# westlake-repl/Adapter4Rec

Hardware: AMD Instinct MI355X
Metric: user-sequences/sec, seq_len=23 BERT+SASRec+Adapter (higher is better)
Workload: dtype bf16

## Files before the change

adapter4rec_amd/_lib.py:

```python
import ctypes as C
import math
import os

import torch

_HERE = os.path.dirname(os.path.abspath(__file__))
LIB_PATH = os.environ.get('A4R_LIB_PATH') or os.path.join(_HERE, 'liba4r_hip.so')

ABI_VERSION = 411
BF16, F32, FP8 = 0, 1, 2
ACT_NONE, ACT_RELU, ACT_GELU, ACT_GELU_TANH, ACT_LEAKY = 0, 1, 2, 3, 4
DACT_MUL = 15
DACT_MUL_Q8 = 14
Q8_OFF, Q8_STEP = 0.1289, 0.0049326
EVAL_MAX_HISTORY = 264
ACT_BY_NAME = {'none': 0, 'relu': 1, 'RELU': 1, 'gelu': 2, 'GELU': 2, 'gelu_new': 3, 'leaky_relu': 4}

EXPORTS = [
    'a4r_version', 'a4r_gemm_nt', 'a4r_gemm_tn', 'a4r_gemm_tn_bias', 'a4r_gemm_tn_multi', 'a4r_gemm_tn2', 'a4r_colsum', 'a4r_attn_fwd', 'a4r_attn_bwd', 'a4r_embed_ln',
    'a4r_ln_fwd', 'a4r_ln_bwd', 'a4r_gather_rows', 'a4r_scatter_rows', 'a4r_rows_idx_copy', 'a4r_act_bwd_f32', 'a4r_score_bce_fwd',
    'a4r_score_bce_bwd', 'a4r_emb_grad_add_inputs', 'a4r_take_inputs', 'a4r_adam_step', 'a4r_pack_matrices',
    'a4r_eval_rank', 'a4r_dropout_apply', 'a4r_gemm_variant', 'a4r_gemm_tail_plan', 'a4r_gemm_tail_max', 'a4r_gemm_rows_256', 'a4r_adapter_ln_fwd', 'a4r_adapter_ln_bwd', 'a4r_ln_fwd_fp8', 'a4r_ln_fwd_sum', 'a4r_quant_rows_fp8', 'a4r_lora_merge', 'a4r_lora_merge_batch', 'a4r_lora_bwd_fused', 'a4r_lora_bwd_fused_ws_floats', 'a4r_phm_build', 'a4r_phm_bwd', 'a4r_unpack_add', 'a4r_memset_zero',
    'a4r_sasrec_block_fwd', 'a4r_sasrec_block_bwd', 'a4r_scatter_rows_fill', 'a4r_attn_long_fwd', 'a4r_attn_long_bwd', 'a4r_patchify', 'a4r_vit_assemble', 'a4r_resample_u8', 'a4r_embed_bwd', 'a4r_mae_keep_indices',
    'a4r_encoder_layer_fwd', 'a4r_encoder_layer_bwd', 'a4r_id_index', 'a4r_id_index_ws_ints', 'a4r_id_grad_sum',
    'a4r_topk_items', 'a4r_grad_sumsq', 'a4r_adamw_step',
]
ID_SUM_CHUNK = 16
TOPK_MAX_K = 256
TOPK_E = (64, 128, 256, 512)
GRAD_NORM_PARTS = 1024


class GemmArgs(C.Structure):
    _fields_ = [('A', C.c_void_p), ('B', C.c_void_p), ('C', C.c_void_p), ('bias', C.c_void_p), ('C2', C.c_void_p),
                ('R1', C.c_void_p), ('R2', C.c_void_p), ('Pre', C.c_void_p),
                ('M', C.c_int32), ('N', C.c_int32), ('K', C.c_int32),
                ('lda', C.c_int32), ('ldb', C.c_int32), ('ldc', C.c_int32), ('ldc2', C.c_int32),
                ('ldr1', C.c_int32), ('ldr2', C.c_int32), ('ldpre', C.c_int32),
                ('in_dtype', C.c_int32), ('out_dtype', C.c_int32), ('act', C.c_int32), ('dact', C.c_int32),
                ('drop_first', C.c_int32), ('c2_mode', C.c_int32), ('alpha', C.c_float), ('drop_p', C.c_float), ('drop_site', C.c_uint32), ('drop_seed', C.c_uint64),
                ('drop_row0', C.c_int64), ('scale_a', C.c_void_p), ('scale_b', C.c_void_p),
                ('c_fp8', C.c_int32), ('c_scale', C.c_float), ('c_scale_out', C.c_void_p), ('q8_tiled', C.c_int32)]


class AttnArgs(C.Structure):
    _fields_ = [('qkv', C.c_void_p), ('ld', C.c_int32), ('q_off', C.c_int32), ('k_off', C.c_int32), ('v_off', C.c_int32),
                ('out', C.c_void_p), ('ldo', C.c_int32), ('dout', C.c_void_p), ('dqkv', C.c_void_p), ('key_mask', C.c_void_p),
                ('n_items', C.c_int32), ('S', C.c_int32), ('n_heads', C.c_int32), ('dh', C.c_int32), ('causal', C.c_int32),
                ('dtype', C.c_int32), ('scale', C.c_float), ('mask_neg', C.c_float),
                ('drop_p', C.c_float), ('drop_site', C.c_uint32), ('drop_seed', C.c_uint64), ('offsets', C.c_void_p)]


class PackDesc(C.Structure):
    _fields_ = [('src_off', C.c_int64), ('dst', C.c_void_p), ('rows', C.c_int32), ('cols', C.c_int32),
                ('rows_pad', C.c_int32), ('cols_pad', C.c_int32), ('transpose', C.c_int32), ('dst_ld', C.c_int32)]


class PhmDesc(C.Structure):
    _fields_ = [('rule_off', C.c_int64), ('wl_off', C.c_int64), ('wr_off', C.c_int64), ('out_off', C.c_int64), ('G', C.c_void_p),
                ('ldg', C.c_int32), ('in_f', C.c_int32), ('out_f', C.c_int32), ('n', C.c_int32), ('pad_', C.c_int32)]


class LayerAdapter(C.Structure):
    _fields_ = [(n, C.c_void_p) for n in ('wd', 'wu', 'wdT', 'wuT', 'wd_f', 'wu_f', 'wdT_f', 'wuT_f', 'bd', 'bu', 'g_wu', 'g_wd', 'g_bu', 'g_bd')] + \
               [(n, C.c_int32) for n in ('ldg_wu', 'ldg_wd', 'act', 'pad_')]


class EncoderLayer(C.Structure):
    _fields_ = [(n, C.c_int32) for n in ('M', 'H', 'F', 'n_items', 'S', 'n_heads', 'dh', 'causal')] + \
               [(n, C.c_float) for n in ('scale', 'mask_neg', 'ln_eps', 'p_attn', 'p_hidden')] + [('drop_site', C.c_uint32), ('drop_seed', C.c_uint64)] + \
               [(n, C.c_void_p) for n in ('key_mask', 'offsets', 'wqkv', 'wqkvT', 'wo', 'woT', 'wi', 'wiT', 'wo2', 'wo2T',
                                          'bqkv', 'bo', 'bi', 'bo2', 'ln1_g', 'ln1_b', 'ln2_g', 'ln2_b')] + \
               [('ad', LayerAdapter * 2)] + \
               [(n, C.c_void_p) for n in ('qkv', 'ctx', 'h1', 'v1', 'zp1', 'z1', 'u', 'upre', 'h2', 'v2', 'zp2', 'z2', 'st1', 'st2')] + \
               [('upre_q8', C.c_int32), ('q8_tiled', C.c_int32)] + \
               [(n, C.c_void_p) for n in ('x_lo', 'x1_lo', 'xout_lo', 'dv1', 'dv2', 'dzp', 'd_h', 'du', 'dx1', 'dctx', 'dqkv')] + [('lo_nibble', C.c_int32)]


class SasrecBlock(C.Structure):
    _PTRS = ('wqkv', 'wfc', 'w1', 'b1', 'w2', 'b2', 'ln1_g', 'ln1_b', 'ln2_g', 'ln2_b', 'wd1', 'bd1', 'wu1', 'bu1', 'wd2', 'bd2', 'wu2', 'bu2',
             'g_wd1', 'g_bd1', 'g_wu1', 'g_bu1', 'g_wd2', 'g_bd2', 'g_wu2', 'g_bu2')
    _fields_ = [(n, C.c_void_p) for n in _PTRS] + \
               [(n, C.c_int32) for n in ('E', 'n_heads', 'F', 'd', 'ldwu', 'ldg_d', 'ldg_u', 'act', 'inner_res')] + \
               [(n, C.c_float) for n in ('eps', 'mask_neg', 'drop_attn', 'drop_hidden')] + [('drop_site', C.c_uint32), ('drop_seed', C.c_uint64)] + \
               [('mode', C.c_int32)] + [(n, C.c_void_p) for n in ('ln3_g', 'ln3_b', 'g_ln3_g', 'g_ln3_b')]


class AddDesc(C.Structure):
    _fields_ = [('src', C.c_void_p), ('dst_off', C.c_int64), ('rows', C.c_int32), ('cols', C.c_int32), ('ld', C.c_int32), ('alpha', C.c_float)]


_lib = None


def lib():
    global _lib
    if _lib is None:
        if not os.path.exists(LIB_PATH):
            raise RuntimeError(
                f'{LIB_PATH} not found: build it with `python -c "import __graft_entry__ as g; g.build()"` '
                '(hipcc --offload-arch=gfx950).  adapter4rec_amd has no CPU / PyTorch fallback.')
        _lib = C.CDLL(LIB_PATH)
        for name in EXPORTS:
            getattr(_lib, name).restype = C.c_int
        _lib.a4r_topk_ws_bytes.restype = C.c_size_t
        got = _lib.a4r_version()
        if got != ABI_VERSION:
            _lib = None
            raise RuntimeError(f'{LIB_PATH} has ABI version {got}, this binding is for {ABI_VERSION}: rebuild it (make -C adapter4rec_amd/csrc)')
    return _lib


def _check(rc, what):
    if rc != 0:
        raise RuntimeError(f'{what} failed with status {rc} ' + {-1: '(invalid argument)', -2: '(launch failure)'}.get(rc, ''))


_DEV_INDEX = None


def _stream():
    global _DEV_INDEX
    if _DEV_INDEX is None:
        _DEV_INDEX = torch.cuda.current_device()
    return C.c_void_p(torch._C._cuda_getCurrentRawStream(_DEV_INDEX))


def _p(t):
    return C.c_void_p(t.data_ptr()) if t is not None else C.c_void_p(0)


def _pi(t):
    return t.data_ptr() if t is not None else 0


def _dt(t):
    if t.dtype == torch.bfloat16:
        return BF16
    if t.dtype == torch.float32:
        return F32
    if t.dtype == torch.uint8:
        return FP8
    raise TypeError(f'unsupported dtype {t.dtype}')


def _ld(t):
    assert t.dim() == 2 and t.stride(1) == 1, 'row-major 2-D tensor expected'
    return t.stride(0)


def require_gpu(*tensors):
    for t in tensors:
        if t is not None and not t.is_cuda:
            raise RuntimeError('adapter4rec_amd kernels need device tensors (no CPU fallback)')


def gemm_nt(A, B, Cout, bias=None, C2=None, R1=None, R2=None, Pre=None, act=0, dact=0, alpha=1.0,
            drop_p=0.0, drop_site=0, drop_seed=0, M=None, drop_first=False, c2_deriv=False, scale_a=None, scale_b=None,
            c_fp8=0, c_scale=1.0, c_scale_out=None, q8_tiled=False):
    if not (A.is_cuda and B.is_cuda and Cout.is_cuda):
        require_gpu(A, B, Cout)
    N, K = B.shape
    din, dout = _dt(A), _dt(Cout)
    if c_fp8:
        assert din == FP8 and Cout.dtype == torch.uint8 and R1 is None and R2 is None and (c_fp8 == 1 or c_scale_out is not None)
        dout = BF16
    assert A.shape[1] == K and Cout.shape[1] == N and _dt(B) == din
    q8c, q8p = c2_deriv == 'q8', dact == DACT_MUL_Q8
    for t, q8 in ((C2, q8c), (R1, False), (R2, False), (Pre, q8p)):
        assert t is None or (t.dtype == torch.uint8 if q8 else _dt(t) == dout)
    assert bias is None or bias.dtype == torch.float32
    g = GemmArgs(A.data_ptr(), B.data_ptr(), Cout.data_ptr(), _pi(bias), _pi(C2), _pi(R1), _pi(R2), _pi(Pre),
                 A.shape[0] if M is None else M, N, K, _ld(A), _ld(B), _ld(Cout),
                 _ld(C2) if C2 is not None else 0, _ld(R1) if R1 is not None else 0, _ld(R2) if R2 is not None else 0,
                 _ld(Pre) if Pre is not None else 0, din, dout, act, dact, int(drop_first), 2 if q8c else int(bool(c2_deriv)), alpha, drop_p, drop_site,
                 drop_seed, 0, _pi(scale_a), _pi(scale_b), int(c_fp8), float(c_scale), _pi(c_scale_out), int(bool(q8_tiled)))
    _check(lib().a4r_gemm_nt(_stream(), C.byref(g)), 'a4r_gemm_nt')


def gemm_variant(v):
    return lib().a4r_gemm_variant(C.c_int(v))


def gemm_tail_max(k):
    return lib().a4r_gemm_tail_max(C.c_int(k))


def gemm_tail_plan(M, N):
    pf, kp = C.c_int(0), C.c_int(0)
    lib().a4r_gemm_tail_plan(C.c_int(M), C.c_int(N), C.byref(pf), C.byref(kp))
    return pf.value, kp.value


def gemm_rows_256(M, N):
    return lib().a4r_gemm_rows_256(C.c_int(M), C.c_int(N))


def adapter_ln_ok(A, d):
    return A.dtype == torch.bfloat16 and d == 64 and A.shape[1] in (128, 256, 512, 768, 1024)


def adapter_ln_fwd(A, R1, R2, Wd, bd, Wu, bu, gamma, beta, eps, act, zp, z, v, y, stats, M=None, y8=None, ys=None, res32=None, y32=None, frag=None):
    require_gpu(A, R1, R2, v, y, res32, y32)
    M = A.shape[0] if M is None else M
    assert y is not None or y8 is not None
    twins = [t for t in (res32, y32) if t is not None]
    lo8 = bool(twins) and twins[0].dtype == torch.int8
    assert all(t.dtype == (torch.int8 if lo8 else torch.float32) and t.shape[0] >= M for t in twins)
    lo4 = lo8 and twins[0].shape[1] == A.shape[1] // 2
    assert not lo8 or all(t.shape[1] == (A.shape[1] // 2 if lo4 else A.shape[1]) for t in twins)
    wd_, wu_ = (Wd, Wu) if frag is None else frag
    _check(lib().a4r_adapter_ln_fwd(_stream(), _p(A), C.c_int(_ld(A)), _p(R1), C.c_int(_ld(R1)), _p(R2), C.c_int(_ld(R2) if R2 is not None else 0),
                                    _p(wd_), _p(bd), _p(wu_), _p(bu), _p(gamma), _p(beta), C.c_float(eps), C.c_int(act),
                                    _p(zp), _p(z), _p(v), C.c_int(_ld(v) if v is not None else 0), _p(y), C.c_int(_ld(y) if y is not None else 0), _p(stats),
                                    C.c_int(M), C.c_int(A.shape[1]), C.c_int(Wd.shape[0]), C.c_int(_dt(A)),
                                    _p(y8), C.c_int(_ld(y8) if y8 is not None else 0), _p(ys),
                                    _p(res32), C.c_int(_ld(res32) if res32 is not None else 0), _p(y32), C.c_int(_ld(y32) if y32 is not None else 0),
                                    C.c_int((0 if frag is None else 1) | (2 if lo8 else 0) | (4 if lo4 else 0))),
           'a4r_adapter_ln_fwd')


def adapter_ln_bwd(dy, v, stats, gamma, dres, zp, act, WuT, WdT, inner_res, dv, dzp, dh, dgamma=None, dbeta=None, dbias=None, M=None,
                   drop_p=0.0, drop_site=0, drop_seed=0, dbd=None, bias_total=False, beta_y=None, frag=None):
    require_gpu(dy, v, dv, dh)
    M = dy.shape[0] if M is None else M
    wut_, wdt_ = (WuT, WdT) if frag is None else frag
    _check(lib().a4r_adapter_ln_bwd(_stream(), _p(dy), C.c_int(_ld(dy)), _p(v), C.c_int(_ld(v)), _p(stats), _p(gamma),
                                    _p(dres), C.c_int(_ld(dres) if dres is not None else 0), _p(zp), C.c_int(act), _p(wut_), _p(wdt_),
                                    C.c_int(int(inner_res)), _p(dv), C.c_int(_ld(dv)), _p(dzp), _p(dh), C.c_int(_ld(dh)),
                                    _p(dgamma), _p(dbeta), _p(dbias), C.c_int(M), C.c_int(dy.shape[1]), C.c_int(WuT.shape[0]), C.c_int(_dt(dy)),
                                    C.c_float(drop_p), C.c_uint32(drop_site), C.c_uint64(drop_seed), _p(dbd),
                                    C.c_int(int(bias_total) | (0 if frag is None else 2)), _p(beta_y)), 'a4r_adapter_ln_bwd')


def sasrec_block(desc, x, log_mask, out, n_users, T, train, dy=None):
    require_gpu(x, log_mask, out, dy)
    assert x.dtype == torch.float32 and out.dtype == torch.float32 and log_mask.dtype == torch.float32 and x.shape[1] == 64 and x.is_contiguous() and out.is_contiguous()
    b = SasrecBlock()
    for k, v in desc.items():
        setattr(b, k, (v.data_ptr() if v is not None else None) if (k in SasrecBlock._PTRS or k in ('ln3_g', 'ln3_b', 'g_ln3_g', 'g_ln3_b')) else v)
    if dy is None:
        _check(lib().a4r_sasrec_block_fwd(_stream(), C.byref(b), _p(x), _p(log_mask), _p(out), C.c_int(n_users), C.c_int(T), C.c_int(int(train))), 'a4r_sasrec_block_fwd')
    else:
        assert dy.dtype == torch.float32 and dy.is_contiguous()
        _check(lib().a4r_sasrec_block_bwd(_stream(), C.byref(b), _p(x), _p(log_mask), _p(dy), _p(out), C.c_int(n_users), C.c_int(T), C.c_int(int(train))),
               'a4r_sasrec_block_bwd')


def gemm_tn(X, Y, Cacc, M=None):
    require_gpu(X, Y, Cacc)
    assert Cacc.dtype == torch.float32 and _dt(X) == _dt(Y)
    M = X.shape[0] if M is None else M
    _check(lib().a4r_gemm_tn(_stream(), _p(X), C.c_int(_ld(X)), _p(Y), C.c_int(_ld(Y)), _p(Cacc), C.c_int(_ld(Cacc)),
                             C.c_int(M), C.c_int(X.shape[1]), C.c_int(Y.shape[1]), C.c_int(_dt(X))), 'a4r_gemm_tn')


def gemm_tn_bias(X, Y, Cacc, xsum, M=None):
    require_gpu(X, Y, Cacc, xsum)
    assert Cacc.dtype == torch.float32 and xsum.dtype == torch.float32 and xsum.numel() >= X.shape[1] and _dt(X) == _dt(Y)
    M = X.shape[0] if M is None else M
    _check(lib().a4r_gemm_tn_bias(_stream(), _p(X), C.c_int(_ld(X)), _p(Y), C.c_int(_ld(Y)), _p(Cacc), C.c_int(_ld(Cacc)),
                                  C.c_int(M), C.c_int(X.shape[1]), C.c_int(Y.shape[1]), C.c_int(_dt(X)), _p(xsum)), 'a4r_gemm_tn_bias')


class TnProb(C.Structure):
    _fields_ = [('X', C.c_void_p), ('Y', C.c_void_p), ('C', C.c_void_p), ('xsum', C.c_void_p),
                ('ldx', C.c_int32), ('ldy', C.c_int32), ('ldc', C.c_int32), ('P', C.c_int32), ('Q', C.c_int32), ('pad_', C.c_int32)]


def gemm_tn_multi(probs, M=None):
    assert 1 <= len(probs) <= 4
    arr = (TnProb * len(probs))()
    dt = _dt(probs[0][0])
    M = probs[0][0].shape[0] if M is None else M
    for a, (X, Y, Cacc, xsum) in zip(arr, probs):
        require_gpu(X, Y, Cacc, xsum)
        assert Cacc.dtype == torch.float32 and _dt(X) == dt and _dt(Y) == dt and (xsum is None or (xsum.dtype == torch.float32 and xsum.numel() >= X.shape[1]))
        a.X, a.Y, a.C, a.xsum = X.data_ptr(), Y.data_ptr(), Cacc.data_ptr(), (xsum.data_ptr() if xsum is not None else None)
        a.ldx, a.ldy, a.ldc, a.P, a.Q = _ld(X), _ld(Y), _ld(Cacc), X.shape[1], Y.shape[1]
    _check(lib().a4r_gemm_tn_multi(_stream(), arr, C.c_int(len(probs)), C.c_int(M), C.c_int(dt)), 'a4r_gemm_tn_multi')


def gemm_tn2(X1, Y1, C1, X2, Y2, C2, M=None, xsum1=None, xsum2=None):
    require_gpu(X1, Y1, C1, X2, Y2, C2, xsum1, xsum2)
    assert C1.dtype == torch.float32 and C2.dtype == torch.float32
    assert (xsum1 is None or (xsum1.dtype == torch.float32 and xsum1.numel() >= X1.shape[1])) and (xsum2 is None or (xsum2.dtype == torch.float32 and xsum2.numel() >= X2.shape[1]))
    M = X1.shape[0] if M is None else M
    _check(lib().a4r_gemm_tn2(_stream(), _p(X1), C.c_int(_ld(X1)), _p(Y1), C.c_int(_ld(Y1)), _p(C1), C.c_int(_ld(C1)), C.c_int(X1.shape[1]), C.c_int(Y1.shape[1]),
                              _p(X2), C.c_int(_ld(X2)), _p(Y2), C.c_int(_ld(Y2)), _p(C2), C.c_int(_ld(C2)), C.c_int(X2.shape[1]), C.c_int(Y2.shape[1]),
                              C.c_int(M), C.c_int(_dt(X1)), _p(xsum1), _p(xsum2)), 'a4r_gemm_tn2')


def colsum(X, out, M=None):
    require_gpu(X, out)
    M = X.shape[0] if M is None else M
    _check(lib().a4r_colsum(_stream(), _p(X), C.c_int(_ld(X)), _p(out), C.c_int(M), C.c_int(X.shape[1]), C.c_int(_dt(X))), 'a4r_colsum')


def _attn_args(qkv, q_off, k_off, v_off, key_mask, n_items, S, n_heads, dh, causal, scale, mask_neg, drop_p, drop_site, drop_seed, offsets=None):
    a = AttnArgs()
    if offsets is not None:
        require_gpu(offsets)
        assert offsets.dtype == torch.int32 and offsets.numel() >= n_items + 1
    a.offsets = _p(offsets)
    a.qkv, a.ld, a.q_off, a.k_off, a.v_off = _p(qkv), _ld(qkv), q_off, k_off, v_off
    a.key_mask = _p(key_mask)
    a.n_items, a.S, a.n_heads, a.dh, a.causal, a.dtype = n_items, S, n_heads, dh, int(causal), _dt(qkv)
    a.scale, a.mask_neg = scale, mask_neg
    a.drop_p, a.drop_site, a.drop_seed = drop_p, drop_site, drop_seed
    return a


def attn_fwd(qkv, out, key_mask, n_items, S, n_heads, dh, q_off, k_off, v_off, causal, scale, mask_neg,
             drop_p=0.0, drop_site=0, drop_seed=0, offsets=None):
    require_gpu(qkv, out)
    a = _attn_args(qkv, q_off, k_off, v_off, key_mask, n_items, S, n_heads, dh, causal, scale, mask_neg, drop_p, drop_site, drop_seed, offsets)
    a.out, a.ldo = _p(out), _ld(out)
    _check(lib().a4r_attn_fwd(_stream(), C.byref(a)), 'a4r_attn_fwd')


def attn_bwd(qkv, dout, dqkv, key_mask, n_items, S, n_heads, dh, q_off, k_off, v_off, causal, scale, mask_neg,
             drop_p=0.0, drop_site=0, drop_seed=0, offsets=None):
    require_gpu(qkv, dout, dqkv)
    assert _ld(dqkv) == _ld(qkv)
    a = _attn_args(qkv, q_off, k_off, v_off, key_mask, n_items, S, n_heads, dh, causal, scale, mask_neg, drop_p, drop_site, drop_seed, offsets)
    a.dout, a.ldo, a.dqkv = _p(dout), _ld(dout), _p(dqkv)
    _check(lib().a4r_attn_bwd(_stream(), C.byref(a)), 'a4r_attn_bwd')


def attn_long_fwd(qkv, out, lse, n_items, S, n_heads, dh, q_off, k_off, v_off, scale, drop_p=0.0, drop_site=0, drop_seed=0, key_mask=None, causal=False):
    require_gpu(qkv, out, lse, key_mask)
    assert lse.dtype == torch.float32 and lse.numel() >= n_items * n_heads * S
    a = _attn_args(qkv, q_off, k_off, v_off, key_mask, n_items, S, n_heads, dh, causal, scale, 0.0, drop_p, drop_site, drop_seed)
    a.out, a.ldo = _p(out), _ld(out)
    _check(lib().a4r_attn_long_fwd(_stream(), C.byref(a), _p(lse)), 'a4r_attn_long_fwd')


def attn_long_bwd(qkv, out, dout, dqkv, lse, delta_ws, n_items, S, n_heads, dh, q_off, k_off, v_off, scale,
                  drop_p=0.0, drop_site=0, drop_seed=0, key_mask=None, causal=False):
    require_gpu(qkv, out, dout, dqkv, lse, delta_ws, key_mask)
    assert _ld(dqkv) == _ld(qkv) and delta_ws.dtype == torch.float32 and delta_ws.numel() >= n_items * n_heads * S
    a = _attn_args(qkv, q_off, k_off, v_off, key_mask, n_items, S, n_heads, dh, causal, scale, 0.0, drop_p, drop_site, drop_seed)
    assert _ld(out) == _ld(dout)
    a.out, a.dout, a.ldo, a.dqkv = _p(out), _p(dout), _ld(dout), _p(dqkv)
    _check(lib().a4r_attn_long_bwd(_stream(), C.byref(a), _p(lse), _p(delta_ws)), 'a4r_attn_long_bwd')


def encoder_layer_fwd(desc, x, x1, x_out):
    require_gpu(x, x1, x_out)
    _check(lib().a4r_encoder_layer_fwd(_stream(), C.byref(desc), _p(x), _p(x1), _p(x_out)), 'a4r_encoder_layer_fwd')


def encoder_layer_bwd(desc, x1, x_out, dx_out, dx_in):
    require_gpu(x1, x_out, dx_out, dx_in)
    _check(lib().a4r_encoder_layer_bwd(_stream(), C.byref(desc), _p(x1), _p(x_out), _p(dx_out), _p(dx_in)), 'a4r_encoder_layer_bwd')


def patchify(img, out, patch, keep_idx=None):
    require_gpu(img, out)
    assert img.is_contiguous()
    if img.dtype == torch.uint8:
        kind, (n, Hi, Wi, Cc) = 1, img.shape
    else:
        assert img.dtype == torch.float32
        kind, (n, Cc, Hi, Wi) = 0, img.shape
    n_keep = keep_idx.shape[1] if keep_idx is not None else (Hi // patch) * (Wi // patch)
    assert keep_idx is None or (keep_idx.dtype == torch.int32 and keep_idx.is_contiguous() and keep_idx.shape[0] == n)
    _check(lib().a4r_patchify(_stream(), _p(img), C.c_int(kind), _p(out), C.c_int(_ld(out)), _p(keep_idx), C.c_int(n_keep),
                              C.c_int(n), C.c_int(Cc), C.c_int(Hi), C.c_int(Wi), C.c_int(patch), C.c_int(_dt(out))), 'a4r_patchify')


def mae_keep_indices(keep, n_patches, noise=None, seed=0, site=0):
    require_gpu(keep, noise)
    assert keep.dtype == torch.int32 and keep.is_contiguous()
    assert noise is None or (noise.dtype == torch.float32 and noise.is_contiguous() and tuple(noise.shape) == (keep.shape[0], n_patches))
    _check(lib().a4r_mae_keep_indices(_stream(), _p(noise), _p(keep), C.c_int(keep.shape[0]), C.c_int(n_patches), C.c_int(keep.shape[1]),
                                      C.c_uint64(int(seed) & (2 ** 64 - 1)), C.c_uint32(site)), 'a4r_mae_keep_indices')


def resample_u8(src, dst, bounds, kk, n_outer, in_len, out_len, inner):
    require_gpu(src, dst, bounds, kk)
    assert src.dtype == torch.uint8 and dst.dtype == torch.uint8 and bounds.dtype == torch.int32 and kk.dtype == torch.int32
    assert src.is_contiguous() and dst.is_contiguous() and src.numel() == n_outer * in_len * inner and dst.numel() == n_outer * out_len * inner
    _check(lib().a4r_resample_u8(_stream(), _p(src), _p(dst), _p(bounds), _p(kk), C.c_int(kk.shape[1]), C.c_long(n_outer),
                                 C.c_int(in_len), C.c_int(out_len), C.c_long(inner)), 'a4r_resample_u8')


def vit_assemble(patches, cls, pos, out, n_items, n_keep, keep_idx=None, tokens_out=0):
    require_gpu(patches, out)
    _check(lib().a4r_vit_assemble(_stream(), _p(patches), C.c_int(_ld(patches)), _p(cls), _p(pos), _p(keep_idx), _p(out),
                                  C.c_int(_ld(out)), C.c_int(n_items), C.c_int(n_keep), C.c_int(cls.numel()), C.c_int(_dt(out)),
                                  C.c_int(tokens_out)), 'a4r_vit_assemble')


def embed_bwd(ids, dpre, dword, dpos, n_items, S, roberta=False, pad_id=0):
    H = dpre.shape[1]
    assert ids.dtype == torch.int64 and ids.dim() == 2 and ids.stride(1) == 1, 'ids: int64 [n_items, >= S] with unit column stride'
    assert ids.shape[0] >= n_items and ids.shape[1] >= S, f'ids {tuple(ids.shape)} smaller than [{n_items}, {S}]'
    assert dpre.dim() == 2 and dpre.shape[0] >= n_items * S, f'dpre {tuple(dpre.shape)}: fewer than {n_items * S} rows'
    for name, t in (('dword', dword), ('dpos', dpos)):
        assert t is None or (t.dtype == torch.float32 and t.dim() == 2 and t.is_contiguous() and t.shape[1] == H), \
            f'{name}: contiguous fp32 [rows, {H}] expected, got {None if t is None else (t.dtype, tuple(t.shape), t.stride())}'
    n_pos = S + pad_id + 1 if roberta else S
    assert dpos is None or dpos.shape[0] >= n_pos, f'dpos has {dpos.shape[0]} rows, position ids reach {n_pos - 1}'
    require_gpu(ids, dpre, dword, dpos)
    _check(lib().a4r_embed_bwd(_stream(), _p(ids), C.c_int(ids.stride(0)), _p(dpre), C.c_int(_ld(dpre)), _p(dword), _p(dpos),
                               C.c_int(n_items), C.c_int(S), C.c_int(dpre.shape[1]), C.c_int(int(roberta)), C.c_int(pad_id),
                               C.c_int(_dt(dpre))), 'a4r_embed_bwd')


def embed_ln(ids, word, pos, type0, gamma, beta, eps, out, n_items, S, roberta=False, pad_id=0,
             drop_p=0.0, drop_site=0, drop_seed=0, pre_out=None, stats_out=None, key_mask_out=None):
    require_gpu(ids, word, out)
    assert ids.dtype == torch.int64 and ids.stride(1) == 1
    _check(lib().a4r_embed_ln(_stream(), _p(ids), C.c_int(ids.stride(0)), _p(word), _p(pos), _p(type0), _p(gamma), _p(beta),
                              C.c_float(eps), _p(out), C.c_int(_ld(out)), C.c_int(n_items), C.c_int(S), C.c_int(word.shape[1]),
                              C.c_int(int(roberta)), C.c_int(pad_id), C.c_int(_dt(out)),
                              C.c_float(drop_p), C.c_uint32(drop_site), C.c_uint64(drop_seed), _p(pre_out), _p(stats_out), _p(key_mask_out)), 'a4r_embed_ln')


def quantize_weight_fp8(w):
    wf = w.detach().float()
    amax = wf.abs().amax(1).clamp_min(1e-30)
    q = (wf * (448.0 / amax)[:, None]).to(torch.float8_e4m3fn).view(torch.uint8).contiguous()
    return q, (amax / 448.0).contiguous()


def quant_rows_fp8(x, q, scale, M=None):
    require_gpu(x, q, scale)
    M = x.shape[0] if M is None else M
    assert q.dtype == torch.uint8 and scale.dtype == torch.float32
    _check(lib().a4r_quant_rows_fp8(_stream(), _p(x), C.c_int(_ld(x)), _p(q), C.c_int(_ld(q)), _p(scale), C.c_int(M), C.c_int(x.shape[1]),
                                    C.c_int(_dt(x))), 'a4r_quant_rows_fp8')


def ln_fwd_sum(h, res, gamma, beta, eps, y, stats, M=None, res32=None, sum_out=None, sum32=None, y32=None):
    require_gpu(h, res, res32, y, sum_out, sum32, y32)
    M = h.shape[0] if M is None else M
    assert res32 is not None or res is not None
    _check(lib().a4r_ln_fwd_sum(_stream(), _p(h), C.c_int(_ld(h)), _p(res32), C.c_int(_ld(res32) if res32 is not None else 0), _p(res),
                                C.c_int(_ld(res) if res is not None else 0), _p(gamma), _p(beta), C.c_float(eps), _p(y), C.c_int(_ld(y)),
                                _p(sum_out), C.c_int(_ld(sum_out) if sum_out is not None else 0), _p(sum32), C.c_int(_ld(sum32) if sum32 is not None else 0),
                                _p(y32), C.c_int(_ld(y32) if y32 is not None else 0), _p(stats), C.c_int(M), C.c_int(h.shape[1]), C.c_int(_dt(h))),
           'a4r_ln_fwd_sum')


def ln_fwd(v, gamma, beta, eps, y, stats, M=None, add=None, drop_p=0.0, drop_site=0, drop_seed=0, y8=None, ys=None):
    require_gpu(v, y, y8)
    M = v.shape[0] if M is None else M
    if y8 is not None:
        assert drop_p == 0.0 and y8.dtype == torch.uint8 and ys.dtype == torch.float32
        _check(lib().a4r_ln_fwd_fp8(_stream(), _p(v), C.c_int(_ld(v)), _p(add), C.c_int(add.shape[0] if add is not None else 0),
                                    _p(gamma), _p(beta), C.c_float(eps), _p(y), C.c_int(_ld(y) if y is not None else 0), _p(y8), C.c_int(_ld(y8)),
                                    _p(ys), _p(stats), C.c_int(M), C.c_int(v.shape[1]), C.c_int(_dt(v))), 'a4r_ln_fwd_fp8')
        return
    _check(lib().a4r_ln_fwd(_stream(), _p(v), C.c_int(_ld(v)), _p(add), C.c_int(add.shape[0] if add is not None else 0),
                            _p(gamma), _p(beta), C.c_float(eps), _p(y), C.c_int(_ld(y)), _p(stats), C.c_int(M),
                            C.c_int(v.shape[1]), C.c_int(_dt(v)), C.c_float(drop_p), C.c_uint32(drop_site), C.c_uint64(drop_seed)),
           'a4r_ln_fwd')


def ln_bwd(dy, v, stats, gamma, dv, M=None, add=None, dgamma=None, dbeta=None, dbias=None, dres=None,
           drop_p=0.0, drop_site=0, drop_seed=0, dv2=None, drop2_p=0.0, drop2_site=0, drop2_seed=0):
    require_gpu(dy, v, dv)
    M = v.shape[0] if M is None else M
    _check(lib().a4r_ln_bwd(_stream(), _p(dy), C.c_int(_ld(dy)), _p(v), C.c_int(_ld(v)), _p(add),
                            C.c_int(add.shape[0] if add is not None else 0), _p(stats), _p(gamma), _p(dres), C.c_int(_ld(dres) if dres is not None else 0), _p(dv), C.c_int(_ld(dv)),
                            _p(dgamma), _p(dbeta), _p(dbias), C.c_int(M), C.c_int(v.shape[1]), C.c_int(_dt(v)),
                            C.c_float(drop_p), C.c_uint32(drop_site), C.c_uint64(drop_seed),
                            _p(dv2), C.c_int(_ld(dv2) if dv2 is not None else 0), C.c_float(drop2_p), C.c_uint32(drop2_site), C.c_uint64(drop2_seed)), 'a4r_ln_bwd')


def gather_rows(src, dst, n, row_step):
    require_gpu(src, dst)
    _check(lib().a4r_gather_rows(_stream(), _p(src), C.c_int(_ld(src)), _p(dst), C.c_int(_ld(dst)), C.c_int(n), C.c_int(row_step),
                                 C.c_int(src.shape[1]), C.c_int(_dt(src))), 'a4r_gather_rows')


def rows_idx_copy(src, dst, idx, n, scatter=False):
    require_gpu(src, dst, idx)
    assert src.dim() == 2 and dst.dim() == 2 and src.dtype == dst.dtype and src.shape[1] == dst.shape[1] and idx.dtype == torch.int32 and idx.numel() >= n
    es = src.element_size()
    _check(lib().a4r_rows_idx_copy(_stream(), _p(src), C.c_int64(src.stride(0) * es), _p(dst), C.c_int64(dst.stride(0) * es), _p(idx), C.c_int(n),
                                   C.c_int64(src.shape[1] * es), C.c_int(int(scatter))), 'a4r_rows_idx_copy')


def id_index_ws_ints(n, item_num):
    k = int(lib().a4r_id_index_ws_ints(C.c_int(n), C.c_int(item_num)))
    if k < 0:
        raise RuntimeError(f'a4r_id_index: n = {n}, item_num = {item_num} outside the supported range (include/a4r.h)')
    return k


def id_index(ids, item_num, rows, slots, ptr, uniq, n_uniq, err, ws):
    require_gpu(ids, rows, slots, ptr, uniq, n_uniq, err, ws)
    n = ids.numel()
    assert ids.dtype == torch.int64 and ids.is_contiguous() and ws.dtype == torch.int32
    assert all(t.dtype == torch.int32 for t in (rows, slots, ptr, uniq, n_uniq, err))
    assert rows.numel() >= n and slots.numel() >= n and ptr.numel() >= n + 1 and uniq.numel() >= n
    _check(lib().a4r_id_index(_stream(), _p(ids), C.c_int(n), C.c_int(item_num), _p(rows), _p(slots), _p(ptr), _p(uniq), _p(n_uniq), _p(err),
                              _p(ws), C.c_int64(ws.numel())), 'a4r_id_index')


def id_grad_sum(src, slots, ptr, uniq, n_uniq, n, grad):
    require_gpu(src, slots, ptr, uniq, n_uniq, grad)
    assert src.dtype == torch.float32 and grad.dtype == torch.float32 and src.shape[1] == grad.shape[1] and src.shape[0] >= n
    _check(lib().a4r_id_grad_sum(_stream(), _p(src), C.c_int(_ld(src)), _p(slots), _p(ptr), _p(uniq), _p(n_uniq), C.c_int(n), _p(grad),
                                 C.c_int(_ld(grad)), C.c_int(grad.shape[1])), 'a4r_id_grad_sum')


def scatter_rows(src, dst, n, row_step):
    require_gpu(src, dst)
    _check(lib().a4r_scatter_rows(_stream(), _p(src), C.c_int(_ld(src)), _p(dst), C.c_int(_ld(dst)), C.c_int(n), C.c_int(row_step),
                                  C.c_int(src.shape[1]), C.c_int(_dt(src))), 'a4r_scatter_rows')


def scatter_rows_fill(src, dst, n, row_step, fill_rows):
    require_gpu(src, dst)
    _check(lib().a4r_scatter_rows_fill(_stream(), _p(src), C.c_int(_ld(src)), _p(dst), C.c_int(_ld(dst)), C.c_int(n), C.c_int(row_step),
                                       C.c_int(src.shape[1]), C.c_int(_dt(src)), C.c_int(fill_rows)), 'a4r_scatter_rows_fill')


def zero(t):
    require_gpu(t)
    assert t.is_contiguous()
    _check(lib().a4r_memset_zero(_stream(), _p(t), C.c_int64(t.numel() * t.element_size())), 'a4r_memset_zero')


def lora_merge(W, A, B, scaling, dst, dstT, r):
    require_gpu(W, dst, dstT)
    out_f, in_f = W.shape
    assert W.dtype == torch.float32 and W.is_contiguous() and (r == 0 or (A.is_contiguous() and B.is_contiguous()))
    _check(lib().a4r_lora_merge(_stream(), _p(W), _p(A) if r else C.c_void_p(0), _p(B) if r else C.c_void_p(0), C.c_float(scaling),
                                _p(dst), C.c_int(_ld(dst)), _p(dstT), C.c_int(_ld(dstT)), C.c_int(out_f), C.c_int(in_f), C.c_int(r),
                                C.c_int(_dt(dst))), 'a4r_lora_merge')


class LoraDesc(C.Structure):
    _fields_ = [('W', C.c_void_p), ('A', C.c_void_p), ('B', C.c_void_p), ('dst', C.c_void_p), ('dstT', C.c_void_p),
                ('scaling', C.c_float), ('ld', C.c_int32), ('ldT', C.c_int32), ('out_f', C.c_int32), ('in_f', C.c_int32), ('r', C.c_int32)]


def lora_table(entries, device):
    descs = []
    for W, A, B, s, dst, dstT, r in entries:
        assert W.dtype == torch.float32 and W.is_contiguous() and (r == 0 or (A.is_contiguous() and B.is_contiguous())) and _dt(dst) == _dt(entries[0][4])
        descs.append(LoraDesc(W.data_ptr(), A.data_ptr() if r else 0, B.data_ptr() if r else 0, dst.data_ptr(), dstT.data_ptr(), float(s),
                              _ld(dst), _ld(dstT), W.shape[0], W.shape[1], int(r)))
    return desc_table(descs, device), len(descs), max(W.numel() for W, *_ in entries), _dt(entries[0][4])


def lora_merge_batch(tab):
    t, n, mx, code = tab
    _check(lib().a4r_lora_merge_batch(_stream(), _p(t), C.c_int(n), C.c_int(mx), C.c_int(code)), 'a4r_lora_merge_batch')


def lora_bwd_fused_ok(x, M, H):
    return x.dtype == torch.bfloat16 and H == 768 and M % 16 == 0


_lora_ws = {}


def lora_bwd_fused(x, dqa, dqb, Aa, Ab, BTa, BTb, scale_a, scale_b, dAa, dAb, dBa, dBb, dbias_a, dbias_b, M, rank_rows=8):
    require_gpu(x, dqa, dqb, dAa, dBa)
    H = x.shape[1]
    assert _ld(dqa) == _ld(dqb) and _ld(Aa) == _ld(Ab) == _ld(BTa) == _ld(BTb) and _ld(dAa) == _ld(dAb) and _ld(dBa) == _ld(dBb)
    ldbias = 0
    for bvec in (dbias_a, dbias_b):
        if bvec is not None:
            assert bvec.dtype == torch.float32 and bvec.dim() == 1
            ldbias = bvec.stride(0)
    ws = _lora_ws.get(x.device)
    if ws is None:
        ws = _lora_ws[x.device] = torch.empty(int(lib().a4r_lora_bwd_fused_ws_floats(C.c_int(H))), dtype=torch.float32, device=x.device)
    _check(lib().a4r_lora_bwd_fused(_stream(), _p(x), C.c_int(_ld(x)), _p(dqa), _p(dqb), C.c_int(_ld(dqa)), _p(Aa), _p(Ab), _p(BTa), _p(BTb),
                                    C.c_int(_ld(Aa)), C.c_float(scale_a), C.c_float(scale_b), _p(dAa), _p(dAb), C.c_int(_ld(dAa)), _p(dBa), _p(dBb),
                                    C.c_int(_ld(dBa)), _p(dbias_a), _p(dbias_b), C.c_int(ldbias), C.c_int(M), C.c_int(H), C.c_int(_dt(x)),
                                    C.c_int(rank_rows), _p(ws), C.c_int64(ws.numel())), 'a4r_lora_bwd_fused')


def desc_table(entries, device):
    arr = (type(entries[0]) * len(entries))(*entries)
    return torch.frombuffer(bytearray(bytes(arr)), dtype=torch.uint8).to(device)


def phm_build(params, desc_dev, n_desc, eff):
    _check(lib().a4r_phm_build(_stream(), _p(params), _p(desc_dev), C.c_int(n_desc), _p(eff)), 'a4r_phm_build')


def phm_bwd(params, desc_dev, n_desc, grads):
    _check(lib().a4r_phm_bwd(_stream(), _p(params), _p(desc_dev), C.c_int(n_desc), _p(grads)), 'a4r_phm_bwd')


def unpack_add(target, desc_dev, n_desc, max_elems):
    _check(lib().a4r_unpack_add(_stream(), _p(target), _p(desc_dev), C.c_int(n_desc), C.c_int(max_elems)), 'a4r_unpack_add')


def dropout_apply(x, y, drop_p, drop_site, drop_seed, M=None):
    require_gpu(x, y)
    M = x.shape[0] if M is None else M
    _check(lib().a4r_dropout_apply(_stream(), _p(x), C.c_int(_ld(x)), _p(y), C.c_int(_ld(y)), C.c_int(M), C.c_int(x.shape[1]),
                                   C.c_int(_dt(x)), C.c_float(drop_p), C.c_uint32(drop_site), C.c_uint64(drop_seed)), 'a4r_dropout_apply')


def act_bwd_f32(dy, pre, dx, act):
    require_gpu(dy, pre, dx)
    _check(lib().a4r_act_bwd_f32(_stream(), _p(dy), _p(pre), _p(dx), C.c_int64(dy.numel()), C.c_int(act)), 'a4r_act_bwd_f32')


def score_bce_fwd(emb, prec, log_mask, pos, neg, loss_ws, B, L, E, cpc):
    require_gpu(emb, prec)
    _check(lib().a4r_score_bce_fwd(_stream(), _p(emb), _p(prec), _p(log_mask), _p(pos), _p(neg), _p(loss_ws),
                                   C.c_int(B), C.c_int(L), C.c_int(E), C.c_int(int(cpc))), 'a4r_score_bce_fwd')


def score_bce_bwd(emb, prec, log_mask, pos, neg, loss_ws, loss_scale, d_prec, d_emb, B, L, E, cpc, scale_dev=None):
    require_gpu(emb, prec, scale_dev)
    assert scale_dev is None or (scale_dev.dtype == torch.float32 and scale_dev.numel() == 1)
    _check(lib().a4r_score_bce_bwd(_stream(), _p(emb), _p(prec), _p(log_mask), _p(pos), _p(neg), _p(loss_ws), C.c_float(loss_scale), _p(scale_dev),
                                   _p(d_prec), _p(d_emb), C.c_int(B), C.c_int(L), C.c_int(E), C.c_int(int(cpc))), 'a4r_score_bce_bwd')


def emb_grad_add_inputs(d_in, d_emb, B, L, E):
    _check(lib().a4r_emb_grad_add_inputs(_stream(), _p(d_in), C.c_int(_ld(d_in)), _p(d_emb), C.c_int(B), C.c_int(L), C.c_int(E)),
           'a4r_emb_grad_add_inputs')


def take_inputs(emb, out, B, L, E):
    _check(lib().a4r_take_inputs(_stream(), _p(emb), _p(out), C.c_int(_ld(out)), C.c_int(B), C.c_int(L), C.c_int(E)), 'a4r_take_inputs')
# ... 98 lines not shown
```

adapter4rec_amd/csrc/a4r_attn.hip:

```cpp
#include <cstdlib>
#include "a4r_common.h"
#include "../../include/a4r.h"

namespace {

template <typename T> A4R_DEV uint4 ldg16(const T* p) { return *reinterpret_cast<const uint4*>(p); }

A4R_DEV void wave_lds_fence() {
    asm volatile("s_waitcnt lgkmcnt(0)" ::: "memory");
    __builtin_amdgcn_wave_barrier();
}

template <typename T, int STRIDE> A4R_DEV void lds_put16(char* tile, int row, int ch, const uint4& v) {
    char* d = tile + row * STRIDE + ch * 16;
    if constexpr (STRIDE % 16 == 0) {
        *reinterpret_cast<uint4*>(d) = v;
    } else {
        reinterpret_cast<uint2*>(d)[0] = make_uint2(v.x, v.y);
        reinterpret_cast<uint2*>(d)[1] = make_uint2(v.z, v.w);
    }
}

template <typename T, int DH> struct AttnCfg {
    static constexpr int PER = Elem<T>::PER16;
    static constexpr int KSTEP = Mma<T>::KSTEP;
    static constexpr int KSD = DH / KSTEP;
    static constexpr int KSP = 32 / KSTEP;
    static constexpr int DT = DH / 16;
    static constexpr int CPR = DH / PER;
    static constexpr int NLD = 32 * CPR / 64;
    static constexpr int PSTRIDE = 32 * (int)sizeof(T);
    static constexpr int GSTRIDE = DH * (int)sizeof(T) + (sizeof(T) == 2 ? 8 : 16);
    static constexpr int OSTRIDE = DH * (int)sizeof(T);
};

template <typename T, int DH>
A4R_DEV void qk_scores(const T* base, int ld, int q_off, int k_off, int S, int lane, f32x4_t (&sc)[2][2]) {
    using C = AttnCfg<T, DH>;
    const int r16 = lane & 15, kg = lane >> 4;
#pragma unroll
    for (int mt = 0; mt < 2; ++mt)
#pragma unroll
        for (int nt = 0; nt < 2; ++nt) sc[mt][nt] = f32x4_t{0.f, 0.f, 0.f, 0.f};
#pragma unroll
    for (int ks = 0; ks < C::KSD; ++ks) {
        uint4 qa[2], kb[2];
#pragma unroll
        for (int t = 0; t < 2; ++t) {
            const int row = min(t * 16 + r16, S - 1);
            qa[t] = ldg16(base + (size_t)row * ld + q_off + (ks * 4 + kg) * C::PER);
            kb[t] = ldg16(base + (size_t)row * ld + k_off + (ks * 4 + kg) * C::PER);
        }
#pragma unroll
        for (int mt = 0; mt < 2; ++mt)
#pragma unroll
            for (int nt = 0; nt < 2; ++nt) Mma<T>::mma(qa[mt], kb[nt], sc[mt][nt]);
    }
}

A4R_DEV void softmax_row(const float (&s)[2], int q, int r16, int S, const float (&km)[2], int causal, float scale, float mask_neg,
                         float (&p)[2]) {
    float x[2];
#pragma unroll
    for (int nt = 0; nt < 2; ++nt) {
        const int key = nt * 16 + r16;
        const float v = s[nt] * scale;
        const bool allowed = (km[nt] != 0.f) && (!causal || key <= q);
        x[nt] = key < S ? (allowed ? v : v + mask_neg) : -INFINITY;
    }
    const float m = group16_max(fmaxf(x[0], x[1]));
    const float e0 = expf(x[0] - m), e1 = expf(x[1] - m);
    const float inv = 1.f / group16_sum(e0 + e1);
    p[0] = e0 * inv;
    p[1] = e1 * inv;
}

template <typename T, int DH, int WAVES>
__global__ void __launch_bounds__(WAVES * 64) attn_fwd_kernel(const T* __restrict__ qkv, int ld, int q_off, int k_off, int v_off,
                                                              T* __restrict__ out, int ldo, const float* __restrict__ key_mask,
                                                              int n_items, int S_in, int n_heads, int causal, float scale, float mask_neg,
                                                              uint64_t seed, uint32_t site, uint32_t thr16, float keep_scale,
                                                              const int* __restrict__ offsets) {
    using C = AttnCfg<T, DH>;
    constexpr int WAVE_LDS = 32 * C::PSTRIDE + 32 * C::GSTRIDE;
    extern __shared__ __attribute__((aligned(16))) char smem[];
    const int lane = threadIdx.x & 63, wave = threadIdx.x >> 6;
    const int r16 = lane & 15, kg = lane >> 4;
    char* Ps = smem + wave * WAVE_LDS;
    char* Vs = Ps + 32 * C::PSTRIDE;
    const int total = n_items * n_heads;
    int gw = blockIdx.x * WAVES + wave;
    const bool active = gw < total;
    if (!active) gw = total - 1;
    const int item = gw / n_heads, head = gw % n_heads;
    const int row0 = offsets ? __builtin_amdgcn_readfirstlane(offsets[item]) : item * S_in;
    const int S = offsets ? __builtin_amdgcn_readfirstlane(offsets[item + 1]) - row0 : S_in;
    const T* base = qkv + (size_t)row0 * ld + head * DH;

    float km[2];
#pragma unroll
    for (int nt = 0; nt < 2; ++nt) {
        const int key = nt * 16 + r16;
        km[nt] = key_mask ? key_mask[(size_t)row0 + min(key, S - 1)] : 1.f;
    }
    uint4 sv[C::NLD];
#pragma unroll
    for (int i = 0; i < C::NLD; ++i) {
        const int id = lane + 64 * i, row = id / C::CPR, ch = id % C::CPR;
        sv[i] = ldg16(base + (size_t)min(row, S - 1) * ld + v_off + ch * C::PER);
    }
    f32x4_t sc[2][2];
    qk_scores<T, DH>(base, ld, q_off, k_off, S, lane, sc);
#pragma unroll
    for (int nt = 0; nt < 2; ++nt)
        if (nt * 16 + r16 >= S) km[nt] = 0.f;

#pragma unroll
    for (int i = 0; i < C::NLD; ++i) {
        const int id = lane + 64 * i, row = id / C::CPR, ch = id % C::CPR;
        lds_put16<T, C::GSTRIDE>(Vs, row, ch, row < S ? sv[i] : make_uint4(0u, 0u, 0u, 0u));
    }

#pragma unroll
    for (int mt = 0; mt < 2; ++mt)
#pragma unroll
        for (int rr = 0; rr < 4; ++rr) {
            const int q = mt * 16 + kg * 4 + rr;
            const float s2[2] = {sc[mt][0][rr], sc[mt][1][rr]};
            float p[2];
            softmax_row(s2, q, r16, S, km, causal, scale, mask_neg, p);
#pragma unroll
            for (int nt = 0; nt < 2; ++nt) {
                const int key = nt * 16 + r16;
                float pv = p[nt];
                if (thr16) pv = dropout_keep(seed, site, ((uint64_t)gw * 32 + q) * 32 + key, thr16) ? pv * keep_scale : 0.f;
                Elem<T>::st(reinterpret_cast<T*>(Ps + q * C::PSTRIDE) + key, pv);
            }
        }
    wave_lds_fence();

    f32x4_t o[2][C::DT];
#pragma unroll
    for (int mt = 0; mt < 2; ++mt)
#pragma unroll
        for (int dt = 0; dt < C::DT; ++dt) o[mt][dt] = f32x4_t{0.f, 0.f, 0.f, 0.f};
#pragma unroll
    for (int ks = 0; ks < C::KSP; ++ks) {
        uint4 pa[2];
#pragma unroll
        for (int mt = 0; mt < 2; ++mt)
            pa[mt] = *reinterpret_cast<const uint4*>(Ps + (mt * 16 + r16) * C::PSTRIDE + (ks * 4 + kg) * 16);
#pragma unroll
        for (int dt = 0; dt < C::DT; ++dt) {
            const uint4 vb = gather_chunk<T>(Vs, C::GSTRIDE, ks * C::KSTEP, dt * 16, lane);
#pragma unroll
            for (int mt = 0; mt < 2; ++mt) Mma<T>::mma(pa[mt], vb, o[mt][dt]);
        }
    }
    wave_lds_fence();
#pragma unroll
    for (int mt = 0; mt < 2; ++mt)
#pragma unroll
        for (int dt = 0; dt < C::DT; ++dt)
#pragma unroll
            for (int rr = 0; rr < 4; ++rr)
                Elem<T>::st(reinterpret_cast<T*>(Vs + (mt * 16 + kg * 4 + rr) * C::OSTRIDE) + dt * 16 + r16, o[mt][dt][rr]);
    wave_lds_fence();
    if (active) {
#pragma unroll
        for (int i = 0; i < C::NLD; ++i) {
            const int id = lane + 64 * i, row = id / C::CPR, ch = id % C::CPR;
            if (row < S)
                *reinterpret_cast<uint4*>(out + ((size_t)row0 + row) * ldo + head * DH + ch * C::PER) =
                    *reinterpret_cast<const uint4*>(Vs + row * C::OSTRIDE + ch * 16);
        }
    }
}

template <typename T, int DH>
A4R_DEV void img_times_tile(const char* Aimg, const char* Gtile, int lane, f32x4_t (&acc)[2][AttnCfg<T, DH>::DT]) {
    using C = AttnCfg<T, DH>;
    const int r16 = lane & 15, kg = lane >> 4;
#pragma unroll
    for (int t = 0; t < 2; ++t)
#pragma unroll
        for (int dt = 0; dt < C::DT; ++dt) acc[t][dt] = f32x4_t{0.f, 0.f, 0.f, 0.f};
#pragma unroll
    for (int ks = 0; ks < C::KSP; ++ks) {
        uint4 a[2];
#pragma unroll
        for (int t = 0; t < 2; ++t) a[t] = *reinterpret_cast<const uint4*>(Aimg + (t * 16 + r16) * C::PSTRIDE + (ks * 4 + kg) * 16);
#pragma unroll
        for (int dt = 0; dt < C::DT; ++dt) {
            const uint4 b = gather_chunk<T>(Gtile, C::GSTRIDE, ks * C::KSTEP, dt * 16, lane);
#pragma unroll
            for (int t = 0; t < 2; ++t) Mma<T>::mma(a[t], b, acc[t][dt]);
        }
    }
}

template <typename T, int DH>
A4R_DEV void store_block(char* stage, const f32x4_t (&acc)[2][AttnCfg<T, DH>::DT], T* gdst, int ldg, int S, int lane, bool active) {
    using C = AttnCfg<T, DH>;
    const int r16 = lane & 15, kg = lane >> 4;
#pragma unroll
    for (int t = 0; t < 2; ++t)
#pragma unroll
        for (int dt = 0; dt < C::DT; ++dt)
#pragma unroll
            for (int rr = 0; rr < 4; ++rr)
                Elem<T>::st(reinterpret_cast<T*>(stage + (t * 16 + kg * 4 + rr) * C::OSTRIDE) + dt * 16 + r16, acc[t][dt][rr]);
    wave_lds_fence();
    if (active) {
#pragma unroll
        for (int i = 0; i < C::NLD; ++i) {
            const int id = lane + 64 * i, row = id / C::CPR, ch = id % C::CPR;
            if (row < S)
                *reinterpret_cast<uint4*>(gdst + (size_t)row * ldg + ch * C::PER) =
                    *reinterpret_cast<const uint4*>(stage + row * C::OSTRIDE + ch * 16);
        }
    }
}

template <typename T, int DH, int WAVES>
__global__ void __launch_bounds__(WAVES * 64) attn_bwd_kernel(const T* __restrict__ qkv, int ld, int q_off, int k_off, int v_off,
                                                              const T* __restrict__ dout, int ldo, T* __restrict__ dqkv,
                                                              const float* __restrict__ key_mask, int n_items, int S_in, int n_heads,
                                                              int causal, float scale, float mask_neg,
                                                              uint64_t seed, uint32_t site, uint32_t thr16, float keep_scale,
                                                              const int* __restrict__ offsets) {
    using C = AttnCfg<T, DH>;
    constexpr int TILE = 32 * C::GSTRIDE, IMG = 32 * C::PSTRIDE;
    constexpr int WAVE_LDS = 3 * TILE + 3 * IMG;
    extern __shared__ __attribute__((aligned(16))) char smem[];
    const int lane = threadIdx.x & 63, wave = threadIdx.x >> 6;
    const int r16 = lane & 15, kg = lane >> 4;
    char* Qs = smem + wave * WAVE_LDS;
    char* Ks = Qs + TILE;
    char* dOs = Ks + TILE;
    char* PT = dOs + TILE;
    char* dS = PT + IMG;
    char* dST = dS + IMG;
    const int total = n_items * n_heads;
    int gw = blockIdx.x * WAVES + wave;
    const bool active = gw < total;
    if (!active) gw = total - 1;
    const int item = gw / n_heads, head = gw % n_heads;
    const int row0 = offsets ? __builtin_amdgcn_readfirstlane(offsets[item]) : item * S_in;
    const int S = offsets ? __builtin_amdgcn_readfirstlane(offsets[item + 1]) - row0 : S_in;
    const T* base = qkv + (size_t)row0 * ld + head * DH;
    const T* dbase = dout + (size_t)row0 * ldo + head * DH;
    T* gbase = dqkv + (size_t)row0 * ld + head * DH;

    float km[2];
#pragma unroll
    for (int nt = 0; nt < 2; ++nt) {
        const int key = nt * 16 + r16;
        km[nt] = key_mask ? key_mask[(size_t)row0 + min(key, S - 1)] : 1.f;
    }
    uint4 fq[C::KSD][2], fk[C::KSD][2], fd[C::KSD][2], fv[C::KSD][2];
#pragma unroll
    for (int ks = 0; ks < C::KSD; ++ks)
#pragma unroll
        for (int t = 0; t < 2; ++t) {
            const int row = t * 16 + r16, rc = min(row, S - 1);
            fq[ks][t] = ldg16(base + (size_t)rc * ld + q_off + (ks * 4 + kg) * C::PER);
            fk[ks][t] = ldg16(base + (size_t)rc * ld + k_off + (ks * 4 + kg) * C::PER);
            fv[ks][t] = ldg16(base + (size_t)rc * ld + v_off + (ks * 4 + kg) * C::PER);
            fd[ks][t] = ldg16(dbase + (size_t)rc * ldo + (ks * 4 + kg) * C::PER);
        }
#pragma unroll
    for (int nt = 0; nt < 2; ++nt)
        if (nt * 16 + r16 >= S) km[nt] = 0.f;
#pragma unroll
    for (int ks = 0; ks < C::KSD; ++ks)
#pragma unroll
        for (int t = 0; t < 2; ++t) {
            const int row = t * 16 + r16, ch = ks * 4 + kg;
            const bool in = row < S;
            const uint4 z = make_uint4(0u, 0u, 0u, 0u);
            lds_put16<T, C::GSTRIDE>(Qs, row, ch, in ? fq[ks][t] : z);
            lds_put16<T, C::GSTRIDE>(Ks, row, ch, in ? fk[ks][t] : z);
            if (!in) fd[ks][t] = z;
            lds_put16<T, C::GSTRIDE>(dOs, row, ch, fd[ks][t]);
        }

    f32x4_t sc[2][2], dp[2][2];
#pragma unroll
    for (int mt = 0; mt < 2; ++mt)
#pragma unroll
        for (int nt = 0; nt < 2; ++nt) { sc[mt][nt] = f32x4_t{0.f, 0.f, 0.f, 0.f}; dp[mt][nt] = sc[mt][nt]; }
#pragma unroll
    for (int ks = 0; ks < C::KSD; ++ks)
#pragma unroll
        for (int mt = 0; mt < 2; ++mt)
#pragma unroll
            for (int nt = 0; nt < 2; ++nt) {
                Mma<T>::mma(fq[ks][mt], fk[ks][nt], sc[mt][nt]);
                Mma<T>::mma(fd[ks][mt], fv[ks][nt], dp[mt][nt]);
            }

#pragma unroll
    for (int mt = 0; mt < 2; ++mt)
#pragma unroll
        for (int rr = 0; rr < 4; ++rr) {
            const int q = mt * 16 + kg * 4 + rr;
            const float s2[2] = {sc[mt][0][rr], sc[mt][1][rr]};
            float p[2], g[2], pd[2];
            softmax_row(s2, q, r16, S, km, causal, scale, mask_neg, p);
#pragma unroll
            for (int nt = 0; nt < 2; ++nt) {
                const int key = nt * 16 + r16;
                float keepf = 1.f;
                if (thr16) keepf = dropout_keep(seed, site, ((uint64_t)gw * 32 + q) * 32 + key, thr16) ? keep_scale : 0.f;
                pd[nt] = p[nt] * keepf;
                g[nt] = dp[mt][nt][rr] * keepf;
            }
            const float delta = group16_sum(g[0] * p[0] + g[1] * p[1]);
#pragma unroll
            for (int nt = 0; nt < 2; ++nt) {
                const int key = nt * 16 + r16;
                const float ds = p[nt] * (g[nt] - delta) * scale;
                Elem<T>::st(reinterpret_cast<T*>(PT + key * C::PSTRIDE) + q, pd[nt]);
                Elem<T>::st(reinterpret_cast<T*>(dS + q * C::PSTRIDE) + key, ds);
                Elem<T>::st(reinterpret_cast<T*>(dST + key * C::PSTRIDE) + q, ds);
            }
        }
    wave_lds_fence();

    f32x4_t acc[2][C::DT];
    img_times_tile<T, DH>(PT, dOs, lane, acc);
    wave_lds_fence();
    store_block<T, DH>(dOs, acc, gbase + v_off, ld, S, lane, active);
    img_times_tile<T, DH>(dST, Qs, lane, acc);
    wave_lds_fence();
    store_block<T, DH>(Qs, acc, gbase + k_off, ld, S, lane, active);
    img_times_tile<T, DH>(dS, Ks, lane, acc);
    wave_lds_fence();
    store_block<T, DH>(Ks, acc, gbase + q_off, ld, S, lane, active);
}

#ifndef A4R_ATTN_BWD_ABL_CT
#define A4R_ATTN_BWD_ABL_CT 0
#endif
typedef short bt_v4s_t __attribute__((ext_vector_type(4)));
template <int DH> struct BtGeo {
    static constexpr int ROWB = DH * 2, CPR = DH / 8, KSD = DH / 32, ND = DH / 16, IMG = 32 * ROWB;
    static constexpr int WAVE_LDS = 2 * IMG + (IMG > 4096 ? IMG : 4096);
    static A4R_DEV int swz(int row) { return CPR == 8 ? ((row >> 1) & 7) : ((row >> 2) & 3); }
};
template <int DH> A4R_DEV uint4 bt_frag_tr(const char* img, int d0, int lane) {
    using G = BtGeo<DH>;
    const int kg = lane >> 4, q = (lane >> 2) & 3, pp = lane & 3;
    const int chunk = (d0 >> 3) + (pp >> 1);
    const int r0 = 4 * kg + q, r1 = r0 + 16;
    const char* a0 = img + r0 * G::ROWB + ((chunk ^ G::swz(r0)) << 4) + 8 * (pp & 1);
    const char* a1 = img + r1 * G::ROWB + ((chunk ^ G::swz(r1)) << 4) + 8 * (pp & 1);
    const bt_v4s_t lo = __builtin_amdgcn_ds_read_tr16_b64_v4i16((__attribute__((address_space(3))) bt_v4s_t*)(a0));
    const bt_v4s_t hi = __builtin_amdgcn_ds_read_tr16_b64_v4i16((__attribute__((address_space(3))) bt_v4s_t*)(a1));
    const uint2 l2 = __builtin_bit_cast(uint2, lo), h2 = __builtin_bit_cast(uint2, hi);
    return make_uint4(l2.x, l2.y, h2.x, h2.y);
}
A4R_DEV uint4 bt_pack(const f32x4_t& a, const f32x4_t& b) {
    return make_uint4(pack2_bf16(a[0], a[1]), pack2_bf16(a[2], a[3]),
                      pack2_bf16(b[0], b[1]), pack2_bf16(b[2], b[3]));
}
A4R_DEV void bt_store4(bf16_t* p, const f32x4_t& v) {
    *reinterpret_cast<uint2*>(p) = make_uint2(pack2_bf16(v[0], v[1]),
                                              pack2_bf16(v[2], v[3]));
}
A4R_DEV float bt_red4(float v, bool mx) {
    const float a = __shfl_xor(v, 16, 64);
    v = mx ? fmaxf(v, a) : v + a;
    const float b = __shfl_xor(v, 32, 64);
    return mx ? fmaxf(v, b) : v + b;
}

template <int DH, int WAVES>
__global__ void __launch_bounds__(WAVES * 64, 3) attn_bwd_tr_kernel(const bf16_t* __restrict__ qkv, int ld, int q_off, int k_off, int v_off,
                                                                 const bf16_t* __restrict__ dout, int ldo, bf16_t* __restrict__ dqkv,
                                                                 const float* __restrict__ key_mask, int n_items, int S_in, int n_heads,
                                                                 int causal, float scale, float mask_neg,
                                                                 uint64_t seed, uint32_t site, uint32_t thr16, float keep_scale,
                                                                 const int* __restrict__ offsets) {
    using T = bf16_t;
    using G = BtGeo<DH>;
    extern __shared__ __attribute__((aligned(16))) char smem[];
    const int lane = threadIdx.x & 63, wave = threadIdx.x >> 6;
    const int r16 = lane & 15, kg = lane >> 4;
    char* Qi = smem + wave * G::WAVE_LDS;
    char* Oi = Qi + G::IMG;
    char* Ki = Oi + G::IMG;
    const int total = n_items * n_heads;
    const int gw = blockIdx.x * WAVES + wave;
    if (gw >= total) return;
    const int item = gw / n_heads, head = gw % n_heads;
    const int row0 = offsets ? __builtin_amdgcn_readfirstlane(offsets[item]) : item * S_in;
    const int S = offsets ? __builtin_amdgcn_readfirstlane(offsets[item + 1]) - row0 : S_in;
    const T* base = qkv + (size_t)row0 * ld + head * DH;
    const T* dbase = dout + (size_t)row0 * ldo + head * DH;
    T* gbase = dqkv + (size_t)row0 * ld + head * DH;

    float kmT[2][4];
#pragma unroll
    for (int nt = 0; nt < 2; ++nt)
#pragma unroll
        for (int r = 0; r < 4; ++r) {
            const int kt = nt * 16 + kg * 4 + r;
            kmT[nt][r] = (kt < S) ? (key_mask ? key_mask[(size_t)row0 + kt] : 1.f) : 0.f;
        }
    uint4 fq[G::KSD][2], fk[G::KSD][2], fd[G::KSD][2], fv[G::KSD][2];
#pragma unroll
    for (int ks = 0; ks < G::KSD; ++ks)
#pragma unroll
        for (int t = 0; t < 2; ++t) {
            const int row = t * 16 + r16, rc = min(row, S - 1);
            if (A4R_ATTN_BWD_ABL_CT & 2) { fq[ks][t] = make_uint4(lane, ks, t, 1); fk[ks][t] = fq[ks][t]; fv[ks][t] = fq[ks][t]; fd[ks][t] = fq[ks][t]; continue; }
            fq[ks][t] = ldg16(base + (size_t)rc * ld + q_off + (ks * 4 + kg) * 8);
            fk[ks][t] = ldg16(base + (size_t)rc * ld + k_off + (ks * 4 + kg) * 8);
            fv[ks][t] = ldg16(base + (size_t)rc * ld + v_off + (ks * 4 + kg) * 8);
            fd[ks][t] = ldg16(dbase + (size_t)rc * ldo + (ks * 4 + kg) * 8);
        }
#pragma unroll
    for (int ks = 0; ks < G::KSD; ++ks)
#pragma unroll
        for (int t = 0; t < 2; ++t) {
            const int row = t * 16 + r16, off = row * G::ROWB + (((ks * 4 + kg) ^ G::swz(row)) << 4);
            if (row >= S) fd[ks][t] = make_uint4(0u, 0u, 0u, 0u);
            *reinterpret_cast<uint4*>(Qi + off) = fq[ks][t];
            *reinterpret_cast<uint4*>(Ki + off) = fk[ks][t];
            *reinterpret_cast<uint4*>(Oi + off) = fd[ks][t];
        }
    f32x4_t scT[2][2], dpT[2][2];
#pragma unroll
    for (int a = 0; a < 2; ++a)
#pragma unroll
        for (int b = 0; b < 2; ++b) { scT[a][b] = f32x4_t{0.f, 0.f, 0.f, 0.f}; dpT[a][b] = scT[a][b]; }
#pragma unroll
    for (int ks = 0; ks < G::KSD; ++ks)
#pragma unroll
        for (int mt = 0; mt < 2; ++mt)
#pragma unroll
            for (int nt = 0; nt < 2; ++nt) {
                Mma<T>::mma(fk[ks][nt], fq[ks][mt], scT[nt][mt]);
                Mma<T>::mma(fv[ks][nt], fd[ks][mt], dpT[nt][mt]);
            }
    wave_lds_fence();
    uint2 pw[2][2], dw[2][2];
    f32x4_t aq[2][G::ND], av[2][G::ND], ak[2][G::ND];
#pragma unroll
    for (int mt = 0; mt < 2; ++mt) {
        const int q = mt * 16 + r16;
        float x[2][4];
        float m = -INFINITY;
#pragma unroll
        for (int nt = 0; nt < 2; ++nt)
#pragma unroll
            for (int r = 0; r < 4; ++r) {
                const int key = nt * 16 + kg * 4 + r;
                const float v = scT[nt][mt][r] * scale;
                const bool allowed = (kmT[nt][r] != 0.f) && (!causal || key <= q);
                x[nt][r] = key < S ? (allowed ? v : v + mask_neg) : -INFINITY;
                m = fmaxf(m, x[nt][r]);
            }
        m = bt_red4(m, true);
        float l = 0.f;
#pragma unroll
        for (int nt = 0; nt < 2; ++nt)
#pragma unroll
            for (int r = 0; r < 4; ++r) { x[nt][r] = __expf(x[nt][r] - m); l += x[nt][r]; }
        const float inv = 1.f / bt_red4(l, false);
        float dsum = 0.f;
        f32x4_t pk[2];
#pragma unroll
        for (int nt = 0; nt < 2; ++nt) {
            uint64_t hsh = 0;
            if (thr16) hsh = a4r_hash64(seed, site, (((uint64_t)gw * 32 + q) * 32 + nt * 16 + kg * 4) >> 2);
#pragma unroll
            for (int r = 0; r < 4; ++r) {
                x[nt][r] *= inv;
                float keepf = 1.f;
                if (thr16) keepf = (((uint32_t)(hsh >> (16 * r)) & 0xffffu) >= thr16) ? keep_scale : 0.f;
                dpT[nt][mt][r] *= keepf;
                pk[nt][r] = x[nt][r] * keepf;
                dsum += dpT[nt][mt][r] * x[nt][r];
            }
        }
        dsum = bt_red4(dsum, false);
#pragma unroll
        for (int nt = 0; nt < 2; ++nt) {
#pragma unroll
            for (int r = 0; r < 4; ++r) dpT[nt][mt][r] = x[nt][r] * (dpT[nt][mt][r] - dsum) * scale;
            pw[nt][mt] = make_uint2(pack2_bf16(pk[nt][0], pk[nt][1]),
                                    pack2_bf16(pk[nt][2], pk[nt][3]));
            dw[nt][mt] = make_uint2(pack2_bf16(dpT[nt][mt][0], dpT[nt][mt][1]),
                                    pack2_bf16(dpT[nt][mt][2], dpT[nt][mt][3]));
        }
        const uint4 dsB = make_uint4(dw[0][mt].x, dw[0][mt].y, dw[1][mt].x, dw[1][mt].y);
#pragma unroll
        for (int dt = 0; dt < G::ND; ++dt) {
            aq[mt][dt] = f32x4_t{0.f, 0.f, 0.f, 0.f};
            Mma<T>::mma(bt_frag_tr<DH>(Ki, dt * 16, lane), dsB, aq[mt][dt]);
        }
    }
    wave_lds_fence();
    unsigned short* Pt = reinterpret_cast<unsigned short*>(Ki);
    unsigned short* Dt = Pt + 32 * 32;
#pragma unroll
    for (int nt = 0; nt < 2; ++nt)
#pragma unroll
        for (int mt = 0; mt < 2; ++mt) {
            const int q = mt * 16 + r16, k0 = nt * 16 + kg * 4;
            Pt[(k0 + 0) * 32 + q] = (unsigned short)(pw[nt][mt].x & 0xffffu);
            Pt[(k0 + 1) * 32 + q] = (unsigned short)(pw[nt][mt].x >> 16);
            Pt[(k0 + 2) * 32 + q] = (unsigned short)(pw[nt][mt].y & 0xffffu);
            Pt[(k0 + 3) * 32 + q] = (unsigned short)(pw[nt][mt].y >> 16);
            Dt[(k0 + 0) * 32 + q] = (unsigned short)(dw[nt][mt].x & 0xffffu);
            Dt[(k0 + 1) * 32 + q] = (unsigned short)(dw[nt][mt].x >> 16);
            Dt[(k0 + 2) * 32 + q] = (unsigned short)(dw[nt][mt].y & 0xffffu);
            Dt[(k0 + 3) * 32 + q] = (unsigned short)(dw[nt][mt].y >> 16);
        }
    wave_lds_fence();
#pragma unroll
    for (int nt = 0; nt < 2; ++nt) {
        const int key = nt * 16 + r16;
        const uint2 p0 = *reinterpret_cast<const uint2*>(Pt + key * 32 + kg * 4), p1 = *reinterpret_cast<const uint2*>(Pt + key * 32 + 16 + kg * 4);
        const uint2 d0 = *reinterpret_cast<const uint2*>(Dt + key * 32 + kg * 4), d1 = *reinterpret_cast<const uint2*>(Dt + key * 32 + 16 + kg * 4);
        const uint4 pB = make_uint4(p0.x, p0.y, p1.x, p1.y), dsB = make_uint4(d0.x, d0.y, d1.x, d1.y);
#pragma unroll
        for (int dt = 0; dt < G::ND; ++dt) {
            av[nt][dt] = f32x4_t{0.f, 0.f, 0.f, 0.f};
            ak[nt][dt] = f32x4_t{0.f, 0.f, 0.f, 0.f};
            Mma<T>::mma(bt_frag_tr<DH>(Oi, dt * 16, lane), pB, av[nt][dt]);
            Mma<T>::mma(bt_frag_tr<DH>(Qi, dt * 16, lane), dsB, ak[nt][dt]);
        }
    }
    wave_lds_fence();
#pragma unroll
    for (int t = 0; t < 2; ++t) {
        const int tok = t * 16 + r16;
#pragma unroll
        for (int dt = 0; dt < G::ND; ++dt) {
            const int off = tok * G::ROWB + (((dt * 2 + (kg >> 1)) ^ G::swz(tok)) << 4) + 8 * (kg & 1);
            bt_store4(reinterpret_cast<T*>(Qi + off), aq[t][dt]);
            bt_store4(reinterpret_cast<T*>(Oi + off), av[t][dt]);
            bt_store4(reinterpret_cast<T*>(Ki + off), ak[t][dt]);
        }
    }
    wave_lds_fence();
    if (!(A4R_ATTN_BWD_ABL_CT & 1)) {
#pragma unroll
        for (int i = 0; i < 32 * G::CPR / 64; ++i) {
            const int id = lane + 64 * i, row = id / G::CPR, ch = id % G::CPR;
            if (row < S) {
                const int off = row * G::ROWB + ((ch ^ G::swz(row)) << 4);
                *reinterpret_cast<uint4*>(gbase + (size_t)row * ld + q_off + ch * 8) = *reinterpret_cast<const uint4*>(Qi + off);
                *reinterpret_cast<uint4*>(gbase + (size_t)row * ld + v_off + ch * 8) = *reinterpret_cast<const uint4*>(Oi + off);
                *reinterpret_cast<uint4*>(gbase + (size_t)row * ld + k_off + ch * 8) = *reinterpret_cast<const uint4*>(Ki + off);
            }
        }
    }
}

struct Launch {
    hipStream_t s; const a4r_attn_t* a; uint32_t thr; float ks;
};

template <typename T, int DH, int WAVES>
int launch_fwd(const Launch& L) {
    using C = AttnCfg<T, DH>;
    const a4r_attn_t& a = *L.a;
    constexpr int LDS = WAVES * (32 * C::PSTRIDE + 32 * C::GSTRIDE);
    const int total = a.n_items * a.n_heads;
    hipLaunchKernelGGL((attn_fwd_kernel<T, DH, WAVES>), dim3((total + WAVES - 1) / WAVES), dim3(WAVES * 64), LDS, L.s,
                       (const T*)a.qkv, a.ld, a.q_off, a.k_off, a.v_off, (T*)a.out, a.ldo, a.offsets ? nullptr : a.key_mask, a.n_items, a.S, a.n_heads,
                       a.causal, a.scale, a.mask_neg, a.drop_seed, a.drop_site, L.thr, L.ks, a.offsets);
    return a4r_launch_status();
}
template <typename T, int DH, int WAVES>
int launch_bwd(const Launch& L) {
    using C = AttnCfg<T, DH>;
    const a4r_attn_t& a = *L.a;
    constexpr int LDS = WAVES * (3 * 32 * C::GSTRIDE + 3 * 32 * C::PSTRIDE);
    static bool lds_ok = false;
    if (!lds_ok) {
        if (int rc = a4r_set_lds(attn_bwd_kernel<T, DH, WAVES>, LDS)) return rc;
        lds_ok = true;
    }
    const int total = a.n_items * a.n_heads;
    hipLaunchKernelGGL((attn_bwd_kernel<T, DH, WAVES>), dim3((total + WAVES - 1) / WAVES), dim3(WAVES * 64), LDS, L.s,
                       (const T*)a.qkv, a.ld, a.q_off, a.k_off, a.v_off, (const T*)a.dout, a.ldo, (T*)a.dqkv, a.offsets ? nullptr : a.key_mask,
                       a.n_items, a.S, a.n_heads, a.causal, a.scale, a.mask_neg, a.drop_seed, a.drop_site, L.thr, L.ks, a.offsets);
    return a4r_launch_status();
}

template <int DH, int WAVES>
int launch_bwd_tr(const Launch& L) {
    const a4r_attn_t& a = *L.a;
    constexpr int LDS = WAVES * BtGeo<DH>::WAVE_LDS;
    static bool lds_ok = false;
    if (!lds_ok) {
        if (int rc = a4r_set_lds(attn_bwd_tr_kernel<DH, WAVES>, LDS)) return rc;
        lds_ok = true;
    }
    const int total = a.n_items * a.n_heads;
    hipLaunchKernelGGL((attn_bwd_tr_kernel<DH, WAVES>), dim3((total + WAVES - 1) / WAVES), dim3(WAVES * 64), LDS, L.s,
                       (const bf16_t*)a.qkv, a.ld, a.q_off, a.k_off, a.v_off, (const bf16_t*)a.dout, a.ldo, (bf16_t*)a.dqkv, a.offsets ? nullptr : a.key_mask,
                       a.n_items, a.S, a.n_heads, a.causal, a.scale, a.mask_neg, a.drop_seed, a.drop_site, L.thr, L.ks, a.offsets);
    return a4r_launch_status();
}

int check(const a4r_attn_t* a, bool bwd) {
    if (!a || !a->qkv) return A4R_EINVAL;
    if (bwd ? (!a->dout || !a->dqkv) : !a->out) return A4R_EINVAL;
    if (a->dtype != A4R_BF16 && a->dtype != A4R_F32) return A4R_EINVAL;
    const bool narrow = a->dh > 0 && a->dh <= 16;
    const bool wide = (a->dh == 128 || a->dh == 256) && a->dtype == A4R_F32 && !a->offsets;
    if (a->n_items <= 0 || a->n_heads <= 0 || a->S <= 0 || a->S > 32 || (a->dh != 32 && a->dh != 64 && !narrow && !wide)) return A4R_EINVAL;
    const int esz = a->dtype == A4R_F32 ? 4 : 2, per = narrow ? 1 : 16 / esz;
    if ((a->ld * esz) % 16 || (a->ldo * esz) % 16 || a->q_off % per || a->k_off % per || a->v_off % per) return A4R_EINVAL;
    if (a->ldo < a->n_heads * a->dh) return A4R_EINVAL;
    if (a->drop_p < 0.f || a->drop_p >= 1.f) return A4R_EINVAL;
    if (a->offsets && narrow) return A4R_EINVAL;
    uintptr_t m = reinterpret_cast<uintptr_t>(a->qkv) | reinterpret_cast<uintptr_t>(a->out) | reinterpret_cast<uintptr_t>(a->dout) |
                  reinterpret_cast<uintptr_t>(a->dqkv);
    if (m & 15u) return A4R_EINVAL;
    return A4R_OK;
}

}

int a4r_attn_small(hipStream_t s, const a4r_attn_t* t, bool bwd);

extern "C" int a4r_attn_fwd(void* stream, const a4r_attn_t* a) {
    if (int e = check(a, false)) return e;
    if (a->dh <= 16) return a4r_attn_small(reinterpret_cast<hipStream_t>(stream), a, false);
    Launch L{reinterpret_cast<hipStream_t>(stream), a, a4r_thr16(a->drop_p), a4r_keep_scale(a->drop_p)};
    if (a->dtype == A4R_BF16) return a->dh == 64 ? launch_fwd<bf16_t, 64, 4>(L) : launch_fwd<bf16_t, 32, 4>(L);
    if (a->dh == 128) return launch_fwd<float, 128, 2>(L);
    if (a->dh == 256) return launch_fwd<float, 256, 1>(L);
    return a->dh == 64 ? launch_fwd<float, 64, 4>(L) : launch_fwd<float, 32, 4>(L);
}

extern "C" int a4r_attn_bwd(void* stream, const a4r_attn_t* a) {
    if (int e = check(a, true)) return e;
    if (a->dh <= 16) return a4r_attn_small(reinterpret_cast<hipStream_t>(stream), a, true);
    Launch L{reinterpret_cast<hipStream_t>(stream), a, a4r_thr16(a->drop_p), a4r_keep_scale(a->drop_p)};
    if (a->dtype == A4R_BF16) {
        return a->dh == 64 ? launch_bwd_tr<64, 4>(L) : launch_bwd_tr<32, 4>(L);
    }
    if (a->dh == 128) return launch_bwd<float, 128, 1>(L);
    if (a->dh == 256) return launch_bwd<float, 256, 1>(L);
    return a->dh == 64 ? launch_bwd<float, 64, 2>(L) : launch_bwd<float, 32, 4>(L);
}
```

adapter4rec_amd/engine.py:

```python
import math
import os as _os

import torch

from . import _lib as L
from .model.bert import backbone_geometry
from .model.modules import AdapterBlock, AdapterPfeifferBlock, HyperComplexAdapterBlock, PHMLinear

FMIN = float(torch.finfo(torch.float32).min)


def pad_to(n, m):
    return (n + m - 1) // m * m


def _skip_unused_items():
    return _os.environ.get('A4R_SKIP_UNUSED_ITEMS', '1')


WGRAD_STREAM = bool(int(_os.environ.get('A4R_WGRAD_STREAM', '0')))

class _LN:

    def __init__(self, mod, eng):
# ... 509 lines not shown
            self.cls_only = False

    def _build_bert(self, bert):
        g = self.geo
        H, nh = g['hidden_size'], g['num_attention_heads']
        self.H, self.F = H, g['intermediate_size']
        if H % 64 or self.F % 64 or (H // nh) not in (32, 64) or self.S > 256 or (self.S > 32 and H // nh != 64):
            raise NotImplementedError(f'encoder geometry H={H} F={self.F} heads={nh} S={self.S}')
        emb = bert.embeddings
        tab = lambda p: p.data if p.requires_grad else self._f32(p)
        wemb = emb.word_embeddings
        self.prompt_n, self.g_prompt = 0, None
        if type(wemb).__name__ == 'SoftEmbedding':
            self.prompt_n = int(wemb.n_tokens)
            if self.prompt_n > self.S:
                raise ValueError(f'--n_tokens {self.prompt_n} exceeds the title length {self.S}')
            self.prompt_param = wemb.learned_embedding
            self.g_prompt = self.grad_view(wemb.learned_embedding)
            wemb = wemb.wte
            if wemb.weight.requires_grad:
                raise NotImplementedError('soft prompt together with a trainable vocabulary table')
            V = wemb.weight.shape[0]
            self.prompt_V = V
            self.emb_word_ext = torch.cat([self._f32(wemb.weight), torch.zeros(self.prompt_n, H, device=self.dev)], 0)
        self.emb_word, self.emb_pos = tab(wemb.weight), tab(emb.position_embeddings.weight)
        self.emb_type = tab(emb.token_type_embeddings.weight)
        self.emb_type0 = self.emb_type[0]
        self.emb_ln = _LN(emb.LayerNorm, self)
        self.g_word, self.g_pos = self.grad_view(wemb.weight), self.grad_view(emb.position_embeddings.weight)
        self.g_type = self.grad_view(emb.token_type_embeddings.weight)
        self.train_emb = any(f is not None for f in (self.g_word, self.g_pos, self.g_type, self.emb_ln.g_gamma, self.emb_ln.g_beta, self.g_prompt))
        if getattr(bert, 'pooler', None) is not None:
            for p in bert.pooler.parameters():
                self.grad_view(p)
        self.cls_only = bool(getattr(self.args, 'cls_only_last', True))
        self.roberta = g['model_type'] == 'roberta'
        self.pad_id = int(g['pad_token_id'])
        self.p_hidden = float(g['hidden_dropout_prob'])
        self.p_attn = float(g['attention_probs_dropout_prob'])
        self.bert_blocks = []
        for i, layer in enumerate(bert.encoder.layer):
            b = _Block()
            att = layer.attention.self
            for lin in (att.query, att.key, att.value):
                if type(lin).__name__ not in ('LoRALinear', 'Linear'):
                    raise NotImplementedError(f'projection module {type(lin).__name__}')
            b.lora = _Lora.for_block((att.query, att.key, att.value), H, self, self.T)
            b.H, b.F, b.nh, b.dh, b.S = H, self.F, nh, H // nh, self.S
            b.is_item = True
            b.long = self.S > 32
            b.causal, b.mask_neg, b.scale = False, FMIN, 1.0 / math.sqrt(H // nh)
            b.ffn_act = L.ACT_GELU
            b.p_hidden, b.p_attn, b.site = self.p_hidden, self.p_attn, 16 * i
            b.wqkv = torch.zeros(3 * H, H, dtype=self.T, device=self.dev)
            b.wqkvT = torch.zeros(H, 3 * H, dtype=self.T, device=self.dev)
            b.bqkv = torch.zeros(3 * H, dtype=torch.float32, device=self.dev)
            self._pack_lora_bias(b, H)
            b.qkv = tuple(None if type(lin).__name__ == 'LoRALinear' else
                          _Dense(self, lin.weight, lin.bias, self.T, b.wqkv[sl * H:(sl + 1) * H], b.wqkvT[:, sl * H:(sl + 1) * H],
                                 b.bqkv[sl * H:(sl + 1) * H])
                          for sl, lin in enumerate((att.query, att.key, att.value)))
            d1, ln1, ad1, pl1, lnn1 = self._so(layer.attention.output, H, self.T)
            d2, ln2, ad2, pl2, lnn2 = self._so(layer.output, H, self.T)
            b.d_o = _Dense(self, d1.weight, d1.bias, self.T)
            b.d_i = _Dense(self, layer.intermediate.dense.weight, layer.intermediate.dense.bias, self.T)
            b.d_o2 = _Dense(self, d2.weight, d2.bias, self.T)
            b.wo, b.woT, b.bo = b.d_o.w, b.d_o.wT, b.d_o.b
            b.wi, b.wiT, b.bi = b.d_i.w, b.d_i.wT, b.d_i.b
            b.wo2, b.wo2T, b.bo2 = b.d_o2.w, b.d_o2.wT, b.d_o2.b
            b.train_dense = any(d is not None and d.trainable for d in b.qkv + (b.d_o, b.d_i, b.d_o2))
            b.ln1, b.ln2 = _LN(ln1, self), _LN(ln2, self)
            b.ad1, b.ad2, b.pl1, b.pl2, b.lnn1, b.lnn2 = ad1, ad2, pl1, pl2, lnn1, lnn2
            b.need_dx = i > 0 or self.train_emb
            b.T = self.T
            self.bert_blocks.append(b)
        lastb = self.bert_blocks[-1]
        if lastb.pl1 == 'parallel' or lastb.pl2 == 'parallel':
            self.cls_only = False

    def _build_head(self):
        fc = self.model.bert_encoder.text_encoders['title'].fc
        self.d_fc = _Dense(self, fc.weight, fc.bias, self.T)
        self.fc_w, self.fc_b = self.d_fc.w, self.d_fc.b
        self.fc_wT32 = torch.zeros(fc.in_features, fc.out_features, dtype=torch.float32, device=self.dev)
        if fc.weight.requires_grad:
            self.add_pack(fc.weight, self.fc_wT32, True)
        else:
            self.fc_wT32.copy_(fc.weight.detach().t().float())
        if self.E % 64:
            raise NotImplementedError('item head: embedding_dim % 64 == 0')

    def _build_sasrec(self):
        te = self.model.user_encoder.transformer_encoder
        E, nh = self.E, self.args.num_attention_heads
        if (E // nh) not in (32, 64, 128, 256) or E % nh or self.Lseq - 1 > 256 or (self.Lseq - 1 > 32 and (E // nh) not in (32, 64)
                                                                                   and not (E // nh == 128 and self.Lseq - 1 <= 128)):
            raise NotImplementedError(f'SASRec geometry E={E} heads={nh} T={self.Lseq - 1}')
        pe = te.position_embedding.weight
        self.pos_emb = pe.data if pe.requires_grad else self._f32(pe)
        self.g_pos_emb = self.grad_view(pe)
        self.sas_ln0 = _LN(te.layer_norm, self)
        self.p_sas = float(self.args.drop_rate)
        f32 = torch.float32
        self.sas_blocks = []
        kad = type(te.transformer_blocks).__name__ == 'SASRecKAdaptedTransformerBlocks'
        block_list = te.transformer_blocks.transformer_blocks if kad else te.transformer_blocks
        for j, blk in enumerate(block_list):
            tb = blk.transformer_block if hasattr(blk, 'transformer_block') else blk
            b = self._make_block(tb, E, nh, self.Lseq - 1, f32, True, -1e9, self.p_sas, 4096 + 16 * j)
            placement = getattr(blk, 'placement', None) if blk is not tb else None
            if blk is not tb:
                if placement == 'pfeiffer':
                    b.ad2, b.pl2, b.lnn2 = self._adapter_of(blk, 'adapter', E, f32), 'pfeiffer', _LN(blk.LN, self)
                else:
                    b.ad1 = self._adapter_of(blk, 'adapter1', E, f32)
                    b.ad2 = self._adapter_of(blk, 'adapter2', E, f32)
                    b.pl1 = (placement or 'serial') if b.ad1 else None
                    b.pl2 = (placement or 'serial') if b.ad2 else None
            self.sas_blocks.append(b)
        self.sas_kads, self.d_com2 = [], None
        if kad:
            tbs = te.transformer_blocks
            self.sas_kads = [self._make_kadapter(m, E, self.Lseq - 1, f32, 5000 + 64 * j) for j, m in enumerate(tbs.adapter_list)]
            self.d_com2 = _Dense(self, tbs.com_dense2.weight, tbs.com_dense2.bias, f32)

    def _sas_fused_ok(self):
        if self.sas_kads or not self.sas_blocks or self.Lseq - 1 > 32:
            return False
        for b in self.sas_blocks:
            if (b.H, getattr(b, 'Hv', b.H), b.nh, b.F, b.T) != (64, 64, 2, 256, torch.float32) or not b.causal or b.lora or b.train_dense:
                return False
            pfe = b.ad1 is None and b.ad2 is not None and b.pl2 == 'pfeiffer' and b.lnn2 is not None
            ser = b.ad1 is not None and b.ad2 is not None and b.pl1 == 'serial' and b.pl2 == 'serial' and b.lnn1 is None and b.lnn2 is None
            if not (pfe or ser):
                return False
            ads = (b.ad2,) if pfe else (b.ad1, b.ad2)
            if any(a.d > 32 or a.dp != 64 or a.act != b.ad2.act or a.kind != b.ad2.kind or a.d != b.ad2.d or a.virtual is not None and pfe for a in ads):
                return False
            if any(f is not None for ln in (b.ln1, b.ln2) for f in (ln.g_gamma, ln.g_beta)):
                return False
        return True

    def _sas_desc(self, b, seed, with_grads):
        gg = lambda f: f() if f is not None else None
        a0 = b.ad1 if b.ad1 is not None else b.ad2
        d = dict(wqkv=b.wqkv, wfc=b.wo, w1=b.wi, b1=b.bi, w2=b.wo2, b2=b.bo2, ln1_g=b.ln1.gamma, ln1_b=b.ln1.beta, ln2_g=b.ln2.gamma, ln2_b=b.ln2.beta,
                 E=64, n_heads=2, F=256, d=a0.d, ldwu=a0.dp, ldg_d=64, ldg_u=64, act=a0.act, inner_res=int(a0.kind == 'houlsby'), mode=0,
                 eps=float(b.ln1.eps), mask_neg=float(b.mask_neg), drop_attn=float(b.p_attn), drop_hidden=float(b.p_hidden),
                 drop_site=int(b.site), drop_seed=int(seed))
        pfe = b.ad1 is None
        if pfe:
            d.update(mode=1, ln3_g=b.lnn2.gamma, ln3_b=b.lnn2.beta, g_ln3_g=gg(b.lnn2.g_gamma) if with_grads else None,
                     g_ln3_b=gg(b.lnn2.g_beta) if with_grads else None, inner_res=0, d=b.ad2.d, ldwu=b.ad2.dp, act=b.ad2.act)
        for k, ad in (('1', b.ad2 if pfe else b.ad1), ('2', b.ad2)):
            d.update({'wd' + k: ad.wd, 'bd' + k: ad.bd, 'wu' + k: ad.wu, 'bu' + k: ad.bu})
            trains = with_grads and (ad.virtual is not None or ad.g_wu is not None) and not (pfe and k == '1')
            wg = with_grads and not (pfe and k == '1')
            d.update({'g_wd' + k: ad.s_wd if trains else None, 'g_wu' + k: ad.s_wu if trains else None,
                      'g_bd' + k: (ad.s_bd if ad.s_bd is not None else gg(ad.g_bd)) if (wg and ad.g_bd is not None) else None,
                      'g_bu' + k: gg(ad.g_bu) if wg else None})
        return d

    def _make_block(self, tb, Hv, nh, S, dt, causal, mask_neg, p_drop, site):
        mha, ff = tb.multi_head_attention, tb.feed_forward
        H = pad_to(Hv, 64)
        Fv = ff.w_1.out_features
        F = pad_to(Fv, 64)
        dh = Hv // nh
        long = S > 32
        wide = dh in (128, 256) and dt == torch.float32 and not long
        wide_long = long and dh == 128 and dt == torch.float32 and S <= 128
        if dh not in (32, 64) and not wide and not wide_long and not (0 < dh <= 16 and not long) or S > 256 or (long and H != Hv):
            raise NotImplementedError(f'transformer block geometry width={Hv} heads={nh} S={S}')
        b = _Block()
        b.long = long
        for lin in (mha.w_Q, mha.w_K, mha.w_V):
            if type(lin).__name__ not in ('LoRALinear', 'Linear'):
                raise NotImplementedError(f'projection module {type(lin).__name__}')
        b.lora = _Lora.for_block((mha.w_Q, mha.w_K, mha.w_V), Hv, self, dt)
        if b.lora and H != Hv:
            raise NotImplementedError('LoRA on a zero-padded block')
        b.H, b.Hv, b.F, b.nh, b.dh, b.S = H, Hv, F, nh, dh, S
        b.causal, b.mask_neg, b.scale = causal, mask_neg, 1.0 / math.sqrt(dh)
        b.ffn_act = L.ACT_RELU
        b.p_hidden, b.p_attn, b.site = p_drop, p_drop, site
        b.wqkv = torch.zeros(3 * H, H, dtype=dt, device=self.dev)
        b.wqkvT = torch.zeros(H, 3 * H, dtype=dt, device=self.dev)
        b.bqkv = torch.zeros(3 * H, dtype=torch.float32, device=self.dev) if b.lora else None
        self._pack_lora_bias(b, H)
        b.qkv = tuple(None if type(lin).__name__ == 'LoRALinear' else
                      _Dense(self, lin.weight, None, dt, b.wqkv[sl * H:(sl + 1) * H], b.wqkvT[:, sl * H:(sl + 1) * H])
                      for sl, lin in enumerate((mha.w_Q, mha.w_K, mha.w_V)))
        b.d_o = _Dense(self, mha.fc.weight, None, dt, pad=(H, H))
        b.d_i = _Dense(self, ff.w_1.weight, ff.w_1.bias, dt, pad=(F, H))
        b.d_o2 = _Dense(self, ff.w_2.weight, ff.w_2.bias, dt, pad=(H, F))
        b.wo, b.woT, b.bo = b.d_o.w, b.d_o.wT, None
        b.wi, b.wiT, b.bi = b.d_i.w, b.d_i.wT, b.d_i.b
        b.wo2, b.wo2T, b.bo2 = b.d_o2.w, b.d_o2.wT, b.d_o2.b
        b.train_dense = any(d is not None and d.trainable for d in b.qkv + (b.d_o, b.d_i, b.d_o2))
        b.ln1, b.ln2 = _LN(mha.layer_norm, self), _LN(ff.layer_norm, self)
        b.ad1 = b.ad2 = b.lnn1 = b.lnn2 = None
        b.pl1 = b.pl2 = None
        b.need_dx = True
        b.T = dt
        return b

    def _pack_lora_bias(self, b, H):
        for lo in b.lora:
            if lo.mod.bias is not None:
                self.add_pack_bias(lo.mod.bias, b.bqkv[lo.slot * H:(lo.slot + 1) * H])

    def _make_kadapter(self, mod, width, S, dt, site):
        k = _KAdapter()
        d = mod.down_project.out_features
        dp = pad_to(d, 64)
        k.width, k.d, k.dp, k.T = width, d, dp, dt
        k.down = _Dense(self, mod.down_project.weight, mod.down_project.bias, dt, pad=(dp, width))
        k.up = _Dense(self, mod.up_project.weight, mod.up_project.bias, dt, pad=(width, dp))
        p_drop = float(mod.transformer_blocks[0].multi_head_attention.dropout.p)
        k.blocks = [self._make_block(tb, d, mod.num_head, S, dt, False, 0.0, p_drop, site + 16 * j)
                    for j, tb in enumerate(mod.transformer_blocks)]
        k.tag = f'kad{site}'
        return k

    def _kad_forward(self, k, fus, n_seq, M, train, seed, out, saved):
        T, dp = k.T, k.dp
        dn = self._buf(k.tag + '.dn', M, dp, T)
        L.gemm_nt(fus, k.down.w, dn, bias=k.down.b, M=M)
        x = dn
        for j, blk in enumerate(k.blocks):
            bufs = saved['blk'][j] if saved is not None else self._block_bufs(k.tag + f'.b{j}.shared', blk, M, True)
            nxt = (saved['bo'] if (saved is not None and j == len(k.blocks) - 1) else self._buf(k.tag + f'.o{j}', M, dp, T))
            self._block_forward(blk, x, None, n_seq, M, bufs, train, seed, nxt)
            x = nxt
        L.gemm_nt(x, k.up.w, out, bias=k.up.b, R1=fus, M=M)

    def _kad_bufs(self, k, M):
        return dict(blk=[self._block_bufs(k.tag + f'.b{j}', blk, M, False) for j, blk in enumerate(k.blocks)],
                    bo=self._buf(k.tag + '.bo', M, k.dp, k.T), fus=self._buf(k.tag + '.fus', M, k.width, k.T))

    def _kad_backward(self, k, d_out, n_seq, M, train, seed, d_fus, saved):
        T, dp = k.T, k.dp
        self._dense_wgrad(k.up, d_out, saved['bo'], M)
        dx = self._buf(k.tag + '.dbo', M, dp, T)
        L.gemm_nt(d_out, k.up.wT, dx, M=M)
        for j in range(len(k.blocks) - 1, -1, -1):
            dprev = self._buf(k.tag + f'.dx{j}', M, dp, T)
            self._block_backward(k.blocks[j], dx, None, n_seq, M, saved['blk'][j], train, seed, dprev)
            dx = dprev
        self._dense_wgrad(k.down, dx, saved['fus'], M)
        L.gemm_nt(dx, k.down.wT, d_fus, R1=d_out, M=M)

    def _buf(self, name, rows, cols, dt):
        key = (name, cols, dt)
        t = self._bufs.get(key)
        if t is None or t.shape[0] < rows:
            t = torch.zeros(rows, cols, dtype=dt, device=self.dev)
            self._bufs[key] = t
        return t[:rows]

    def _buf_tail0(self, name, rows, cols, dt, real):
        t = self._buf(name, rows, cols, dt)
        key = (name, cols, dt)
        hw = self._dirty.get(key, 0)
        if hw > real:
            full = self._bufs[key]
            full[real:min(hw, full.shape[0])].zero_()
        self._dirty[key] = real
        return t

    def _q8(self, blk):
        if blk.d_i is not None and (blk.d_i.trainable or blk.d_o2.trainable):
            return False
        return self.q8_deriv and blk.T == torch.bfloat16 and getattr(blk, 'ffn_act', L.ACT_GELU) == L.ACT_GELU and blk.F % 16 == 0

    def _vskip(self, blk, which):
        ad, pl, ln = (blk.ad1, blk.pl1, blk.ln1) if which == '1' else (blk.ad2, blk.pl2, blk.ln2)
        if ad is None or pl != 'serial' or hasattr(blk, 'lnA') or blk.T != torch.bfloat16:
            return False
        if not (getattr(blk, 'Hv', blk.H) == blk.H and blk.H in (128, 256, 512, 768) and ad.dp == 64):
            return False
        if ln.g_gamma is not None or ln.g_beta is not None:
            return False
        key = '_vskip_ok' + which
        if not hasattr(blk, key):
            g, b = ln.gamma.detach().float(), ln.beta.detach().float()
            setattr(blk, key, bool(float(g.abs().min()) > 1e-3 and float((b / g).abs().max()) < 8.0))
        return getattr(blk, key)

    def _q8t(self, blk, M):
        return self._q8(blk) and M % 256 == 0 and blk.F % 256 == 0

    def _block_bufs(self, tag, blk, M, shared, Mc=None):
        pre = tag if not shared else tag.split('.')[0] + '.shared'
        T, H, F = blk.T, blk.H, blk.F
        d = {}
        d['qkv'] = self._buf(pre + '.qkv', M, 3 * H, T)
        if getattr(blk, 'long', False):
            d['lse'] = self._buf(pre + '.lse', (M // blk.S + 1) * blk.nh * blk.S, 1, torch.float32)
            if not shared:
                d['ctx_o'] = self._buf(pre + '.ctx_o', M, H, T)
        if Mc is not None:
            pre, M = pre + '.cls', Mc
        if (blk.lora or blk.pl1 == 'parallel' or blk.train_dense) and not shared:
            d['xin'] = self._buf(pre + '.xin', d['qkv'].shape[0], H, T)
        if (blk.pl2 == 'parallel' or blk.train_dense) and not shared:
            d['x1s'] = self._buf(pre + '.x1s', M, H, T)
        if blk.train_dense and not shared:
            d['ctx_s'] = self._buf(pre + '.ctx_s', M, H, T)
            d['u_s'] = self._buf(pre + '.u_s', M, F, T)
        keep_y = not shared and Mc is None
        d['h1'] = self._buf(pre + '.h1', M, H, T)
        d['y1' if keep_y and self._vskip(blk, '1') else 'v1'] = self._buf(pre + '.v1', M, H, T)
        d['st1'] = self._buf(pre + '.st1', M, 2, torch.float32)
        d['upre'] = self._buf(pre + '.upre', M, F, torch.uint8 if self._q8(blk) else T)
        d['h2'] = self._buf(pre + '.h2', M, H, T)
        d['y2' if keep_y and self._vskip(blk, '2') else 'v2'] = self._buf(pre + '.v2', M, H, T)
        d['st2'] = self._buf(pre + '.st2', M, 2, torch.float32)
        for k, ad, pl in (('1', blk.ad1, blk.pl1), ('2', blk.ad2, blk.pl2)):
            if ad is not None:
                d['zp' + k] = self._buf(pre + '.zp' + k, M, ad.dp, T)
                d['z' + k] = self._buf(pre + '.z' + k, M, ad.dp, T)
                if pl == 'pfeiffer':
                    d['t' + k] = self._buf(pre + '.t' + k, M, H, T)
                    d['va' + k] = self._buf(pre + '.va' + k, M, H, T)
                    d['sta' + k] = self._buf(pre + '.sta' + k, M, 2, torch.float32)
        return d

    @staticmethod
    def _vc(blk, t):
        hv = getattr(blk, 'Hv', blk.H)
        return t if hv == t.shape[1] else t[:, :hv]

    def _sub_forward(self, blk, which, dense_in, w, bias, resid, ln, ad, pl, lnn, bufs, M, p_drop, site, seed, out, scales=None, out8=None):
        h, v, st = bufs['h' + which], bufs.get('v' + which), bufs['st' + which]
        self._twin.pop(out.data_ptr(), None)
        assert v is not None or out.data_ptr() == bufs['y' + which].data_ptr()
        sk = dict(scale_a=scales[0], scale_b=scales[1]) if scales is not None else {}
        y8, ys = out8 if out8 is not None else (None, None)
        if not (ad is not None and pl not in ('pfeiffer', 'parallel') and self._fuse(blk, ad, h)):
            if out8 is not None:
                self._sub_forward(blk, which, dense_in, w, bias, resid, ln, ad, pl, lnn, bufs, M, p_drop, site, seed, out, scales=scales)
                L.quant_rows_fp8(out, y8, ys, M=M)
                return
        r32mode = self.res32 and blk.T == torch.bfloat16 and getattr(blk, 'Hv', blk.H) == blk.H and v is not None and v.shape[1] == blk.H
        if ad is None:
            if r32mode:
                hd = self._buf('res32.h', M, blk.H, blk.T)
                L.gemm_nt(dense_in, w, hd, bias=bias, drop_p=p_drop, drop_site=site, drop_seed=seed, M=M, **sk)
                y32 = self._buf('res32.' + which, M, blk.H, torch.float32)
                L.ln_fwd_sum(hd, resid, ln.gamma, ln.beta, ln.eps, out, st, M=M, res32=self._twin_of(resid, M), sum_out=v, y32=y32)
                self._twin[out.data_ptr()] = y32
                return
            L.gemm_nt(dense_in, w, v, bias=bias, R1=resid, drop_p=p_drop, drop_site=site, drop_seed=seed, drop_first=True, M=M, **sk)
            L.ln_fwd(self._vc(blk, v), ln.gamma, ln.beta, ln.eps, self._vc(blk, out), st, M=M)
            return
        zp, z = bufs['zp' + which], bufs['z' + which]
        if pl == 'pfeiffer':
            va, t, sta = bufs['va' + which], bufs['t' + which], bufs['sta' + which]
            if r32mode and self._fuse(blk, ad, t):
                hd = self._buf('res32.h', M, blk.H, blk.T)
                va32 = self._buf('res32.va', M, blk.H, torch.float32)
                L.gemm_nt(dense_in, w, hd, bias=bias, drop_p=p_drop, drop_site=site, drop_seed=seed, M=M, **sk)
                L.ln_fwd_sum(hd, resid, ln.gamma, ln.beta, ln.eps, t, sta, M=M, res32=self._twin_of(resid, M), sum_out=va, sum32=va32)
                y32 = self._buf('res32.' + which, M, blk.H, torch.float32)
                L.adapter_ln_fwd(t, va, None, ad.wd, ad.bd, ad.wu, ad.bu, lnn.gamma, lnn.beta, lnn.eps, ad.act, zp, z, v, out, st, M=M, res32=va32, y32=y32, frag=ad.frag_f)
                self._twin[out.data_ptr()] = y32
                return
            L.gemm_nt(dense_in, w, va, bias=bias, R1=resid, drop_p=p_drop, drop_site=site, drop_seed=seed, drop_first=True, M=M, **sk)
            L.ln_fwd(va, ln.gamma, ln.beta, ln.eps, t, sta, M=M)
            if self._fuse(blk, ad, t):
                L.adapter_ln_fwd(t, va, None, ad.wd, ad.bd, ad.wu, ad.bu, lnn.gamma, lnn.beta, lnn.eps, ad.act, zp, z, v, out, st, M=M, frag=ad.frag_f)
                return
            L.gemm_nt(t, ad.wd, z, bias=ad.bd, C2=zp, act=ad.act, M=M)
            L.gemm_nt(z, ad.wu, v, bias=ad.bu, R1=va, M=M)
            L.ln_fwd(v, lnn.gamma, lnn.beta, lnn.eps, out, st, M=M)
            return
        if pl == 'parallel':
            L.gemm_nt(dense_in, w, h, bias=bias, R1=resid, drop_p=p_drop, drop_site=site, drop_seed=seed, drop_first=True, M=M, **sk)
            L.gemm_nt(resid, ad.wd, z, bias=ad.bd, C2=zp, act=ad.act, M=M)
            L.gemm_nt(z, ad.wu, v, bias=ad.bu, R1=h, R2=resid, M=M)
            L.ln_fwd(v, ln.gamma, ln.beta, ln.eps, out, st, M=M)
            return
        L.gemm_nt(dense_in, w, h, bias=bias, drop_p=p_drop, drop_site=site, drop_seed=seed, M=M, **sk)
        comp = ad.kind == 'compacter'
        if self._fuse(blk, ad, h):
            r32 = y32 = None
            if (self.res32 or self.res24) and blk.T == torch.bfloat16:
                r32 = self._twin_of(resid, M)
                y32 = self._buf(('res8.' if self.res24 else 'res32.') + which, M, blk.H // self.lo_div if self.res24 else blk.H, torch.int8 if self.res24 else torch.float32)
            L.adapter_ln_fwd(h, resid if comp else h, None if comp else resid, ad.wd, ad.bd, ad.wu, ad.bu, ln.gamma, ln.beta, ln.eps, ad.act,
                             zp, z, v, out, st, M=M, y8=y8, ys=ys, **(dict(res32=r32, y32=y32) if y32 is not None else {}), frag=ad.frag_f)
            if y32 is not None:
                self._twin[out.data_ptr()] = y32
            return
        L.gemm_nt(h, ad.wd, z, bias=ad.bd, C2=zp, act=ad.act, M=M)
        if comp:
            L.gemm_nt(z, ad.wu, v, bias=ad.bu, R1=resid, M=M)
        else:
            L.gemm_nt(z, ad.wu, v, bias=ad.bu, R1=h, R2=resid, M=M)
        L.ln_fwd(v, ln.gamma, ln.beta, ln.eps, out, st, M=M)

    _pk = None

    def _off(self, blk):
        return self._pk['off'] if (self._pk is not None and getattr(blk, 'is_item', False)) else None

    def _cls_gather(self, src, dst, n_items, S, blk=None):
        if self._pk is not None and (blk is None or getattr(blk, 'is_item', False)):
            L.rows_idx_copy(src, dst, self._pk['off'], n_items)
        else:
            L.gather_rows(src, dst, n_items, S)

    def _cls_scatter_fill(self, src, dst, n_items, S, M, blk=None):
        if self._pk is not None and (blk is None or getattr(blk, 'is_item', False)):
            L.zero(dst[:M])
            L.rows_idx_copy(src, dst, self._pk['off'], n_items, scatter=True)
        else:
            L.scatter_rows_fill(src, dst, n_items, S, M)

    def _twin_of(self, t, M):
        w = self._twin.get(t.data_ptr())
        return w if (w is not None and w.shape[0] >= M and w.shape[1] == (t.shape[1] // self.lo_div if w.dtype == torch.int8 else t.shape[1])) else None

    def _fuse_bwd(self, blk, ad, t):
        return self._fuse(blk, ad, t) and blk.H != 1024

    def _fuse(self, blk, ad, t):
        return getattr(blk, 'Hv', blk.H) == blk.H and L.adapter_ln_ok(t, ad.dp)

    LAYER_CALL = _os.environ.get('A4R_LAYER_CALL', '1') != '0'
    _LAYER_DBG = _os.environ.get('A4R_LAYER_CALL', '1')

    def _layer_ok(self, blk, bufs, cls_rows, backward):
        if not (self.LAYER_CALL and hasattr(L, 'encoder_layer_fwd') and blk.T == torch.bfloat16 and not self.fp8 and not self.res32):
            return False
        if (self._LAYER_DBG == '2' and backward) or (self._LAYER_DBG == '3' and not backward):
            return False
        if cls_rows is not None or getattr(blk, 'long', False) or blk.lora or blk.train_dense or hasattr(blk, 'lnA') or getattr(blk, 'Hv', blk.H) != blk.H:
            return False
        if any(k in bufs for k in ('xin', 'x1s', 'ctx_s', 'u_s')) or blk.ffn_act != L.ACT_GELU or blk.S > 32 or blk.H not in (128, 256, 512, 768):
            return False
        if any(d is not None and d.trainable for d in blk.qkv):
            return False
        for ad, pl, ln in ((blk.ad1, blk.pl1, blk.ln1), (blk.ad2, blk.pl2, blk.ln2)):
            if ad is None or pl != 'serial' or ad.kind == 'compacter' or ad.virtual is not None or ad.dp != 64:
                return False
            if ln.g_gamma is not None or ln.g_beta is not None:
                return False
            if backward and ad.g_wu is not None and (WGRAD_STREAM or ad.s_wu is not None or ad.s_bd is not None or ad.g_bu is None or ad.g_bd is None):
                return False
        return True

    def _layer_desc(self, blk, bufs, M):
        key = (id(blk), id(bufs), M)
        cache = self.__dict__.setdefault('_layer_descs', {})
        hit = cache.get(key)
        if hit is not None and hit['bufs'] is bufs:
            return hit
        if len(cache) >= 256:
            cache.clear()
        T, H, F = blk.T, blk.H, blk.F
        d = L.EncoderLayer()
        d.M, d.H, d.F, d.S, d.n_heads, d.dh, d.causal = M, H, F, blk.S, blk.nh, blk.dh, int(blk.causal)
        d.scale, d.mask_neg, d.ln_eps = blk.scale, blk.mask_neg, blk.ln1.eps
        p = lambda t: None if t is None else t.data_ptr()
        d.wqkv, d.wqkvT, d.wo, d.woT, d.wi, d.wiT, d.wo2, d.wo2T = (p(t) for t in (blk.wqkv, blk.wqkvT, blk.wo, blk.woT, blk.wi, blk.wiT, blk.wo2, blk.wo2T))
        d.bqkv, d.bo, d.bi, d.bo2 = p(blk.bqkv), p(blk.bo), p(blk.bi), p(blk.bo2)
        d.ln1_g, d.ln1_b, d.ln2_g, d.ln2_b = p(blk.ln1.gamma), p(blk.ln1.beta), p(blk.ln2.gamma), p(blk.ln2.beta)
        keep = []
        for i, ad in enumerate((blk.ad1, blk.ad2)):
            a = d.ad[i]
            a.wd, a.wu, a.wdT, a.wuT, a.bd, a.bu, a.act = p(ad.wd), p(ad.wu), p(ad.wdT), p(ad.wuT), p(ad.bd), p(ad.bu), ad.act
            if ad.frag_f is not None:
                a.wd_f, a.wu_f, a.wuT_f, a.wdT_f = p(ad.frag_f[0]), p(ad.frag_f[1]), p(ad.frag_b[0]), p(ad.frag_b[1])
        x1 = bufs['y1'] if 'y1' in bufs else self._buf('x1', M, H, T)
        ws = dict(ctx=self._buf('ctx', M, H, T), u=self._buf('u', M, F, T), x1=x1)
        d.qkv, d.ctx, d.h1, d.v1, d.zp1, d.z1 = p(bufs['qkv']), p(ws['ctx']), p(bufs['h1']), p(bufs.get('v1')), p(bufs['zp1']), p(bufs['z1'])
        d.u, d.upre, d.h2, d.v2, d.zp2, d.z2 = p(ws['u']), p(bufs['upre']), p(bufs['h2']), p(bufs.get('v2')), p(bufs['zp2']), p(bufs['z2'])
        d.st1, d.st2 = p(bufs['st1']), p(bufs['st2'])
        d.upre_q8, d.q8_tiled = int(self._q8(blk)), int(self._q8t(blk, M))
        hit = dict(d=d, x1=x1, keep=keep, ws=ws, bufs=bufs)
        cache[key] = hit
        return hit

    def _layer_forward(self, blk, x, key_mask, n_items, M, bufs, train, seed, x_out):
        e = self._layer_desc(blk, bufs, M)
        d, x1 = e['d'], e['x1']
        d.n_items, d.p_attn, d.p_hidden = n_items, (blk.p_attn if train else 0.0), (blk.p_hidden if train else 0.0)
        d.drop_site, d.drop_seed = blk.site, seed
        d.key_mask = None if key_mask is None else key_mask.data_ptr()
        off = self._off(blk)
        d.offsets = None if off is None else off.data_ptr()
        x_lo = self._twin_of(x, M) if self.res24 else None
        x1_lo = self._buf('res8.1', M, blk.H // self.lo_div, torch.int8) if self.res24 else None
        xo_lo = self._buf('res8.2', M, blk.H // self.lo_div, torch.int8) if self.res24 else None
        d.x_lo, d.x1_lo, d.xout_lo = (None if t is None else t.data_ptr() for t in (x_lo, x1_lo, xo_lo))
        d.lo_nibble = 1 if (self.res24 and self.lo_div == 2) else 0
        self._twin.pop(x1.data_ptr(), None)
        self._twin.pop(x_out.data_ptr(), None)
        if 'y2' in bufs:
            assert x_out.data_ptr() == bufs['y2'].data_ptr()
        L.encoder_layer_fwd(d, x, x1, x_out)
        if self.res24:
            self._twin[x1.data_ptr()], self._twin[x_out.data_ptr()] = x1_lo, xo_lo

    def _layer_backward(self, blk, dx_out, key_mask, n_items, M, bufs, train, seed, dx_in):
        e = self._layer_desc(blk, bufs, M)
        d, T, H, F = e['d'], blk.T, blk.H, blk.F
        d.n_items, d.p_attn, d.p_hidden = n_items, (blk.p_attn if train else 0.0), (blk.p_hidden if train else 0.0)
        d.drop_site, d.drop_seed = blk.site, seed
        d.key_mask = None if key_mask is None else key_mask.data_ptr()
        off = self._off(blk)
        d.offsets = None if off is None else off.data_ptr()
        self._wgrad_join()
        for i, ad in enumerate((blk.ad1, blk.ad2)):
            a = d.ad[i]
            if ad.g_wu is not None:
                gw, gd, gbu, gbd = ad.g_wu(), ad.g_wd(), ad.g_bu(), ad.g_bd()
                a.g_wu, a.g_wd, a.g_bu, a.g_bd, a.ldg_wu, a.ldg_wd = gw.data_ptr(), gd.data_ptr(), gbu.data_ptr(), gbd.data_ptr(), gw.stride(0), gd.stride(0)
            else:
                a.g_wu = a.g_wd = a.g_bu = a.g_bd = None
        n_tok = self._pk['Mtok'] if off is not None else n_items * blk.S
        sc = dict(dv1=self._buf('dv1', M, H, T), dv2=self._buf('dv2', M, H, T), dzp=self._buf('dzp', M, 64, T), d_h=self._buf('dh2', M, H, T),
                  du=self._buf('du', M, F, T), dx1=self._buf('dx1', M, H, T), dctx=self._buf('dctx', M, H, T))
        for k, t in sc.items():
            setattr(d, k, t.data_ptr())
        d.dqkv = self._buf_tail0('dqkv', M, 3 * H, T, n_tok).data_ptr() if dx_in is not None else self._buf('dqkv', M, 3 * H, T).data_ptr()
        x_out = bufs['y2'] if 'y2' in bufs else bufs['v2']
        L.encoder_layer_bwd(d, e['x1'], x_out, dx_out, dx_in)

    def _block_forward(self, blk, x, key_mask, n_items, M, bufs, train, seed, x_out, cls_rows=None, x8=None, want8=False):
        T, H = blk.T, blk.H
        if x8 is None and not want8 and self._layer_ok(blk, bufs, cls_rows, False):
            self._layer_forward(blk, x, key_mask, n_items, M, bufs, train, seed, x_out)
            return None
        pa = blk.p_attn if train else 0.0
        ph = blk.p_hidden if train else 0.0
        f8 = self.fp8 and T == torch.bfloat16 and M % 256 == 0 and getattr(blk, 'wqkv8', None) is not None
        if f8:
            if x8 is None:
                x8 = (self._buf('x8', M, H, torch.uint8), self._buf('x8s', M, 1, torch.float32))
                L.quant_rows_fp8(x, x8[0], x8[1], M=M)
            L.gemm_nt(x8[0], blk.wqkv8, bufs['qkv'], bias=blk.bqkv, M=M, scale_a=x8[1], scale_b=blk.wqkv8s)
        else:
            L.gemm_nt(x, blk.wqkv, bufs['qkv'], bias=blk.bqkv, M=M)
        if 'xin' in bufs and x.data_ptr() != bufs['xin'].data_ptr():
            L.gather_rows(x, bufs['xin'], M, 1)
        if getattr(blk, 'long', False):
            ctx = bufs['ctx_o'] if 'ctx_o' in bufs else self._buf('ctx', M, H, T)
            L.attn_long_fwd(bufs['qkv'], ctx, bufs['lse'], n_items, blk.S, blk.nh, blk.dh, 0, H, 2 * H, blk.scale,
                            drop_p=pa, drop_site=blk.site, drop_seed=seed, key_mask=key_mask, causal=blk.causal)
        else:
            ctx = bufs['ctx_s'] if ('ctx_s' in bufs and cls_rows is None) else self._buf('ctx', M, H, T)
            L.attn_fwd(bufs['qkv'], ctx, key_mask, n_items, blk.S, blk.nh, blk.dh, 0, H, 2 * H, blk.causal, blk.scale, blk.mask_neg,
                       drop_p=pa, drop_site=blk.site, drop_seed=seed, offsets=self._off(blk))
        if cls_rows is not None:
            ctx_c, x_c = self._buf('ctx_c', cls_rows, H, T), self._buf('x_c', cls_rows, H, T)
            self._cls_gather(ctx, ctx_c, n_items, blk.S, blk)
            self._cls_gather(x, x_c, n_items, blk.S, blk)
            x32 = self._twin_of(x, M) if (self.res32 or self.res24) else None
            if x32 is not None:
                if x32.dtype == torch.int8:
                    x_c32 = self._buf('x_c8', cls_rows, x32.shape[1], torch.int8)
                    self._cls_gather(x32.view(torch.bfloat16), x_c32.view(torch.bfloat16), n_items, blk.S, blk)
                else:
                    x_c32 = self._buf('x_c32', cls_rows, H, torch.float32)
                    self._cls_gather(x32, x_c32, n_items, blk.S, blk)
                self._twin[x_c.data_ptr()] = x_c32
            ctx, x, M = ctx_c, x_c, cls_rows
        if 'ctx_s' in bufs and ctx is not bufs['ctx_s']:
            L.gather_rows(ctx, bufs['ctx_s'], M, 1)
        x1 = self._buf('x1', M, H, T)
        x1 = bufs['x1s'] if 'x1s' in bufs else x1
        if 'y1' in bufs:
            if 'x1s' in bufs:
                raise RuntimeError('y1 and x1s are the same tensor: one of them should not have been allocated')
            x1 = bufs['y1']
        f8 = self.fp8 and T == torch.bfloat16 and M % 256 == 0
        f8_o = f8 and getattr(blk, 'wo8', None) is not None and 'ctx_s' not in bufs
        f8_up = f8 and getattr(blk, 'wi8', None) is not None and blk.ffn_act == L.ACT_GELU
        f8_ffn = f8_up and getattr(blk, 'wo28', None) is not None and 'u_s' not in bufs and self._q8(blk)
        x1_8 = (self._buf('x1_8', M, H, torch.uint8), self._buf('x1_8s', M, 1, torch.float32)) if f8_up else None
        if f8_o:
            c8, cs = self._buf('ctx8', M, H, torch.uint8), self._buf('ctx8s', M, 1, torch.float32)
            L.quant_rows_fp8(ctx, c8, cs, M=M)
            self._sub_forward(blk, '1', c8, blk.wo8, blk.bo, x, blk.ln1, blk.ad1, blk.pl1, blk.lnn1, bufs, M, ph, blk.site + 1, seed, x1,
                              scales=(cs, blk.wo8s), out8=x1_8)
        else:
            self._sub_forward(blk, '1', ctx, blk.wo, blk.bo, x, blk.ln1, blk.ad1, blk.pl1, blk.lnn1, bufs, M, ph, blk.site + 1, seed, x1, out8=x1_8)
        out8 = (self._buf('x8', M, H, torch.uint8), self._buf('x8s', M, 1, torch.float32)) if (want8 and f8) else None
        if f8_ffn:
            u = self._buf('u8', M, blk.F, torch.uint8)
            L.gemm_nt(x1_8[0], blk.wi8, u, bias=blk.bi, C2=bufs['upre'], act=L.ACT_GELU, c2_deriv='q8', M=M, scale_a=x1_8[1], scale_b=blk.wi8s,
                      c_fp8=1, c_scale=self.FP8_U_SCALE, q8_tiled=self._q8t(blk, M))
            self._sub_forward(blk, '2', u, blk.wo28, blk.bo2, x1, blk.ln2, blk.ad2, blk.pl2, blk.lnn2, bufs, M, ph, blk.site + 2, seed, x_out,
                              scales=(self._const_rows('su', M, self.FP8_U_SCALE), blk.wo28s), out8=out8)
            return out8
        u = bufs['u_s'] if 'u_s' in bufs else self._buf('u', M, blk.F, T)
        if f8_up:
            L.gemm_nt(x1_8[0], blk.wi8, u, bias=blk.bi, C2=bufs['upre'], act=L.ACT_GELU, c2_deriv='q8' if self._q8(blk) else True, M=M,
                      scale_a=x1_8[1], scale_b=blk.wi8s, q8_tiled=self._q8t(blk, M))
        else:
            L.gemm_nt(x1, blk.wi, u, bias=blk.bi, C2=bufs['upre'], act=blk.ffn_act, c2_deriv='q8' if self._q8(blk) else True, M=M,
                      q8_tiled=self._q8t(blk, M))
        self._sub_forward(blk, '2', u, blk.wo2, blk.bo2, x1, blk.ln2, blk.ad2, blk.pl2, blk.lnn2, bufs, M, ph, blk.site + 2, seed, x_out, out8=out8)
        return out8

    def _sub_backward(self, blk, which, dy, ln, ad, pl, lnn, bufs, M, p_drop, site, seed):
        T, H = blk.T, blk.H
        v, st = bufs.get('v' + which), bufs['st' + which]
        beta_y = None
        if v is None:
            v, beta_y = bufs['y' + which], ln.beta
        gg = lambda f: f() if f is not None else None
        self._wgrad_join()
        if ad is None:
            dv = self._buf('dv' + which, M, H, T)
            if p_drop > 0 and getattr(blk, 'Hv', H) == H:
                dh = self._buf('dh' + which, M, H, T)
                L.ln_bwd(dy, v, st, ln.gamma, dv, M=M, dgamma=gg(ln.g_gamma), dbeta=gg(ln.g_beta),
                         dv2=dh, drop2_p=p_drop, drop2_site=site, drop2_seed=seed)
                return dh, dv
            L.ln_bwd(self._vc(blk, dy), self._vc(blk, v), st, ln.gamma, self._vc(blk, dv), M=M, dgamma=gg(ln.g_gamma), dbeta=gg(ln.g_beta))
            if p_drop > 0:
                dh = self._buf('dh' + which, M, H, T)
                L.dropout_apply(dv, dh, p_drop, site, seed, M=M)
                return dh, dv
            return dv, dv
        zp, z = bufs['zp' + which], bufs['z' + which]
        dzp = self._buf('dzp', M, ad.dp, T)
        dv = self._buf('dv' + which, M, H, T)
        dh = self._buf('dh' + which, M, H, T)
        if pl == 'pfeiffer':
            va, t, sta = bufs['va' + which], bufs['t' + which], bufs['sta' + which]
            dt = self._buf('dt', M, H, T)
            fused_bd = False
            b2 = False
            if self._fuse_bwd(blk, ad, dy):
                b2 = self._tn2_bias_ok(ad, dv, M)
                L.adapter_ln_bwd(dy, v, st, lnn.gamma, None, zp, ad.act, ad.wuT, ad.wdT, False, dv, dzp, dt,
                                 dgamma=gg(lnn.g_gamma), dbeta=gg(lnn.g_beta), dbias=None if b2 else gg(ad.g_bu), M=M, dbd=None if b2 else self._bd_target(ad), frag=ad.frag_b)
                fused_bd = self._bd_target(ad) is not None
            else:
                L.ln_bwd(dy, v, st, lnn.gamma, dv, M=M, dgamma=gg(lnn.g_gamma), dbeta=gg(lnn.g_beta), dbias=gg(ad.g_bu))
                L.gemm_nt(dv, ad.wuT, dzp, Pre=zp, dact=ad.act, M=M)
                L.gemm_nt(dzp, ad.wdT, dt, M=M)
            self._adapter_wgrads(ad, dv, z, dzp, t, M, bd_done=fused_bd, bias_in_tn2=b2)
            dva = self._buf('dva', M, H, T)
            if p_drop > 0:
                L.ln_bwd(dt, va, sta, ln.gamma, dva, M=M, dgamma=gg(ln.g_gamma), dbeta=gg(ln.g_beta), dres=dv,
                         dv2=dh, drop2_p=p_drop, drop2_site=site, drop2_seed=seed)
                return dh, dva
            L.ln_bwd(dt, va, sta, ln.gamma, dva, M=M, dgamma=gg(ln.g_gamma), dbeta=gg(ln.g_beta), dres=dv)
            return dva, dva
        h = bufs['h' + which]
        if pl != 'parallel' and self._fuse_bwd(blk, ad, dy):
            b2 = self._tn2_bias_ok(ad, dv, M)
            L.adapter_ln_bwd(dy, v, st, ln.gamma, None, zp, ad.act, ad.wuT, ad.wdT, ad.kind != 'compacter', dv, dzp, dh,
                             dgamma=gg(ln.g_gamma), dbeta=gg(ln.g_beta), dbias=None if b2 else gg(ad.g_bu), M=M,
                             drop_p=p_drop, drop_site=site, drop_seed=seed, dbd=None if b2 else self._bd_target(ad), beta_y=beta_y, frag=ad.frag_b)
            self._adapter_wgrads(ad, dv, z, dzp, h, M, bd_done=self._bd_target(ad) is not None, bias_in_tn2=b2)
            return dh, dv
        assert beta_y is None, 'a sub-layer that keeps y instead of v runs the fused backward only'
        L.ln_bwd(dy, v, st, ln.gamma, dv, M=M, dgamma=gg(ln.g_gamma), dbeta=gg(ln.g_beta), dbias=gg(ad.g_bu))
        L.gemm_nt(dv, ad.wuT, dzp, Pre=zp, dact=ad.act, M=M)
        if pl == 'parallel':
            sub_in = bufs['xin'] if which == '1' else bufs['x1s']
            dres = self._buf('dres' + which, M, H, T)
            L.gemm_nt(dzp, ad.wdT, dres, R1=dv, R2=dv, M=M)
            self._adapter_wgrads(ad, dv, z, dzp, sub_in, M)
            if p_drop > 0:
                L.dropout_apply(dv, dh, p_drop, site, seed, M=M)
                return dh, dres
            return dv, dres
        if ad.kind == 'compacter':
            L.gemm_nt(dzp, ad.wdT, dh, drop_p=p_drop, drop_site=site, drop_seed=seed, M=M)
        else:
            L.gemm_nt(dzp, ad.wdT, dh, R1=dv, drop_p=p_drop, drop_site=site, drop_seed=seed, M=M)
        self._adapter_wgrads(ad, dv, z, dzp, h, M)
        return dh, dv

    LORA_FUSED = _os.environ.get('A4R_LORA_FUSED', '1') != '0'

    def _lora_backward_all(self, blk, dqkv, x, M):
        sh = blk.lora[0].share if blk.lora else None
        if sh is None or any(lo.share is not sh for lo in blk.lora):
            for lo in blk.lora:
                self._lora_backward(blk, lo, dqkv, x, M)
            return
        H, T = blk.H, blk.T
        a, b = blk.lora
        dqa, dqb = dqkv[:, a.slot * H:(a.slot + 1) * H], dqkv[:, b.slot * H:(b.slot + 1) * H]
        if self.LORA_FUSED and a.r <= 15 and b.r <= 15 and L.lora_bwd_fused_ok(x, M, H):
            oc, R = _Lora.ONES_COL, (8 if a.r <= 8 and b.r <= 8 else 16)
            L.lora_bwd_fused(x, dqa, dqb, sh['A'][a.off:a.off + R], sh['A'][b.off:b.off + R], a.BT[a.off:a.off + R], b.BT[b.off:b.off + R],
                             a.scaling, b.scaling, sh['s_A'][a.off:a.off + R], sh['s_A'][b.off:b.off + R],
                             a.s_B[:, a.off:a.off + R], b.s_B[:, b.off:b.off + R],
                             a.s_B[:, oc] if a.g_bias is not None else None, b.s_B[:, oc] if b.g_bias is not None else None, M, rank_rows=R)
            return
        t = self._buf('lora_t', M, 64, T)
        dt = self._buf('lora_dt', M, 64, T)
        L.gemm_nt(x, sh['A'], t, bias=sh['ones'], M=M)
        L.gemm_nt(dqa, a.BT, dt, alpha=a.scaling, M=M)
        L.gemm_nt(dqb, b.BT, dt, alpha=b.scaling, R1=dt, M=M)
        if T == torch.bfloat16 and M % 64 == 0:
            L.gemm_tn2(dqa, t, a.s_B, dqb, t, b.s_B, M=M)
        else:
            L.gemm_tn(dqa, t, a.s_B, M=M)
            L.gemm_tn(dqb, t, b.s_B, M=M)
        L.gemm_tn(dt, x, sh['s_A'], M=M)

    def _lora_backward(self, blk, lo, dqkv, x, M):
        H, T = blk.H, blk.T
        dq = dqkv[:, lo.slot * H:(lo.slot + 1) * H]
        if lo.g_bias is not None:
            L.colsum(dq, lo.g_bias(), M=M)
        if lo.r == 0:
            if lo.g_W is not None:
                L.gemm_tn(dq, x, lo.g_W(), M=M)
            return
        t = self._buf('lora_t', M, lo.rp, T)
        dt = self._buf('lora_dt', M, lo.rp, T)
        L.gemm_nt(x, lo.A, t, M=M)
        L.gemm_nt(dq, lo.BT, dt, alpha=lo.scaling, M=M)
        L.gemm_tn(dq, t, lo.s_B, M=M)
        L.gemm_tn(dt, x, lo.s_A, M=M)

    WGRAD_SIDE_OK = True

    def _wgrad_join(self):
        if self._wdone is not None:
            torch.cuda.current_stream().wait_event(self._wdone)
            self._wdone = None

    def _bd_target(self, ad):
        if ad.g_bd is None:
            return None
        return ad.s_bd if ad.s_bd is not None else ad.g_bd()

    def _tn2_bias_ok(self, ad, dv, M):
        return (not (WGRAD_STREAM and self.WGRAD_SIDE_OK) and dv.dtype == torch.bfloat16 and M % 64 == 0
                and (ad.virtual is not None or ad.g_wu is not None) and ad.s_bd is None and ad.g_bu is not None and ad.g_bd is not None
                and ad.dp == 64 and dv.shape[1] % 64 == 0)

    def _adapter_wgrads(self, ad, dv, z, dzp, down_in, M, bd_done=False, bias_in_tn2=False):
        if ad.virtual is None and ad.g_wu is None:
            return
        if WGRAD_STREAM and self.WGRAD_SIDE_OK and ad.s_wu is None and ad.virtual is None and torch.device(self.dev).type == 'cuda':
            if self._wstream is None:
                self._wstream = torch.cuda.Stream(device=self.dev)
                self._wev = [torch.cuda.Event(), torch.cuda.Event()]
            ev = self._wev[0]
            ev.record()
            with torch.cuda.stream(self._wstream):
                self._wstream.wait_event(ev)
                if dv.dtype == torch.bfloat16:
                    L.gemm_tn2(dv, z, ad.g_wu(), dzp, down_in, ad.g_wd(), M=M)
                else:
                    L.gemm_tn(dv, z, ad.g_wu(), M=M)
                    L.gemm_tn(dzp, down_in, ad.g_wd(), M=M)
                if ad.g_bd is not None and ad.s_bd is None and not bd_done:
                    L.colsum(dzp, ad.g_bd(), M=M)
                self._wev[1].record()
            self._wdone = self._wev[1]
            self._wev.reverse()
            if ad.g_bd is not None and ad.s_bd is not None and not bd_done:
                L.colsum(dzp, ad.s_bd, M=M)
            return
        t_wu, t_wd = (ad.s_wu if ad.s_wu is not None else ad.g_wu()), (ad.s_wd if ad.s_wd is not None else ad.g_wd())
        if bias_in_tn2:
            assert dv.shape[1] * z.shape[1] == dzp.shape[1] * down_in.shape[1]
            L.gemm_tn2(dv, z, t_wu, dzp, down_in, t_wd, M=M, xsum1=ad.g_bu(), xsum2=ad.g_bd())
            return
        if dv.dtype == torch.bfloat16 and dv.shape[1] * z.shape[1] == dzp.shape[1] * down_in.shape[1] and M % 64 == 0:
            L.gemm_tn2(dv, z, t_wu, dzp, down_in, t_wd, M=M)
        else:
            L.gemm_tn(dv, z, t_wu, M=M)
            L.gemm_tn(dzp, down_in, t_wd, M=M)
        if ad.g_bd is not None and not bd_done:
            L.colsum(dzp, ad.s_bd if ad.s_bd is not None else ad.g_bd(), M=M)

    def _block_backward(self, blk, dx_out, key_mask, n_items, M, bufs, train, seed, dx_in, cls_rows=None):
        T, H, F = blk.T, blk.H, blk.F
        if self._layer_ok(blk, bufs, cls_rows, True):
            self._layer_backward(blk, dx_out, key_mask, n_items, M, bufs, train, seed, dx_in)
            return
        pa = blk.p_attn if train else 0.0
        ph = blk.p_hidden if train else 0.0
        M_full = M
        if cls_rows is not None:
            M = cls_rows
        dh2, dres2 = self._sub_backward(blk, '2', dx_out, blk.ln2, blk.ad2, blk.pl2, blk.lnn2, bufs, M, ph, blk.site + 2, seed)
        self._dense_wgrad(blk.d_o2, dh2, bufs.get('u_s'), M)
        dx1 = self._buf('dx1', M, H, T)
        if (self.fp8 and getattr(blk, 'wo2T8', None) is not None and T == torch.bfloat16 and M % 256 == 0 and bufs['upre'].dtype == torch.uint8
                and 'u_s' not in bufs):
            do8, dos = self._buf('do8', M, H, torch.uint8), self._buf('do8s', M, 1, torch.float32)
            L.quant_rows_fp8(dh2, do8, dos, M=M)
            du8, dus = self._buf('du8', M, F, torch.uint8), self._buf('du8s', M, 1, torch.float32)
            L.gemm_nt(do8, blk.wo2T8, du8, Pre=bufs['upre'], dact=L.DACT_MUL_Q8, M=M, scale_a=dos, scale_b=blk.wo2T8s,
                      c_fp8=2, c_scale=blk.c_du, c_scale_out=dus, q8_tiled=self._q8t(blk, M))
            L.gemm_nt(du8, blk.wiT8, dx1, R1=dres2, M=M, scale_a=dus, scale_b=blk.wiT8s)
        else:
            du = self._buf('du', M, F, T)
            L.gemm_nt(dh2, blk.wo2T, du, Pre=bufs['upre'], dact=L.DACT_MUL_Q8 if self._q8(blk) else L.DACT_MUL, M=M, q8_tiled=self._q8t(blk, M))
            self._dense_wgrad(blk.d_i, du, bufs.get('x1s'), M)
            L.gemm_nt(du, blk.wiT, dx1, R1=dres2, M=M)
        dh1, dres1 = self._sub_backward(blk, '1', dx1, blk.ln1, blk.ad1, blk.pl1, blk.lnn1, bufs, M, ph, blk.site + 1, seed)
        qkv_train = any(d is not None and d.trainable for d in blk.qkv)
        pend = []
        if qkv_train and cls_rows is None:
            pend = [(blk.d_o, dh1, bufs.get('ctx_s'))]
        else:
            self._dense_wgrad(blk.d_o, dh1, bufs.get('ctx_s'), M)
        if dx_in is None and not blk.lora and not qkv_train:
            return
        dctx = self._buf('dctx_c' if cls_rows is not None else 'dctx', M, H, T)
        L.gemm_nt(dh1, blk.woT, dctx, M=M)
        if cls_rows is not None:
            M = M_full
            full = self._buf('dctx', M, H, T)
            self._cls_scatter_fill(dctx, full, n_items, blk.S, M, blk)
            dctx = full
            rfull = self._buf('dres_full', M, H, T)
            self._cls_scatter_fill(dres1, rfull, n_items, blk.S, M, blk)
            dres1 = rfull
        n_tok = self._pk['Mtok'] if self._off(blk) is not None else n_items * blk.S
        dqkv = self._buf_tail0('dqkv', M, 3 * H, T, n_tok)
        if getattr(blk, 'long', False):
            ws = self._buf('attn_ws', bufs['lse'].shape[0], 1, torch.float32)
            L.attn_long_bwd(bufs['qkv'], bufs['ctx_o'], dctx, dqkv, bufs['lse'], ws, n_items, blk.S, blk.nh, blk.dh, 0, H, 2 * H, blk.scale,
                            drop_p=pa, drop_site=blk.site, drop_seed=seed, key_mask=key_mask, causal=blk.causal)
        else:
            L.attn_bwd(bufs['qkv'], dctx, dqkv, key_mask, n_items, blk.S, blk.nh, blk.dh, 0, H, 2 * H, blk.causal, blk.scale, blk.mask_neg,
                       drop_p=pa, drop_site=blk.site, drop_seed=seed, offsets=self._off(blk))
        if blk.lora:
            self._lora_backward_all(blk, dqkv, bufs['xin'], M)
        self._dense_wgrads([(d, dqkv[:, sl * H:(sl + 1) * H], bufs.get('xin')) for sl, d in enumerate(blk.qkv)] + pend, M)
        if dx_in is not None:
            L.gemm_nt(dqkv, blk.wqkvT, dx_in, R1=dres1, M=M)

    def _dense_wgrads(self, items, M):
        live = [(d, dy, x) for d, dy, x in items if d is not None and d.trainable]
        if len(live) < 2 or len(live) > 4 or any(d.g_w is None for d, _, _ in live):
            for d, dy, x in live:
                self._dense_wgrad(d, dy, x, M)
            return
        L.gemm_tn_multi([(dy, x, d.s_w if d.s_w is not None else d.g_w().view(d.out_f, d.in_f),
                          None if d.g_b is None else (d.s_b if d.s_b is not None else d.g_b())) for d, dy, x in live], M=M)

    def _dense_wgrad(self, d, dy, x, M):
        if d is None or not d.trainable:
            return
        if d.g_w is not None and d.g_b is not None:
            L.gemm_tn_bias(dy, x, d.s_w if d.s_w is not None else d.g_w().view(d.out_f, d.in_f),
                           d.s_b if d.s_b is not None else d.g_b(), M=M)
            return
        if d.g_w is not None:
            L.gemm_tn(dy, x, d.s_w if d.s_w is not None else d.g_w().view(d.out_f, d.in_f), M=M)
        if d.g_b is not None:
            L.colsum(dy, d.s_b if d.s_b is not None else d.g_b(), M=M)

    def _kad_chain_forward(self, x_last, n_items, M, Ip, train, seed, cls, keep):
        H, T, nb = self.H, self.T, len(self.bert_blocks)
        if keep and (getattr(self, '_kad_saved_b', None) is None or self._kad_saved_M != M):
            self._kad_saved_b = [self._kad_bufs(k, M) for k in self.bert_kads]
            self._kad_saved_M = M
        last = None
        for j, (kk, kad) in enumerate(zip(self.bert_klist, self.bert_kads)):
            sv = self._kad_saved_b[j] if keep else None
            fus = sv['fus'] if sv is not None else self._buf(kad.tag + '.fus', M, H, T)
            fus.copy_(x_last if kk == nb else self._buf(f'khs{kk}', M, H, T))
            if last is not None:
                fus.add_(last)
            out = self._buf(kad.tag + '.out', M, H, T)
            self._kad_forward(kad, fus, n_items, M, train, seed, out, sv)
            last = out
        cat = self._buf('kcat', Ip, 2 * H, T)
        L.gather_rows(x_last, cat[:, :H], n_items, self.S)
        L.gather_rows(last, cat[:, H:], n_items, self.S)
        L.gemm_nt(cat, self.d_com.w, cls, bias=self.d_com.b, M=Ip)

    def _kad_chain_backward(self, dcls, n_items, M, Ip, train, seed, dxb):
        H, T, S = self.H, self.T, self.S
        self._dense_wgrad(self.d_com, dcls, self._buf('kcat', Ip, 2 * H, T), Ip)
        dcat = self._buf('dkcat', Ip, 2 * H, T)
        L.gemm_nt(dcls, self.d_com.wT, dcat, M=Ip)
        dxb.zero_()
        L.scatter_rows(dcat[:, :H], dxb, n_items, S)
        dlast = self._buf('kd_last', M, H, T)
        dlast.zero_()
        L.scatter_rows(dcat[:, H:], dlast, n_items, S)
        d_hs = {}
        for j in range(len(self.bert_kads) - 1, -1, -1):
            kad, kk = self.bert_kads[j], self.bert_klist[j]
            d_fus = self._buf(kad.tag + '.dfus', M, H, T)
            self._kad_backward(kad, dlast, n_items, M, train, seed, d_fus, self._kad_saved_b[j])
            d_hs[kk] = d_fus if kk not in d_hs else d_hs[kk].add_(d_fus)
            dlast = d_fus
        return d_hs

    def _encode(self, news, n_items, train, seed, saved):
        S, H = self.S, self.H
        pk = self._pk
        M = pad_to(pk['Mtok'], 256) if pk is not None else pad_to(n_items * S, 256)
        self._twin.clear()
        key_mask = self._buf('kmask', n_items, S, torch.float32)
        x = self._buf('xa', M, H, self.T)
        direct_xin = lambda j: (saved is not None and j < len(self.bert_blocks) and 'xin' in saved[j] and 'y2' not in saved[j]
                                and tuple(saved[j]['xin'].shape) == (M, H))
        if direct_xin(0):
            x = saved[0]['xin']
        keep = self.train_emb and saved is not None
        word = self.emb_word
        if self.prompt_n:
            n, V = self.prompt_n, self.prompt_V
            word = self.emb_word_ext
            word[V:V + n].copy_(self.prompt_param.detach())
            news = news.clone()
            red = torch.arange(V, V + n, device=news.device).expand(news.shape[0], n)
            if self.roberta:
                red = torch.where(news[:, :n] == self.pad_id, -red - 1, red)
            news[:, :n] = red
        x_emb = self._buf('x_unpacked', pad_to(n_items * S, 256), H, self.T) if pk is not None else x
        L.embed_ln(news, word, self.emb_pos, self.emb_type0, self.emb_ln.gamma, self.emb_ln.beta, self.emb_ln.eps,
                   x_emb, n_items, S, roberta=self.roberta, pad_id=self.pad_id,
                   drop_p=self.p_hidden if train else 0.0, drop_site=999, drop_seed=seed,
                   pre_out=self._buf('emb_pre', M, H, self.T) if keep else None,
                   stats_out=self._buf('emb_st', M, 2, torch.float32) if keep else None, key_mask_out=key_mask)
        if pk is not None:
            L.rows_idx_copy(x_emb, x, pk['map'], pk['Mtok'])
            if M > pk['Mtok']:
                L.zero(x[pk['Mtok']:M])
            key_mask = None
        self._news = news
        other = self._buf('xb', M, H, self.T)
        xa_buf = self._buf('xa', M, H, self.T)
        Ip = pad_to(n_items, 128)
        cls = self._buf('cls', Ip, H, self.T)
        last = len(self.bert_blocks) - 1
        x8 = None
        for i, blk in enumerate(self.bert_blocks):
            cmode = self.cls_only and i == last
            bufs = saved[i] if saved is not None else self._block_bufs('bert.shared', blk, M, True, Mc=Ip if cmode else None)
            w8 = self.fp8 and i != last
            if cmode:
                self._block_forward(blk, x, key_mask, n_items, M, bufs, train, seed, cls, cls_rows=Ip, x8=x8)
            elif 'y2' in bufs:
                x8 = self._block_forward(blk, x, key_mask, n_items, M, bufs, train, seed, bufs['y2'], x8=x8, want8=w8)
                x = bufs['y2']
            else:
                out = other if x.data_ptr() != other.data_ptr() else xa_buf
                if direct_xin(i + 1) and not (self.fp8 and i != last):
                    out = saved[i + 1]['xin']
                x8 = self._block_forward(blk, x, key_mask, n_items, M, bufs, train, seed, out, x8=x8, want8=w8)
                x = out
            if not cmode:
                if (i + 1) in self.bert_klist and i != last:
                    self._buf(f'khs{i + 1}', M, H, self.T).copy_(x)
        if self.bert_kads:
            self._kad_chain_forward(x, n_items, M, Ip, train, seed, cls, saved is not None)
        elif not self.cls_only:
            self._cls_gather(x, cls, n_items, S)
        emb = self._buf('emb', Ip, self.E, torch.float32)
        pre = self._buf('embpre', Ip, self.E, torch.float32)
        L.gemm_nt(cls, self.fc_w, emb, bias=self.fc_b, C2=pre, act=L.ACT_GELU, M=Ip)
        return emb, pre, key_mask, M

    def _user_forward(self, xin, log_mask, B, train, seed, saved):
        E, Tn = self.E, self.Lseq - 1
        Mu = pad_to(B * Tn, 128)
        x = self._buf('sx_a', Mu, E, torch.float32)
        st0 = self._buf('sst0', Mu, 2, torch.float32)
        L.ln_fwd(xin, self.sas_ln0.gamma, self.sas_ln0.beta, self.sas_ln0.eps, x, st0, M=Mu, add=self.pos_emb[:Tn],
                 drop_p=self.p_sas if train else 0.0, drop_site=4000, drop_seed=seed)
        if self._sas_fused_ok():
            xs = [x] + [self._buf(f'sas.fused{j}', Mu, E, torch.float32) for j in range(len(self.sas_blocks))]
            for j, blk in enumerate(self.sas_blocks):
                L.sasrec_block(self._sas_desc(blk, seed, False), xs[j], log_mask, xs[j + 1], B, Tn, train)
            self._sas_xs = xs
            return xs[-1], Mu
        other = self._buf('sx_b', Mu, E, torch.float32)
        keep = saved is not None
        if self.sas_kads and keep and (getattr(self, '_kad_saved_s', None) is None or self._kad_saved_Mu != Mu):
            self._kad_saved_s = [self._kad_bufs(k, Mu) for k in self.sas_kads]
            self._kad_saved_Mu = Mu
        last = None
        for j, blk in enumerate(self.sas_blocks):
            if self.sas_kads:
                kad = self.sas_kads[j]
                sv = self._kad_saved_s[j] if keep else None
                fus = sv['fus'] if sv is not None else self._buf(kad.tag + '.fus', Mu, E, torch.float32)
                fus.copy_(x)
                if last is not None:
                    fus.add_(last)
                out = self._buf(kad.tag + '.out', Mu, E, torch.float32)
                self._kad_forward(kad, fus, B, Mu, train, seed, out, sv)
                last = out
            bufs = saved[j] if saved is not None else self._block_bufs('sas.shared', blk, Mu, True)
            self._block_forward(blk, x, log_mask, B, Mu, bufs, train, seed, other)
            x, other = other, x
        if self.sas_kads:
            cat = self._buf('skcat', Mu, 2 * E, torch.float32)
            cat[:, :E].copy_(x)
            cat[:, E:].copy_(last)
            y = self._buf('sk_y', Mu, E, torch.float32)
            L.gemm_nt(cat, self.d_com2.w, y, bias=self.d_com2.b, M=Mu)
            x = y
        return x, Mu

    def _pre_forward(self, n_items):
        """torch-side preparation of a step that must sit BEFORE its first kernel (image tower: the ViT-MAE masking order)."""

    def _stack_attrs(self, news, n):
        S = self.S0
        out = torch.zeros(self.n_attr * n, 2 * S, dtype=torch.int64, device=news.device)
        if self.roberta:
            out[:, :S] = self.pad_id
        for k, (st, nw) in enumerate(self.attrs):
            out[k * n:(k + 1) * n, :nw] = news[:n, st:st + nw]
            out[k * n:(k + 1) * n, S:S + nw] = news[:n, st + nw:st + 2 * nw]
        return out

    _ADD_DESC_BYTES = 32

    def _attr_table(self, key, src, dst_off_rows, n, into_rows):
        cache = self.__dict__.setdefault('_attr_tabs', {})
        k = (key, src.data_ptr(), n)
        if k not in cache:
            if len(cache) >= 64:
                cache.clear()
            E, a = self.E, 1.0 / self.n_attr
            ents = [L.AddDesc(src.data_ptr() + (0 if into_rows else j * n * E * 4), (j * n * E if into_rows else 0), n, E, E, a) for j in range(self.n_attr)]
            cache[k] = L.desc_table(ents, self.dev)
        return cache[k]

    def _attr_mean(self, emb_all, n):
        emb = self._buf('emb_mean', pad_to(n, 128), self.E, torch.float32)
        L.zero(emb)
        tab = self._attr_table('fwd', emb_all, 0, n, False)
        for j in range(self.n_attr):
            L.unpack_add(emb, tab[j * self._ADD_DESC_BYTES:], 1, n * self.E)
        return emb

    def _attr_spread(self, d_emb, n):
        Ip = pad_to(self.n_attr * n, 128)
        d_all = self._buf('d_emb_attr', Ip, self.E, torch.float32)
        L.zero(d_all)
        L.unpack_add(d_all, self._attr_table('bwd', d_emb, 0, n, True), self.n_attr, n * self.E)
        return d_all, Ip

    @torch.no_grad()
    def encode_items(self, news):
        L.require_gpu(news)
        self._set_S(self.S0)
        self._pk = None
        n = news.shape[0]
        news = news.contiguous()
        if news.dtype != torch.int64:
            news = news.long()
        self.pack_trainables()
        if self.n_attr > 1:
            emb, _, _, _ = self._encode(self._stack_attrs(news, n), self.n_attr * n, False, 0, None)
            return self._attr_mean(emb, n)[:n].clone()
        emb, _, _, _ = self._encode(news, n, False, 0, None)
        return emb[:n].clone()

    @torch.no_grad()
    def user_encode(self, input_embs, log_mask):
        L.require_gpu(input_embs, log_mask)
        B, Tn, E = input_embs.shape
        assert Tn == self.Lseq - 1 and E == self.E
        Mu = pad_to(B * Tn, 128)
        xin = self._buf('sxin', Mu, E, torch.float32)
        xin[:B * Tn].copy_(input_embs.reshape(B * Tn, E).float())
        lm = log_mask.float().contiguous()
        self.pack_trainables()
        out, _ = self._user_forward(xin, lm, B, False, 0, None)
        return out[:B * Tn].view(B, Tn, E).clone()


    def _kept_rows(self, B):
        mode = _skip_unused_items()
        if mode == '0' or self.Lseq < 3:
            return None
        if self.arch == 'cpc':
            return B * (self.Lseq + 1)
        n_c = B * (2 * self.Lseq - 1)
        if mode == '2':
            return n_c
        ncu = 256
        if torch.device(self.dev).type == 'cuda':
            ncu = torch.cuda.get_device_properties(self.dev).multi_processor_count
        ntn = max(1, self.H // 256)
        rounds = lambda n: -(-(pad_to(n * self.S, 256) // 256 * ntn) // ncu)
        return n_c if rounds(n_c) < rounds(B * 2 * self.Lseq) else None

    host_log_mask = None
    host_lens = None
    host_max_tokens = None

    def _set_S(self, S):
        if S != self.S and type(self) is TransRecEngine:
            self.S = S
            for b in self.bert_blocks:
                b.S = S

    def _kept_index(self, hm, B):
        import numpy as np
        lm = (hm.detach().reshape(B, self.Lseq - 1).numpy() != 0)
        Ls, T = self.Lseq, self.Lseq - 1
        pos = np.zeros((B, Ls), bool)
        neg = np.zeros((B, Ls), bool)
        pos[:, :T] |= lm
        if self.arch == 'cpc':
            pos[:, Ls - 1] = True
            neg[:, T - 1] = True
        else:
            pos[:, 1:] |= lm
            neg[:, :T] = lm
        if self.sas_kads:
# ... 359 lines not shown
```

include/a4r.h:

```cpp
#ifndef A4R_H
#define A4R_H
#include <stddef.h>
#include <stdint.h>
#ifdef __cplusplus
extern "C" {
#endif

#define A4R_BF16 0
#define A4R_F32 1
#define A4R_FP8 2
#define A4R_ACT_NONE 0
#define A4R_ACT_RELU 1
#define A4R_ACT_GELU 2
#define A4R_ACT_GELU_TANH 3
#define A4R_ACT_LEAKY 4
#define A4R_DACT_MUL 15
#define A4R_DACT_MUL_Q8 14

#ifndef A4R_OK
#define A4R_OK 0
#define A4R_EINVAL (-1)
#define A4R_ELAUNCH (-2)
#endif

#define A4R_ABI_VERSION 411
int a4r_version(void);

typedef struct {
    const void* A; const void* B; void* C;
    const float* bias; void* C2; const void* R1; const void* R2; const void* Pre;
    int32_t M, N, K;
    int32_t lda, ldb, ldc, ldc2, ldr1, ldr2, ldpre;
    int32_t in_dtype, out_dtype;
    int32_t act, dact;
    int32_t drop_first;
    int32_t c2_mode;
    float alpha;
    float drop_p; uint32_t drop_site; uint64_t drop_seed;
    int64_t drop_row0;
    const float* scale_a; const float* scale_b;
    int32_t c_fp8; float c_scale; float* c_scale_out;
    int32_t q8_tiled;
} a4r_gemm_t;
int a4r_gemm_nt(void* stream, const a4r_gemm_t* g);
int a4r_gemm_tail_plan(int M, int N, int* p_full, int* kp);
int a4r_gemm_tail_max(int k);
int a4r_gemm_rows_256(int M, int N);
int a4r_gemm_variant(int v);

int a4r_gemm_tn(void* stream, const void* X, int ldx, const void* Y, int ldy, float* C, int ldc,
                int M, int P, int Q, int dtype);
int a4r_gemm_tn_bias(void* stream, const void* X, int ldx, const void* Y, int ldy, float* C, int ldc,
                     int M, int P, int Q, int dtype, float* xsum);
typedef struct a4r_tn_prob_t {
    const void* X; const void* Y; float* C; float* xsum;
    int32_t ldx, ldy, ldc, P, Q, pad_;
} a4r_tn_prob_t;
int a4r_gemm_tn_multi(void* stream, const a4r_tn_prob_t* probs, int n, int M, int dtype);
typedef struct {
    const float *wqkv, *wfc, *w1, *b1, *w2, *b2;
    const float *ln1_g, *ln1_b, *ln2_g, *ln2_b;
    const float *wd1, *bd1, *wu1, *bu1, *wd2, *bd2, *wu2, *bu2;
    float *g_wd1, *g_bd1, *g_wu1, *g_bu1, *g_wd2, *g_bd2, *g_wu2, *g_bu2;
    int32_t E, n_heads, F, d, ldwu, ldg_d, ldg_u, act, inner_res;
    float eps, mask_neg, drop_attn, drop_hidden;
    uint32_t drop_site; uint64_t drop_seed;
    int32_t mode; const float *ln3_g, *ln3_b; float *g_ln3_g, *g_ln3_b;
} a4r_sasrec_block_t;
int a4r_sasrec_block_fwd(void* stream, const a4r_sasrec_block_t* b, const float* x, const float* log_mask, float* y, int n_users, int T, int train);
int a4r_sasrec_block_bwd(void* stream, const a4r_sasrec_block_t* b, const float* x, const float* log_mask, const float* dy, float* dx,
                         int n_users, int T, int train);

int a4r_gemm_tn2(void* stream, const void* X1, int ldx1, const void* Y1, int ldy1, float* C1, int ldc1, int P1, int Q1,
                 const void* X2, int ldx2, const void* Y2, int ldy2, float* C2, int ldc2, int P2, int Q2, int M, int dtype,
                 float* xsum1, float* xsum2);

int a4r_colsum(void* stream, const void* X, int ldx, float* out, int M, int N, int dtype);

int a4r_adapter_ln_fwd(void* stream, const void* A, int lda, const void* R1, int ldr1, const void* R2, int ldr2,
                       const void* Wd, const float* bd, const void* Wu, const float* bu,
                       const float* gamma, const float* beta, float eps, int act,
                       void* zp, void* z, void* v, int ldv, void* y, int ldy, float* stats, int M, int H, int d, int dtype,
                       void* y8, int ld8, float* ys,
                       const float* res32, int ldres32, float* y32, int ldy32,
                       int w_frag);
int a4r_adapter_ln_bwd(void* stream, const void* dy, int lddy, const void* v, int ldv, const float* stats, const float* gamma,
                       const void* dres, int lddres, const void* zp, int act, const void* WuT, const void* WdT, int inner_res,
                       void* dv, int lddv, void* dzp, void* dh, int lddh, float* dgamma, float* dbeta, float* dbias,
                       int M, int H, int d, int dtype, float drop_p, uint32_t drop_site, uint64_t drop_seed, float* dbd, int flags,
                       const float* beta_y);

typedef struct {
    const void* qkv; int32_t ld; int32_t q_off, k_off, v_off;
    void* out; int32_t ldo;
    const void* dout; void* dqkv;
    const float* key_mask;
    int32_t n_items, S, n_heads, dh, causal, dtype;
    float scale, mask_neg;
    float drop_p; uint32_t drop_site; uint64_t drop_seed;
    const int32_t* offsets;
} a4r_attn_t;
int a4r_attn_fwd(void* stream, const a4r_attn_t* a);
int a4r_attn_bwd(void* stream, const a4r_attn_t* a);

int a4r_attn_long_fwd(void* stream, const a4r_attn_t* a, float* lse);
int a4r_attn_long_bwd(void* stream, const a4r_attn_t* a, const float* lse, float* delta_ws);

int a4r_patchify(void* stream, const void* img, int src_kind, void* out, int ldo, const int32_t* keep_idx, int n_keep,
                 int n_items, int C, int Himg, int Wimg, int patch, int dtype);
int a4r_vit_assemble(void* stream, const void* patches, int ldp, const float* cls, const float* pos, const int32_t* keep_idx,
                     void* out, int ldo, int n_items, int n_keep, int H, int dtype, int tokens_out);

int a4r_mae_keep_indices(void* stream, const float* noise, int32_t* keep, int n_items, int n_patches, int n_keep, uint64_t seed,
                         uint32_t site);

int a4r_resample_u8(void* stream, const void* src, void* dst, const int32_t* bounds, const int32_t* kk, int ksize,
                    long n_outer, int in_len, int out_len, long inner);

int a4r_embed_ln(void* stream, const int64_t* ids, int ld_ids, const float* word, const float* pos,
                 const float* type0, const float* gamma, const float* beta, float eps,
                 void* out, int ldo, int n_items, int S, int H, int roberta, int pad_id, int dtype,
                 float drop_p, uint32_t drop_site, uint64_t drop_seed, void* pre_out, float* stats_out, float* key_mask_out);
int a4r_embed_bwd(void* stream, const int64_t* ids, int ld_ids, const void* dpre, int ldd, float* dword, float* dpos,
                  int n_items, int S, int H, int roberta, int pad_id, int dtype);

int a4r_ln_fwd(void* stream, const void* v, int ldv, const float* add, int add_rows,
               const float* gamma, const float* beta, float eps,
               void* y, int ldy, float* stats, int M, int H, int dtype,
               float drop_p, uint32_t drop_site, uint64_t drop_seed);
int a4r_ln_fwd_sum(void* stream, const void* h, int ldh, const float* res32, int ldres32, const void* res, int ldres,
                   const float* gamma, const float* beta, float eps, void* y, int ldy, void* sum, int ldsum, float* sum32, int ldsum32,
                   float* y32, int ldy32, float* stats, int M, int H, int dtype);
int a4r_ln_fwd_fp8(void* stream, const void* v, int ldv, const float* add, int add_rows,
                   const float* gamma, const float* beta, float eps,
                   void* y, int ldy, void* y8, int ld8, float* yscale, float* stats, int M, int H, int dtype);
int a4r_quant_rows_fp8(void* stream, const void* x, int ldx, void* q, int ldq, float* scale, int M, int H, int dtype);
int a4r_ln_bwd(void* stream, const void* dy, int lddy, const void* v, int ldv, const float* add, int add_rows,
               const float* stats, const float* gamma, const void* dres, int lddres, void* dv, int lddv,
               float* dgamma, float* dbeta, float* dbias, int M, int H, int dtype,
               float drop_p, uint32_t drop_site, uint64_t drop_seed,
               void* dv2, int lddv2, float drop2_p, uint32_t drop2_site, uint64_t drop2_seed);

int a4r_gather_rows(void* stream, const void* in, int ldi, void* out, int ldo, int n, int row_step, int H, int dtype);
int a4r_scatter_rows(void* stream, const void* in, int ldi, void* out, int ldo, int n, int row_step, int H, int dtype);
int a4r_rows_idx_copy(void* stream, const void* in, int64_t ldi_bytes, void* out, int64_t ldo_bytes, const int32_t* idx, int n,
                      int64_t row_bytes, int scatter);
int a4r_scatter_rows_fill(void* stream, const void* in, int ldi, void* out, int ldo, int n, int row_step, int H, int dtype, int fill_rows);

int a4r_dropout_apply(void* stream, const void* x, int ldx, void* y, int ldy, int M, int N, int dtype,
                      float drop_p, uint32_t drop_site, uint64_t drop_seed);

int a4r_act_bwd_f32(void* stream, const float* dy, const float* pre, float* dx, int64_t n, int act);

int a4r_score_bce_fwd(void* stream, const float* emb, const float* prec, const float* log_mask,
                      float* pos, float* neg, float* loss_ws, int B, int L, int E, int cpc);
int a4r_score_bce_bwd(void* stream, const float* emb, const float* prec, const float* log_mask,
                      const float* pos, const float* neg, const float* loss_ws, float loss_scale, const float* loss_scale_dev,
                      float* d_prec, float* d_emb, int B, int L, int E, int cpc);
int a4r_emb_grad_add_inputs(void* stream, const float* d_in, int ldi, float* d_emb, int B, int L, int E);
int a4r_take_inputs(void* stream, const float* emb, float* out, int ldo, int B, int L, int E);

int a4r_adam_step(void* stream, float* p, const float* g, float* m, float* v, int64_t n,
                  const int32_t* seg_end, const int32_t* seg_group, int n_seg,
                  const float* group_lr, int step, float beta1, float beta2, float eps, float grad_scale);

#define A4R_GRAD_NORM_PARTS 1024
int a4r_grad_sumsq(void* stream, const float* g, int64_t n, float grad_scale, double* partials);
int a4r_adamw_step(void* stream, float* p, const float* g, float* m, float* v, int64_t n,
                   const int32_t* seg_end, const int32_t* seg_group, int n_seg,
                   const float* group_lr, int step, float beta1, float beta2, float eps, float grad_scale,
                   const float* group_wd, int decoupled, const double* partials, float max_norm, float* norm_out);

typedef struct {
    int64_t src_off; void* dst; int32_t rows, cols, rows_pad, cols_pad, transpose, dst_ld;
} a4r_pack_desc_t;
int a4r_pack_matrices(void* stream, const float* flat, const a4r_pack_desc_t* desc_dev, int n_desc, int max_elems, int dtype);

typedef struct {
    int64_t rule_off, wl_off, wr_off;
    int64_t out_off;
    const float* G; int32_t ldg;
    int32_t in_f, out_f, n, pad_;
} a4r_phm_desc_t;
typedef struct { const float* src; int64_t dst_off; int32_t rows, cols, ld; float alpha; } a4r_add_desc_t;
int a4r_lora_merge(void* stream, const float* W, const float* A, const float* B, float scaling,
                   void* dst, int ld, void* dstT, int ldT, int out_f, int in_f, int r, int dtype);
typedef struct {
    const float* W; const float* A; const float* B; void* dst; void* dstT;
    float scaling; int32_t ld, ldT, out_f, in_f, r;
} a4r_lora_desc_t;
int a4r_lora_merge_batch(void* stream, const a4r_lora_desc_t* desc_dev, int n_desc, int max_elems, int dtype);
int a4r_lora_bwd_fused(void* stream, const void* x, int ldx, const void* dqa, const void* dqb, int lddq,
                       const void* Aa, const void* Ab, const void* BTa, const void* BTb, int ldw, float scale_a, float scale_b,
                       float* dAa, float* dAb, int lda, float* dBa, float* dBb, int ldb, float* dbias_a, float* dbias_b, int ldbias,
                       int M, int H, int dtype, int rank_rows, float* ws, int64_t ws_floats);
int a4r_lora_bwd_fused_ws_floats(int H);
int a4r_phm_build(void* stream, const float* params, const a4r_phm_desc_t* desc_dev, int n_desc, float* eff);
int a4r_phm_bwd(void* stream, const float* params, const a4r_phm_desc_t* desc_dev, int n_desc, float* grads);
int a4r_unpack_add(void* stream, float* target, const a4r_add_desc_t* desc_dev, int n_desc, int max_elems);
int a4r_memset_zero(void* stream, void* p, int64_t bytes);

#define A4R_EVAL_MAX_HISTORY 264
int a4r_eval_rank(void* stream, const float* prec, const float* item_emb, const int32_t* target,
                  const int32_t* hist_ptr, const int32_t* hist_idx, int32_t* rank, int U, int N1, int E);

#define A4R_TOPK_MAX_K 256
size_t a4r_topk_ws_bytes(int U, int N1, int K);
int a4r_topk_items(void* stream, const float* prec, const float* item_emb, const int32_t* excl_ptr, const int32_t* excl_idx,
                   int32_t* ids, float* scores, void* ws, int U, int N1, int E, int K);

int a4r_id_index(void* stream, const int64_t* ids, int n, int item_num, int32_t* rows, int32_t* slots, int32_t* ptr, int32_t* uniq,
                 int32_t* n_uniq, int32_t* err, int32_t* ws, int64_t ws_ints);
int a4r_id_index_ws_ints(int n, int item_num);
#define A4R_ID_SUM_CHUNK 16
int a4r_id_grad_sum(void* stream, const float* src, int ld_src, const int32_t* slots, const int32_t* ptr, const int32_t* uniq,
                    const int32_t* n_uniq, int n, float* grad, int ldg, int E);

typedef struct {
    const void *wd, *wu, *wdT, *wuT;
    const void *wd_f, *wu_f, *wdT_f, *wuT_f;
    const float *bd, *bu;
    float *g_wu, *g_wd, *g_bu, *g_bd;
    int32_t ldg_wu, ldg_wd, act, pad_;
} a4r_layer_adapter_t;
typedef struct {
    int32_t M, H, F, n_items, S, n_heads, dh, causal;
    float scale, mask_neg, ln_eps, p_attn, p_hidden;
    uint32_t drop_site; uint64_t drop_seed;
    const float* key_mask; const int32_t* offsets;
    const void *wqkv, *wqkvT, *wo, *woT, *wi, *wiT, *wo2, *wo2T;
    const float *bqkv, *bo, *bi, *bo2, *ln1_g, *ln1_b, *ln2_g, *ln2_b;
    a4r_layer_adapter_t ad[2];
    void *qkv, *ctx, *h1, *v1, *zp1, *z1, *u, *upre, *h2, *v2, *zp2, *z2; float *st1, *st2;
    int32_t upre_q8, q8_tiled;
    const void* x_lo; void *x1_lo, *xout_lo;
    void *dv1, *dv2, *dzp, *d_h, *du, *dx1, *dctx, *dqkv;
    int32_t lo_nibble;
} a4r_encoder_layer_t;
int a4r_encoder_layer_fwd(void* stream, const a4r_encoder_layer_t* l, const void* x, void* x1, void* x_out);
int a4r_encoder_layer_bwd(void* stream, const a4r_encoder_layer_t* l, const void* x1, const void* x_out, const void* dx_out, void* dx_in);

#ifdef __cplusplus
}
#endif
#endif
```

Before: 1862.

## Compute attention only for the CLS query in the last BERT layer

When only the CLS output of a block is needed, the Q projection now runs on the gathered CLS rows alone, and new attention fwd/bwd kernels compute a single query row per item against the full keys and values. The backward pass produces dq only for CLS and splits the input-gradient GEMM into a KV part over all rows plus a Q part over the CLS rows. This removes the Q-projection and attention work for the other query rows, at the cost of extra kernel template variants, more small GEMM launches and gather/scatter copies.

```diff
diff --git a/adapter4rec_amd/_lib.py b/adapter4rec_amd/_lib.py
--- a/adapter4rec_amd/_lib.py
+++ b/adapter4rec_amd/_lib.py
@@ -17,7 +17,7 @@
 ACT_BY_NAME = {'none': 0, 'relu': 1, 'RELU': 1, 'gelu': 2, 'GELU': 2, 'gelu_new': 3, 'leaky_relu': 4}
 
 EXPORTS = [
-    'a4r_version', 'a4r_gemm_nt', 'a4r_gemm_tn', 'a4r_gemm_tn_bias', 'a4r_gemm_tn_multi', 'a4r_gemm_tn2', 'a4r_colsum', 'a4r_attn_fwd', 'a4r_attn_bwd', 'a4r_embed_ln',
+    'a4r_version', 'a4r_gemm_nt', 'a4r_gemm_tn', 'a4r_gemm_tn_bias', 'a4r_gemm_tn_multi', 'a4r_gemm_tn2', 'a4r_colsum', 'a4r_attn_fwd', 'a4r_attn_bwd', 'a4r_attn_cls_fwd', 'a4r_attn_cls_bwd', 'a4r_embed_ln',
     'a4r_ln_fwd', 'a4r_ln_bwd', 'a4r_gather_rows', 'a4r_scatter_rows', 'a4r_rows_idx_copy', 'a4r_act_bwd_f32', 'a4r_score_bce_fwd',
     'a4r_score_bce_bwd', 'a4r_emb_grad_add_inputs', 'a4r_take_inputs', 'a4r_adam_step', 'a4r_pack_matrices',
     'a4r_eval_rank', 'a4r_dropout_apply', 'a4r_gemm_variant', 'a4r_gemm_tail_plan', 'a4r_gemm_tail_max', 'a4r_gemm_rows_256', 'a4r_adapter_ln_fwd', 'a4r_adapter_ln_bwd', 'a4r_ln_fwd_fp8', 'a4r_ln_fwd_sum', 'a4r_quant_rows_fp8', 'a4r_lora_merge', 'a4r_lora_merge_batch', 'a4r_lora_bwd_fused', 'a4r_lora_bwd_fused_ws_floats', 'a4r_phm_build', 'a4r_phm_bwd', 'a4r_unpack_add', 'a4r_memset_zero',
@@ -326,6 +326,25 @@
     a = _attn_args(qkv, q_off, k_off, v_off, key_mask, n_items, S, n_heads, dh, causal, scale, mask_neg, drop_p, drop_site, drop_seed, offsets)
     a.dout, a.ldo, a.dqkv = _p(dout), _ld(dout), _p(dqkv)
     _check(lib().a4r_attn_bwd(_stream(), C.byref(a)), 'a4r_attn_bwd')
+
+
+def attn_cls_fwd(qkv, q_cls, out, key_mask, n_items, S, n_heads, dh, k_off, v_off, causal, scale, mask_neg,
+                 drop_p=0.0, drop_site=0, drop_seed=0, offsets=None):
+    require_gpu(qkv, q_cls, out)
+    assert _dt(q_cls) == _dt(qkv) and _dt(out) == _dt(qkv) and q_cls.shape[0] >= n_items and out.shape[0] >= n_items
+    a = _attn_args(qkv, 0, k_off, v_off, key_mask, n_items, S, n_heads, dh, causal, scale, mask_neg, drop_p, drop_site, drop_seed, offsets)
+    a.out, a.ldo = _p(out), _ld(out)
+    _check(lib().a4r_attn_cls_fwd(_stream(), C.byref(a), _p(q_cls), C.c_int(_ld(q_cls))), 'a4r_attn_cls_fwd')
+
+
+def attn_cls_bwd(qkv, q_cls, dout, dqkv, dq_cls, key_mask, n_items, S, n_heads, dh, k_off, v_off, causal, scale, mask_neg,
+                 drop_p=0.0, drop_site=0, drop_seed=0, offsets=None):
+    require_gpu(qkv, q_cls, dout, dqkv, dq_cls)
+    assert _ld(dqkv) == _ld(qkv) and _ld(dq_cls) == _ld(q_cls) and _dt(q_cls) == _dt(qkv) and _dt(dout) == _dt(qkv) and _dt(dq_cls) == _dt(qkv)
+    assert min(q_cls.shape[0], dout.shape[0], dq_cls.shape[0]) >= n_items
+    a = _attn_args(qkv, 0, k_off, v_off, key_mask, n_items, S, n_heads, dh, causal, scale, mask_neg, drop_p, drop_site, drop_seed, offsets)
+    a.dout, a.ldo, a.dqkv = _p(dout), _ld(dout), _p(dqkv)
+    _check(lib().a4r_attn_cls_bwd(_stream(), C.byref(a), _p(q_cls), _p(dq_cls), C.c_int(_ld(q_cls))), 'a4r_attn_cls_bwd')
 
 
 def attn_long_fwd(qkv, out, lse, n_items, S, n_heads, dh, q_off, k_off, v_off, scale, drop_p=0.0, drop_site=0, drop_seed=0, key_mask=None, causal=False):
diff --git a/adapter4rec_amd/csrc/a4r_attn.hip b/adapter4rec_amd/csrc/a4r_attn.hip
--- a/adapter4rec_amd/csrc/a4r_attn.hip
+++ b/adapter4rec_amd/csrc/a4r_attn.hip
@@ -34,8 +34,8 @@
     static constexpr int OSTRIDE = DH * (int)sizeof(T);
 };
 
-template <typename T, int DH>
-A4R_DEV void qk_scores(const T* base, int ld, int q_off, int k_off, int S, int lane, f32x4_t (&sc)[2][2]) {
+template <typename T, int DH, int MT>
+A4R_DEV void qk_scores(const T* qp, int qld, const T* kp, int ld, int S, int lane, f32x4_t (&sc)[2][2]) {
     using C = AttnCfg<T, DH>;
     const int r16 = lane & 15, kg = lane >> 4;
 #pragma unroll
@@ -44,15 +44,15 @@
         for (int nt = 0; nt < 2; ++nt) sc[mt][nt] = f32x4_t{0.f, 0.f, 0.f, 0.f};
 #pragma unroll
     for (int ks = 0; ks < C::KSD; ++ks) {
-        uint4 qa[2], kb[2];
+        uint4 qa[MT], kb[2];
 #pragma unroll
         for (int t = 0; t < 2; ++t) {
             const int row = min(t * 16 + r16, S - 1);
-            qa[t] = ldg16(base + (size_t)row * ld + q_off + (ks * 4 + kg) * C::PER);
-            kb[t] = ldg16(base + (size_t)row * ld + k_off + (ks * 4 + kg) * C::PER);
-        }
-#pragma unroll
-        for (int mt = 0; mt < 2; ++mt)
+            if (t < MT) qa[t] = ldg16(qp + (size_t)row * qld + (ks * 4 + kg) * C::PER);
+            kb[t] = ldg16(kp + (size_t)row * ld + (ks * 4 + kg) * C::PER);
+        }
+#pragma unroll
+        for (int mt = 0; mt < MT; ++mt)
 #pragma unroll
             for (int nt = 0; nt < 2; ++nt) Mma<T>::mma(qa[mt], kb[nt], sc[mt][nt]);
     }
@@ -75,13 +75,14 @@
     p[1] = e1 * inv;
 }
 
-template <typename T, int DH, int WAVES>
+template <typename T, int DH, int WAVES, bool CQ>
 __global__ void __launch_bounds__(WAVES * 64) attn_fwd_kernel(const T* __restrict__ qkv, int ld, int q_off, int k_off, int v_off,
                                                               T* __restrict__ out, int ldo, const float* __restrict__ key_mask,
                                                               int n_items, int S_in, int n_heads, int causal, float scale, float mask_neg,
                                                               uint64_t seed, uint32_t site, uint32_t thr16, float keep_scale,
-                                                              const int* __restrict__ offsets) {
+                                                              const int* __restrict__ offsets, const T* __restrict__ q_cls, int ld_cls) {
     using C = AttnCfg<T, DH>;
+    constexpr int MT = CQ ? 1 : 2, QR = CQ ? 1 : 4;
     constexpr int WAVE_LDS = 32 * C::PSTRIDE + 32 * C::GSTRIDE;
     extern __shared__ __attribute__((aligned(16))) char smem[];
     const int lane = threadIdx.x & 63, wave = threadIdx.x >> 6;
@@ -110,7 +111,8 @@
         sv[i] = ldg16(base + (size_t)min(row, S - 1) * ld + v_off + ch * C::PER);
     }
     f32x4_t sc[2][2];
-    qk_scores<T, DH>(base, ld, q_off, k_off, S, lane, sc);
+    if constexpr (CQ) qk_scores<T, DH, 1>(q_cls + (size_t)item * ld_cls + head * DH, 0, base + k_off, ld, S, lane, sc);
+    else qk_scores<T, DH, 2>(base + q_off, ld, base + k_off, ld, S, lane, sc);
 #pragma unroll
     for (int nt = 0; nt < 2; ++nt)
         if (nt * 16 + r16 >= S) km[nt] = 0.f;
@@ -122,9 +124,9 @@
     }
 
 #pragma unroll
-    for (int mt = 0; mt < 2; ++mt)
-#pragma unroll
-        for (int rr = 0; rr < 4; ++rr) {
+    for (int mt = 0; mt < MT; ++mt)
+#pragma unroll
+        for (int rr = 0; rr < QR; ++rr) {
             const int q = mt * 16 + kg * 4 + rr;
             const float s2[2] = {sc[mt][0][rr], sc[mt][1][rr]};
             float p[2];
@@ -139,34 +141,37 @@
         }
     wave_lds_fence();
 
-    f32x4_t o[2][C::DT];
-#pragma unroll
-    for (int mt = 0; mt < 2; ++mt)
+    f32x4_t o[MT][C::DT];
+#pragma unroll
+    for (int mt = 0; mt < MT; ++mt)
 #pragma unroll
         for (int dt = 0; dt < C::DT; ++dt) o[mt][dt] = f32x4_t{0.f, 0.f, 0.f, 0.f};
 #pragma unroll
     for (int ks = 0; ks < C::KSP; ++ks) {
-        uint4 pa[2];
-#pragma unroll
-        for (int mt = 0; mt < 2; ++mt)
+        uint4 pa[MT];
+#pragma unroll
+        for (int mt = 0; mt < MT; ++mt)
             pa[mt] = *reinterpret_cast<const uint4*>(Ps + (mt * 16 + r16) * C::PSTRIDE + (ks * 4 + kg) * 16);
 #pragma unroll
         for (int dt = 0; dt < C::DT; ++dt) {
             const uint4 vb = gather_chunk<T>(Vs, C::GSTRIDE, ks * C::KSTEP, dt * 16, lane);
 #pragma unroll
-            for (int mt = 0; mt < 2; ++mt) Mma<T>::mma(pa[mt], vb, o[mt][dt]);
-        }
-    }
-    wave_lds_fence();
-#pragma unroll
-    for (int mt = 0; mt < 2; ++mt)
+            for (int mt = 0; mt < MT; ++mt) Mma<T>::mma(pa[mt], vb, o[mt][dt]);
+        }
+    }
+    wave_lds_fence();
+#pragma unroll
+    for (int mt = 0; mt < MT; ++mt)
 #pragma unroll
         for (int dt = 0; dt < C::DT; ++dt)
 #pragma unroll
-            for (int rr = 0; rr < 4; ++rr)
+            for (int rr = 0; rr < QR; ++rr)
                 Elem<T>::st(reinterpret_cast<T*>(Vs + (mt * 16 + kg * 4 + rr) * C::OSTRIDE) + dt * 16 + r16, o[mt][dt][rr]);
     wave_lds_fence();
-    if (active) {
+    if constexpr (CQ) {
+        if (active && lane < C::CPR)
+            *reinterpret_cast<uint4*>(out + (size_t)item * ldo + head * DH + lane * C::PER) = *reinterpret_cast<const uint4*>(Vs + lane * 16);
+    } else if (active) {
 #pragma unroll
         for (int i = 0; i < C::NLD; ++i) {
             const int id = lane + 64 * i, row = id / C::CPR, ch = id % C::CPR;
@@ -222,13 +227,14 @@
     }
 }
 
-template <typename T, int DH, int WAVES>
+template <typename T, int DH, int WAVES, bool CQ>
 __global__ void __launch_bounds__(WAVES * 64) attn_bwd_kernel(const T* __restrict__ qkv, int ld, int q_off, int k_off, int v_off,
                                                               const T* __restrict__ dout, int ldo, T* __restrict__ dqkv,
                                                               const float* __restrict__ key_mask, int n_items, int S_in, int n_heads,
                                                               int causal, float scale, float mask_neg,
                                                               uint64_t seed, uint32_t site, uint32_t thr16, float keep_scale,
-                                                              const int* __restrict__ offsets) {
+                                                              const int* __restrict__ offsets, const T* __restrict__ q_cls,
+                                                              T* __restrict__ dq_cls, int ld_cls) {
     using C = AttnCfg<T, DH>;
     constexpr int TILE = 32 * C::GSTRIDE, IMG = 32 * C::PSTRIDE;
     constexpr int WAVE_LDS = 3 * TILE + 3 * IMG;
@@ -249,7 +255,9 @@
     const int row0 = offsets ? __builtin_amdgcn_readfirstlane(offsets[item]) : item * S_in;
     const int S = offsets ? __builtin_amdgcn_readfirstlane(offsets[item + 1]) - row0 : S_in;
     const T* base = qkv + (size_t)row0 * ld + head * DH;
-    const T* dbase = dout + (size_t)row0 * ldo + head * DH;
+    const T* dbase = CQ ? dout + (size_t)item * ldo + head * DH : dout + (size_t)row0 * ldo + head * DH;
+    const T* qbase = CQ ? q_cls + (size_t)item * ld_cls + head * DH : base + q_off;
+    const int ldq = CQ ? 0 : ld, ldd = CQ ? 0 : ldo;
     T* gbase = dqkv + (size_t)row0 * ld + head * DH;
 
     float km[2];
@@ -264,10 +272,10 @@
 #pragma unroll
         for (int t = 0; t < 2; ++t) {
             const int row = t * 16 + r16, rc = min(row, S - 1);
-            fq[ks][t] = ldg16(base + (size_t)rc * ld + q_off + (ks * 4 + kg) * C::PER);
+            fq[ks][t] = ldg16(qbase + (size_t)rc * ldq + (ks * 4 + kg) * C::PER);
             fk[ks][t] = ldg16(base + (size_t)rc * ld + k_off + (ks * 4 + kg) * C::PER);
             fv[ks][t] = ldg16(base + (size_t)rc * ld + v_off + (ks * 4 + kg) * C::PER);
-            fd[ks][t] = ldg16(dbase + (size_t)rc * ldo + (ks * 4 + kg) * C::PER);
+            fd[ks][t] = ldg16(dbase + (size_t)rc * ldd + (ks * 4 + kg) * C::PER);
         }
 #pragma unroll
     for (int nt = 0; nt < 2; ++nt)
@@ -281,7 +289,7 @@
             const uint4 z = make_uint4(0u, 0u, 0u, 0u);
             lds_put16<T, C::GSTRIDE>(Qs, row, ch, in ? fq[ks][t] : z);
             lds_put16<T, C::GSTRIDE>(Ks, row, ch, in ? fk[ks][t] : z);
-            if (!in) fd[ks][t] = z;
+            if (CQ ? row != 0 : !in) fd[ks][t] = z;
             lds_put16<T, C::GSTRIDE>(dOs, row, ch, fd[ks][t]);
         }
 
@@ -337,7 +345,8 @@
     store_block<T, DH>(Qs, acc, gbase + k_off, ld, S, lane, active);
     img_times_tile<T, DH>(dS, Ks, lane, acc);
     wave_lds_fence();
-    store_block<T, DH>(Ks, acc, gbase + q_off, ld, S, lane, active);
+    if constexpr (CQ) store_block<T, DH>(Ks, acc, dq_cls + (size_t)item * ld_cls + head * DH, ld_cls, 1, lane, active);
+    else store_block<T, DH>(Ks, acc, gbase + q_off, ld, S, lane, active);
 }
 
 #ifndef A4R_ATTN_BWD_ABL_CT
@@ -376,15 +385,17 @@
     return mx ? fmaxf(v, b) : v + b;
 }
 
-template <int DH, int WAVES>
+template <int DH, int WAVES, bool CQ>
 __global__ void __launch_bounds__(WAVES * 64, 3) attn_bwd_tr_kernel(const bf16_t* __restrict__ qkv, int ld, int q_off, int k_off, int v_off,
                                                                  const bf16_t* __restrict__ dout, int ldo, bf16_t* __restrict__ dqkv,
                                                                  const float* __restrict__ key_mask, int n_items, int S_in, int n_heads,
                                                                  int causal, float scale, float mask_neg,
                                                                  uint64_t seed, uint32_t site, uint32_t thr16, float keep_scale,
-                                                                 const int* __restrict__ offsets) {
+                                                                 const int* __restrict__ offsets, const bf16_t* __restrict__ q_cls,
+                                                                 bf16_t* __restrict__ dq_cls, int ld_cls) {
     using T = bf16_t;
     using G = BtGeo<DH>;
+    constexpr int MT = CQ ? 1 : 2;
     extern __shared__ __attribute__((aligned(16))) char smem[];
     const int lane = threadIdx.x & 63, wave = threadIdx.x >> 6;
     const int r16 = lane & 15, kg = lane >> 4;
@@ -398,7 +409,9 @@
     const int row0 = offsets ? __builtin_amdgcn_readfirstlane(offsets[item]) : item * S_in;
     const int S = offsets ? __builtin_amdgcn_readfirstlane(offsets[item + 1]) - row0 : S_in;
     const T* base = qkv + (size_t)row0 * ld + head * DH;
-    const T* dbase = dout + (size_t)row0 * ldo + head * DH;
+    const T* dbase = CQ ? dout + (size_t)item * ldo + head * DH : dout + (size_t)row0 * ldo + head * DH;
+    const T* qbase = CQ ? q_cls + (size_t)item * ld_cls + head * DH : base + q_off;
+    const int ldq = CQ ? 0 : ld, ldd = CQ ? 0 : ldo;
     T* gbase = dqkv + (size_t)row0 * ld + head * DH;
 
     float kmT[2][4];
@@ -416,17 +429,17 @@
         for (int t = 0; t < 2; ++t) {
             const int row = t * 16 + r16, rc = min(row, S - 1);
             if (A4R_ATTN_BWD_ABL_CT & 2) { fq[ks][t] = make_uint4(lane, ks, t, 1); fk[ks][t] = fq[ks][t]; fv[ks][t] = fq[ks][t]; fd[ks][t] = fq[ks][t]; continue; }
-            fq[ks][t] = ldg16(base + (size_t)rc * ld + q_off + (ks * 4 + kg) * 8);
+            fq[ks][t] = ldg16(qbase + (size_t)rc * ldq + (ks * 4 + kg) * 8);
             fk[ks][t] = ldg16(base + (size_t)rc * ld + k_off + (ks * 4 + kg) * 8);
             fv[ks][t] = ldg16(base + (size_t)rc * ld + v_off + (ks * 4 + kg) * 8);
-            fd[ks][t] = ldg16(dbase + (size_t)rc * ldo + (ks * 4 + kg) * 8);
+            fd[ks][t] = ldg16(dbase + (size_t)rc * ldd + (ks * 4 + kg) * 8);
         }
 #pragma unroll
     for (int ks = 0; ks < G::KSD; ++ks)
 #pragma unroll
         for (int t = 0; t < 2; ++t) {
             const int row = t * 16 + r16, off = row * G::ROWB + (((ks * 4 + kg) ^ G::swz(row)) << 4);
-            if (row >= S) fd[ks][t] = make_uint4(0u, 0u, 0u, 0u);
+            if (CQ ? row != 0 : row >= S) fd[ks][t] = make_uint4(0u, 0u, 0u, 0u);
             *reinterpret_cast<uint4*>(Qi + off) = fq[ks][t];
             *reinterpret_cast<uint4*>(Ki + off) = fk[ks][t];
             *reinterpret_cast<uint4*>(Oi + off) = fd[ks][t];
@@ -439,7 +452,7 @@
 #pragma unroll
     for (int ks = 0; ks < G::KSD; ++ks)
 #pragma unroll
-        for (int mt = 0; mt < 2; ++mt)
+        for (int mt = 0; mt < MT; ++mt)
 #pragma unroll
             for (int nt = 0; nt < 2; ++nt) {
                 Mma<T>::mma(fk[ks][nt], fq[ks][mt], scT[nt][mt]);
@@ -447,9 +460,9 @@
             }
     wave_lds_fence();
     uint2 pw[2][2], dw[2][2];
-    f32x4_t aq[2][G::ND], av[2][G::ND], ak[2][G::ND];
-#pragma unroll
-    for (int mt = 0; mt < 2; ++mt) {
+    f32x4_t aq[MT][G::ND], av[2][G::ND], ak[2][G::ND];
+#pragma unroll
+    for (int mt = 0; mt < MT; ++mt) {
         const int q = mt * 16 + r16;
         float x[2][4];
         float m = -INFINITY;
@@ -509,7 +522,7 @@
 #pragma unroll
     for (int nt = 0; nt < 2; ++nt)
 #pragma unroll
-        for (int mt = 0; mt < 2; ++mt) {
+        for (int mt = 0; mt < MT; ++mt) {
             const int q = mt * 16 + r16, k0 = nt * 16 + kg * 4;
             Pt[(k0 + 0) * 32 + q] = (unsigned short)(pw[nt][mt].x & 0xffffu);
             Pt[(k0 + 1) * 32 + q] = (unsigned short)(pw[nt][mt].x >> 16);
@@ -524,8 +537,12 @@
 #pragma unroll
     for (int nt = 0; nt < 2; ++nt) {
         const int key = nt * 16 + r16;
-        const uint2 p0 = *reinterpret_cast<const uint2*>(Pt + key * 32 + kg * 4), p1 = *reinterpret_cast<const uint2*>(Pt + key * 32 + 16 + kg * 4);
-        const uint2 d0 = *reinterpret_cast<const uint2*>(Dt + key * 32 + kg * 4), d1 = *reinterpret_cast<const uint2*>(Dt + key * 32 + 16 + kg * 4);
+        const uint2 p0 = *reinterpret_cast<const uint2*>(Pt + key * 32 + kg * 4), d0 = *reinterpret_cast<const uint2*>(Dt + key * 32 + kg * 4);
+        uint2 p1 = make_uint2(0u, 0u), d1 = p1;
+        if constexpr (!CQ) {
+            p1 = *reinterpret_cast<const uint2*>(Pt + key * 32 + 16 + kg * 4);
+            d1 = *reinterpret_cast<const uint2*>(Dt + key * 32 + 16 + kg * 4);
+        }
         const uint4 pB = make_uint4(p0.x, p0.y, p1.x, p1.y), dsB = make_uint4(d0.x, d0.y, d1.x, d1.y);
 #pragma unroll
         for (int dt = 0; dt < G::ND; ++dt) {
@@ -542,7 +559,7 @@
 #pragma unroll
         for (int dt = 0; dt < G::ND; ++dt) {
             const int off = tok * G::ROWB + (((dt * 2 + (kg >> 1)) ^ G::swz(tok)) << 4) + 8 * (kg & 1);
-            bt_store4(reinterpret_cast<T*>(Qi + off), aq[t][dt]);
+            if (t < MT) bt_store4(reinterpret_cast<T*>(Qi + off), aq[t < MT ? t : 0][dt]);
             bt_store4(reinterpret_cast<T*>(Oi + off), av[t][dt]);
             bt_store4(reinterpret_cast<T*>(Ki + off), ak[t][dt]);
         }
@@ -554,7 +571,11 @@
             const int id = lane + 64 * i, row = id / G::CPR, ch = id % G::CPR;
             if (row < S) {
                 const int off = row * G::ROWB + ((ch ^ G::swz(row)) << 4);
-                *reinterpret_cast<uint4*>(gbase + (size_t)row * ld + q_off + ch * 8) = *reinterpret_cast<const uint4*>(Qi + off);
+                if constexpr (CQ) {
+                    if (row == 0) *reinterpret_cast<uint4*>(dq_cls + (size_t)item * ld_cls + head * DH + ch * 8) = *reinterpret_cast<const uint4*>(Qi + off);
+                } else {
+                    *reinterpret_cast<uint4*>(gbase + (size_t)row * ld + q_off + ch * 8) = *reinterpret_cast<const uint4*>(Qi + off);
+                }
                 *reinterpret_cast<uint4*>(gbase + (size_t)row * ld + v_off + ch * 8) = *reinterpret_cast<const uint4*>(Oi + off);
                 *reinterpret_cast<uint4*>(gbase + (size_t)row * ld + k_off + ch * 8) = *reinterpret_cast<const uint4*>(Ki + off);
             }
@@ -564,49 +585,52 @@
 
 struct Launch {
     hipStream_t s; const a4r_attn_t* a; uint32_t thr; float ks;
+    const void* q_cls = nullptr; void* dq_cls = nullptr; int ld_cls = 0;
 };
 
-template <typename T, int DH, int WAVES>
+template <typename T, int DH, int WAVES, bool CQ = false>
 int launch_fwd(const Launch& L) {
     using C = AttnCfg<T, DH>;
     const a4r_attn_t& a = *L.a;
     constexpr int LDS = WAVES * (32 * C::PSTRIDE + 32 * C::GSTRIDE);
     const int total = a.n_items * a.n_heads;
-    hipLaunchKernelGGL((attn_fwd_kernel<T, DH, WAVES>), dim3((total + WAVES - 1) / WAVES), dim3(WAVES * 64), LDS, L.s,
+    hipLaunchKernelGGL((attn_fwd_kernel<T, DH, WAVES, CQ>), dim3((total + WAVES - 1) / WAVES), dim3(WAVES * 64), LDS, L.s,
                        (const T*)a.qkv, a.ld, a.q_off, a.k_off, a.v_off, (T*)a.out, a.ldo, a.offsets ? nullptr : a.key_mask, a.n_items, a.S, a.n_heads,
-                       a.causal, a.scale, a.mask_neg, a.drop_seed, a.drop_site, L.thr, L.ks, a.offsets);
+                       a.causal, a.scale, a.mask_neg, a.drop_seed, a.drop_site, L.thr, L.ks, a.offsets, (const T*)L.q_cls, L.ld_cls);
     return a4r_launch_status();
 }
-template <typename T, int DH, int WAVES>
+template <typename T, int DH, int WAVES, bool CQ = false>
 int launch_bwd(const Launch& L) {
     using C = AttnCfg<T, DH>;
     const a4r_attn_t& a = *L.a;
     constexpr int LDS = WAVES * (3 * 32 * C::GSTRIDE + 3 * 32 * C::PSTRIDE);
     static bool lds_ok = false;
     if (!lds_ok) {
-        if (int rc = a4r_set_lds(attn_bwd_kernel<T, DH, WAVES>, LDS)) return rc;
+        if (int rc = a4r_set_lds(attn_bwd_kernel<T, DH, WAVES, CQ>, LDS)) return rc;
         lds_ok = true;
     }
     const int total = a.n_items * a.n_heads;
-    hipLaunchKernelGGL((attn_bwd_kernel<T, DH, WAVES>), dim3((total + WAVES - 1) / WAVES), dim3(WAVES * 64), LDS, L.s,
+    hipLaunchKernelGGL((attn_bwd_kernel<T, DH, WAVES, CQ>), dim3((total + WAVES - 1) / WAVES), dim3(WAVES * 64), LDS, L.s,
                        (const T*)a.qkv, a.ld, a.q_off, a.k_off, a.v_off, (const T*)a.dout, a.ldo, (T*)a.dqkv, a.offsets ? nullptr : a.key_mask,
-                       a.n_items, a.S, a.n_heads, a.causal, a.scale, a.mask_neg, a.drop_seed, a.drop_site, L.thr, L.ks, a.offsets);
+                       a.n_items, a.S, a.n_heads, a.causal, a.scale, a.mask_neg, a.drop_seed, a.drop_site, L.thr, L.ks, a.offsets,
+                       (const T*)L.q_cls, (T*)L.dq_cls, L.ld_cls);
     return a4r_launch_status();
 }
 
-template <int DH, int WAVES>
+template <int DH, int WAVES, bool CQ = false>
 int launch_bwd_tr(const Launch& L) {
     const a4r_attn_t& a = *L.a;
     constexpr int LDS = WAVES * BtGeo<DH>::WAVE_LDS;
     static bool lds_ok = false;
     if (!lds_ok) {
-        if (int rc = a4r_set_lds(attn_bwd_tr_kernel<DH, WAVES>, LDS)) return rc;
+        if (int rc = a4r_set_lds(attn_bwd_tr_kernel<DH, WAVES, CQ>, LDS)) return rc;
         lds_ok = true;
     }
     const int total = a.n_items * a.n_heads;
-    hipLaunchKernelGGL((attn_bwd_tr_kernel<DH, WAVES>), dim3((total + WAVES - 1) / WAVES), dim3(WAVES * 64), LDS, L.s,
+    hipLaunchKernelGGL((attn_bwd_tr_kernel<DH, WAVES, CQ>), dim3((total + WAVES - 1) / WAVES), dim3(WAVES * 64), LDS, L.s,
                        (const bf16_t*)a.qkv, a.ld, a.q_off, a.k_off, a.v_off, (const bf16_t*)a.dout, a.ldo, (bf16_t*)a.dqkv, a.offsets ? nullptr : a.key_mask,
-                       a.n_items, a.S, a.n_heads, a.causal, a.scale, a.mask_neg, a.drop_seed, a.drop_site, L.thr, L.ks, a.offsets);
+                       a.n_items, a.S, a.n_heads, a.causal, a.scale, a.mask_neg, a.drop_seed, a.drop_site, L.thr, L.ks, a.offsets,
+                       (const bf16_t*)L.q_cls, (bf16_t*)L.dq_cls, L.ld_cls);
     return a4r_launch_status();
 }
 
@@ -628,6 +652,14 @@
     return A4R_OK;
 }
 
+int check_cls(const a4r_attn_t* a, bool bwd, const void* q_cls, void* dq_cls, int ld_cls) {
+    if (int e = check(a, bwd)) return e;
+    const int esz = a->dtype == A4R_F32 ? 4 : 2;
+    if (a->dh != 64 || !q_cls || (bwd && !dq_cls) || ld_cls < a->n_heads * a->dh || (ld_cls * esz) % 16) return A4R_EINVAL;
+    if ((reinterpret_cast<uintptr_t>(q_cls) | reinterpret_cast<uintptr_t>(dq_cls)) & 15u) return A4R_EINVAL;
+    return A4R_OK;
+}
+
 }
 
 int a4r_attn_small(hipStream_t s, const a4r_attn_t* t, bool bwd);
@@ -653,3 +685,15 @@
     if (a->dh == 256) return launch_bwd<float, 256, 1>(L);
     return a->dh == 64 ? launch_bwd<float, 64, 2>(L) : launch_bwd<float, 32, 4>(L);
 }
+
+extern "C" int a4r_attn_cls_fwd(void* stream, const a4r_attn_t* a, const void* q_cls, int ld_cls) {
+    if (int e = check_cls(a, false, q_cls, nullptr, ld_cls)) return e;
+    Launch L{reinterpret_cast<hipStream_t>(stream), a, a4r_thr16(a->drop_p), a4r_keep_scale(a->drop_p), q_cls, nullptr, ld_cls};
+    return a->dtype == A4R_BF16 ? launch_fwd<bf16_t, 64, 4, true>(L) : launch_fwd<float, 64, 4, true>(L);
+}
+
+extern "C" int a4r_attn_cls_bwd(void* stream, const a4r_attn_t* a, const void* q_cls, void* dq_cls, int ld_cls) {
+    if (int e = check_cls(a, true, q_cls, dq_cls, ld_cls)) return e;
+    Launch L{reinterpret_cast<hipStream_t>(stream), a, a4r_thr16(a->drop_p), a4r_keep_scale(a->drop_p), q_cls, dq_cls, ld_cls};
+    return a->dtype == A4R_BF16 ? launch_bwd_tr<64, 4, true>(L) : launch_bwd<float, 64, 2, true>(L);
+}
diff --git a/adapter4rec_amd/engine.py b/adapter4rec_amd/engine.py
--- a/adapter4rec_amd/engine.py
+++ b/adapter4rec_amd/engine.py
@@ -835,6 +835,7 @@
                 d['ctx_o'] = self._buf(pre + '.ctx_o', M, H, T)
         if Mc is not None:
             pre, M = pre + '.cls', Mc
+            d['q_c'] = self._buf(pre + '.q_c', M, H, T)
         if (blk.lora or blk.pl1 == 'parallel' or blk.train_dense) and not shared:
             d['xin'] = self._buf(pre + '.xin', d['qkv'].shape[0], H, T)
         if (blk.pl2 == 'parallel' or blk.train_dense) and not shared:
@@ -951,6 +952,23 @@
             L.rows_idx_copy(src, dst, self._pk['off'], n_items, scatter=True)
         else:
             L.scatter_rows_fill(src, dst, n_items, S, M)
+
+    CLS_QUERY = True
+
+    def _cls_query_ok(self, blk, bufs, cls_rows):
+        return (self.CLS_QUERY and cls_rows is not None and 'q_c' in bufs and hasattr(L, 'attn_cls_fwd') and not self.fp8
+                and not getattr(blk, 'long', False) and blk.S <= 32 and blk.dh == 64 and not blk.lora and not blk.train_dense
+                and 'xin' not in bufs and getattr(blk, 'Hv', blk.H) == blk.H)
+
+    @staticmethod
+    def _cls_query_views(blk):
+        v = getattr(blk, '_cq_views', None)
+        if v is None or v[0] != (blk.wqkv.data_ptr(), blk.wqkvT.data_ptr()):
+            H, b = blk.H, blk.bqkv
+            v = ((blk.wqkv.data_ptr(), blk.wqkvT.data_ptr()),
+                 (blk.wqkv[:H], blk.wqkv[H:], None if b is None else b[:H], None if b is None else b[H:], blk.wqkvT[:, :H], blk.wqkvT[:, H:]))
+            blk._cq_views = v
+        return v[1]
 
     def _twin_of(self, t, M):
         w = self._twin.get(t.data_ptr())
@@ -1071,7 +1089,11 @@
         pa = blk.p_attn if train else 0.0
         ph = blk.p_hidden if train else 0.0
         f8 = self.fp8 and T == torch.bfloat16 and M % 256 == 0 and getattr(blk, 'wqkv8', None) is not None
-        if f8:
+        cq = self._cls_query_ok(blk, bufs, cls_rows)
+        if cq:
+            wq, wkv, bq, bkv, _, _ = self._cls_query_views(blk)
+            L.gemm_nt(x, wkv, bufs['qkv'][:, H:], bias=bkv, M=M)
+        elif f8:
             if x8 is None:
                 x8 = (self._buf('x8', M, H, torch.uint8), self._buf('x8s', M, 1, torch.float32))
                 L.quant_rows_fp8(x, x8[0], x8[1], M=M)
@@ -1084,14 +1106,21 @@
             ctx = bufs['ctx_o'] if 'ctx_o' in bufs else self._buf('ctx', M, H, T)
             L.attn_long_fwd(bufs['qkv'], ctx, bufs['lse'], n_items, blk.S, blk.nh, blk.dh, 0, H, 2 * H, blk.scale,
                             drop_p=pa, drop_site=blk.site, drop_seed=seed, key_mask=key_mask, causal=blk.causal)
+        elif cq:
+            ctx_c, x_c = self._buf('ctx_c', cls_rows, H, T), self._buf('x_c', cls_rows, H, T)
+            self._cls_gather(x, x_c, n_items, blk.S, blk)
+            L.gemm_nt(x_c, wq, bufs['q_c'], bias=bq, M=cls_rows)
+            L.attn_cls_fwd(bufs['qkv'], bufs['q_c'], ctx_c, key_mask, n_items, blk.S, blk.nh, blk.dh, H, 2 * H, blk.causal, blk.scale, blk.mask_neg,
+                           drop_p=pa, drop_site=blk.site, drop_seed=seed, offsets=self._off(blk))
         else:
             ctx = bufs['ctx_s'] if ('ctx_s' in bufs and cls_rows is None) else self._buf('ctx', M, H, T)
             L.attn_fwd(bufs['qkv'], ctx, key_mask, n_items, blk.S, blk.nh, blk.dh, 0, H, 2 * H, blk.causal, blk.scale, blk.mask_neg,
                        drop_p=pa, drop_site=blk.site, drop_seed=seed, offsets=self._off(blk))
         if cls_rows is not None:
-            ctx_c, x_c = self._buf('ctx_c', cls_rows, H, T), self._buf('x_c', cls_rows, H, T)
-            self._cls_gather(ctx, ctx_c, n_items, blk.S, blk)
-            self._cls_gather(x, x_c, n_items, blk.S, blk)
+            if not cq:
+                ctx_c, x_c = self._buf('ctx_c', cls_rows, H, T), self._buf('x_c', cls_rows, H, T)
+                self._cls_gather(ctx, ctx_c, n_items, blk.S, blk)
+                self._cls_gather(x, x_c, n_items, blk.S, blk)
             x32 = self._twin_of(x, M) if (self.res32 or self.res24) else None
             if x32 is not None:
                 if x32.dtype == torch.int8:
@@ -1351,6 +1380,24 @@
             return
         dctx = self._buf('dctx_c' if cls_rows is not None else 'dctx', M, H, T)
         L.gemm_nt(dh1, blk.woT, dctx, M=M)
+        if self._cls_query_ok(blk, bufs, cls_rows):
+            M = M_full
+            n_tok = self._pk['Mtok'] if self._off(blk) is not None else n_items * blk.S
+            dqkv = self._buf_tail0('dqkv', M, 3 * H, T, n_tok)
+            dq_c = self._buf('dq_c', cls_rows, H, T)
+            L.attn_cls_bwd(bufs['qkv'], bufs['q_c'], dctx, dqkv, dq_c, key_mask, n_items, blk.S, blk.nh, blk.dh, H, 2 * H, blk.causal, blk.scale,
+                           blk.mask_neg, drop_p=pa, drop_site=blk.site, drop_seed=seed, offsets=self._off(blk))
+            if dx_in is not None:
+                _, _, _, _, wqT, wkvT = self._cls_query_views(blk)
+                L.gemm_nt(dqkv[:, H:], wkvT, dx_in, M=M)
+                dx_g, dx_c = self._buf('dx_g', cls_rows, H, T), self._buf('dx_c', cls_rows, H, T)
+                self._cls_gather(dx_in, dx_g, n_items, blk.S, blk)
+                L.gemm_nt(dq_c, wqT, dx_c, R1=dx_g, R2=dres1, M=cls_rows)
+                if self._off(blk) is not None:
+                    L.rows_idx_copy(dx_c, dx_in, self._pk['off'], n_items, scatter=True)
+                else:
+                    L.scatter_rows(dx_c, dx_in, n_items, blk.S)
+            return
         if cls_rows is not None:
             M = M_full
             full = self._buf('dctx', M, H, T)
diff --git a/include/a4r.h b/include/a4r.h
--- a/include/a4r.h
+++ b/include/a4r.h
@@ -102,6 +102,8 @@
 } a4r_attn_t;
 int a4r_attn_fwd(void* stream, const a4r_attn_t* a);
 int a4r_attn_bwd(void* stream, const a4r_attn_t* a);
+int a4r_attn_cls_fwd(void* stream, const a4r_attn_t* a, const void* q_cls, int ld_cls);
+int a4r_attn_cls_bwd(void* stream, const a4r_attn_t* a, const void* q_cls, void* dq_cls, int ld_cls);
 
 int a4r_attn_long_fwd(void* stream, const a4r_attn_t* a, float* lse);
 int a4r_attn_long_bwd(void* stream, const a4r_attn_t* a, const float* lse, float* delta_ws);
```

After: 1874 (median of 6 runs). No clear change (+0.7%).
